# DeMoriarty/TorchPQ

Hardware: AMD Instinct MI355X
Metric: queries/sec + recall@100, SIFT1M IVFPQ d=128 m=64 nprobe=32 (higher is better)
Workload: dtype f32; 1 GPU; SIFT1M-like d=128 n=1000000 IVFPQ n_cells=1024 m=64 nprobe=32 k=100 on 1xMI355X per rank; n_query_per_rank=10000, code_layout=packed, codes=u8 (8-bit PQ), arithmetic=f32 LUT entries, f32 sums, exact ids, use_smart_probing=False, parallelism=query-sharded x1, replicated index, world_size_seen=1, index_broadcast_bytes=0

## Files before the change

include/torchpq_amd.h:

```cpp
#ifndef TORCHPQ_AMD_H_
#define TORCHPQ_AMD_H_

#include <stddef.h>
#include <stdint.h>

#ifdef __cplusplus
extern "C" {
#endif

#define TPQ_VERSION 500

#define TPQ_OK 0
#define TPQ_ERR_INVALID_ARGUMENT (-1)
#define TPQ_ERR_HIP (-2)
#define TPQ_ERR_WORKSPACE (-3)
#define TPQ_ERR_UNSUPPORTED (-4)

#define TPQ_METRIC_NEG_SQ_L2 0
#define TPQ_METRIC_INNER 1

typedef void* tpq_stream_t;

int tpq_version(void);
const char* tpq_last_error(void);

size_t tpq_ivfpq_scan_workspace_bytes(int nq, int k, int n_split, int m);

int tpq_ivfpq_scan_topk(const uint8_t* codes, const float* lut, const uint8_t* is_empty,
                        const int64_t* cell_start, const int64_t* cell_size,
                        const int64_t* n_probe_list, float* out_vals, int64_t* out_addr,
                        const int64_t* address2id, int64_t* out_ids, int64_t n_slots, int nq,
                        int max_nprobe, int m, int k, int n_split, void* workspace,
                        size_t workspace_bytes, tpq_stream_t stream);

int tpq_ivfpq_pack_codes(const uint8_t* codes, uint8_t* packed, int64_t n_slots, int m,
                         int64_t slot_begin, int64_t slot_end, tpq_stream_t stream);

int tpq_ivfpq_scan_topk_packed(const uint8_t* packed, const uint8_t* codes, const float* lut,
                               const uint8_t* is_empty, const int64_t* cell_start,
                               const int64_t* cell_size, const int64_t* n_probe_list,
                               float* out_vals, int64_t* out_addr, const int64_t* address2id,
                               int64_t* out_ids, int64_t n_slots, int nq, int max_nprobe, int m,
                               int k, int n_split, void* workspace, size_t workspace_bytes,
                               tpq_stream_t stream);
size_t tpq_ivfpq_scan_tickets_bytes(int nq);

#define TPQ_SCAN_ROUTE_REF 0
#define TPQ_SCAN_ROUTE_ONE_LAUNCH 1
#define TPQ_SCAN_ROUTE_LISTS 2
#define TPQ_SCAN_ROUTE_POOLS 3
#define TPQ_SCAN_ROUTE_DUMP_F32 8
#define TPQ_SCAN_ROUTE_DUMP_SEL16 16
#define TPQ_SCAN_ROUTE_DUMP_SEL16_W8 17
int tpq_ivfpq_scan_route(int nq, int k, int n_split, int m, int ds, int max_nprobe, int64_t slots_hint, int has_lut,
                         int has_packed, int has_tickets, int residual);
int tpq_ivfpq_scan_order(const int64_t* cell_start, const int64_t* cell_size, const int64_t* n_probe_list, int nq,
                         int max_nprobe, int tile_shift, int32_t* order, int32_t* rank, int32_t* work,
                         tpq_stream_t stream);
int tpq_ivfpq_scan_ordered(int nq, int k, int n_split, int m, int ds, int max_nprobe, int64_t slots_hint, int has_lut,
                           int has_packed, int has_tickets, int residual, int slots, size_t workspace_bytes);
int tpq_ivfpq_scan_topk_packed_tickets(const uint8_t* packed, const uint8_t* codes, const float* lut,
                                       const uint8_t* is_empty, const int64_t* cell_start,
                                       const int64_t* cell_size, const int64_t* n_probe_list,
                                       float* out_vals, int64_t* out_addr, const int64_t* address2id,
                                       int64_t* out_ids, int64_t n_slots, int nq, int max_nprobe,
                                       int m, int k, int n_split, void* workspace,
                                       size_t workspace_bytes, int32_t* tickets, int64_t slots_hint,
                                       tpq_stream_t stream);

int tpq_ivfpq_search_fused(const uint8_t* packed, const uint8_t* codes, const float* query,
                           const float* codebook, int ds, int metric, const uint8_t* is_empty,
                           const int64_t* cell_start, const int64_t* cell_size,
                           const int64_t* n_probe_list, float* out_vals, int64_t* out_addr,
                           const int64_t* address2id, int64_t* out_ids, int64_t n_slots, int nq,
                           int max_nprobe, int m, int k, int n_split, void* workspace,
                           size_t workspace_bytes, tpq_stream_t stream);
int tpq_ivfpq_search_fused_tickets(const uint8_t* packed, const uint8_t* codes, const float* query,
                                   const float* codebook, int ds, int metric, const uint8_t* is_empty,
                                   const int64_t* cell_start, const int64_t* cell_size,
                                   const int64_t* n_probe_list, float* out_vals, int64_t* out_addr,
                                   const int64_t* address2id, int64_t* out_ids, int64_t n_slots,
                                   int nq, int max_nprobe, int m, int k, int n_split, void* workspace,
                                   size_t workspace_bytes, int32_t* tickets, int64_t slots_hint,
                                   tpq_stream_t stream);
int tpq_ivfpq_search_fused_cells(const uint8_t* packed, const uint8_t* codes, const float* query,
                                 const float* codebook, int ds, int metric, const uint8_t* is_empty,
                                 const int64_t* cell_start, const int64_t* cell_size,
                                 const int64_t* n_probe_list, float* out_vals, int64_t* out_addr,
                                 const int64_t* address2id, int64_t* out_ids, int64_t n_slots,
                                 int nq, int max_nprobe, int m, int k, int n_split, void* workspace,
                                 size_t workspace_bytes, int32_t* tickets, int64_t slots_hint,
                                 const int64_t* cells, int n_cells, tpq_stream_t stream);
int tpq_ivfpq_scan_cell_major(int nq, int k, int n_split, int m, int ds, int max_nprobe, int64_t slots_hint, int has_lut,
                              int has_packed, int has_tickets, int residual, int n_cells, int64_t n_slots,
                              size_t workspace_bytes);
int tpq_ivfpq_scan_cell_norms(int nq, int k, int n_split, int m, int ds, int max_nprobe, int64_t slots_hint, int has_lut,
                              int has_packed, int has_tickets, int residual, int n_cells, int64_t n_slots,
                              size_t workspace_bytes);
size_t tpq_ivfpq_cell_candidates_workspace_bytes(int nq, int max_nprobe, int n_cells, int first_probe);
size_t tpq_ivfpq_cell_candidates_norms_workspace_bytes(int nq, int max_nprobe, int n_cells, int first_probe,
                                                       int64_t n_slots);
int tpq_ivfpq_cell_candidates(const uint8_t* codes, const float* query, const float* codebook, int ds, int metric,
                              const uint8_t* is_empty, const int64_t* cell_start, const int64_t* cell_size,
                              const int64_t* n_probe_list, const int64_t* cells, int n_cells, int first_probe,
                              const float* threshold, int64_t n_slots, int nq, int max_nprobe, int m, int capacity,
                              int32_t* out_count, uint32_t* out_keys, uint32_t* out_addr, float* out_delta,
                              int32_t* out_flags, void* workspace, size_t workspace_bytes, tpq_stream_t stream);
float tpq_ivfpq_cell_fold_threshold(float threshold, float q2);
int tpq_ivfpq_scan_cell_threshold(int nq, int k, int n_split, int m, int ds, int max_nprobe, int64_t slots_hint,
                                  int has_lut, int has_packed, int has_tickets, int residual, int n_cells,
                                  int64_t n_slots, size_t workspace_bytes);
int tpq_ivfpq_scan_use_cell_threshold(int on);
int tpq_ivfpq_scan_cell_threshold_probes(void);

int tpq_ivfpq_scan_topk_residual(const uint8_t* codes, const float* part1, const float* part2,
                                 const float* full_lut, const int64_t* cells,
                                 const float* base_sims, const uint8_t* is_empty,
                                 const int64_t* cell_start, const int64_t* cell_size,
                                 const int64_t* n_probe_list, float* out_vals, int64_t* out_addr,
                                 const int64_t* address2id, int64_t* out_ids, int64_t n_slots,
                                 int nq, int max_nprobe, int m, int k, tpq_stream_t stream);
int tpq_residual_part1(const float* query, const float* codebook, float* part1, int m, int ds,
                       int nq, tpq_stream_t stream);

int tpq_ivfpq_residual_slot_terms(const uint8_t* codes, const float* part2,
                                  const int64_t* cell_start, const int64_t* cell_size,
                                  float* slot_term, float* cell_bound, int64_t n_slots,
                                  int n_cells, int m, tpq_stream_t stream);
int tpq_ivfpq_scan_topk_residual_packed(
    const uint8_t* packed, const uint8_t* codes, const float* part1, const float* query,
    const float* codebook, int ds, const float* part2, const float* slot_term,
    const float* cell_bound, const int64_t* cells, const float* base_sims, const uint8_t* is_empty,
    const int64_t* cell_start, const int64_t* cell_size, const int64_t* n_probe_list,
    float* out_vals, int64_t* out_addr, const int64_t* address2id, int64_t* out_ids,
    int64_t n_slots, int nq, int max_nprobe, int m, int k, int n_split, void* workspace,
    size_t workspace_bytes, tpq_stream_t stream);

int tpq_adc_lut(const float* query, const float* codebook, float* lut, int m, int ds, int nq,
                int metric, tpq_stream_t stream);

int tpq_topk_select(const float* x, float* vals, int64_t* idx, int rows, int cols, int k,
                    tpq_stream_t stream);

int tpq_coarse_select(const float* dots, const float* a2, const float* b2, float* vals, int64_t* idx,
                      int rows, int cols, int k, tpq_stream_t stream);

size_t tpq_ivfpq_coarse_probe_workspace_bytes(int nq, int n_cells);
int tpq_ivfpq_coarse_probe(const float* query, const float* centroids,
                           const int64_t* cell_start_tbl, const int64_t* cell_size_tbl,
                           float* topk_sims, int64_t* cells, int64_t* cell_start,
                           int64_t* cell_size, int64_t* n_probe_list, int d, int nq, int n_cells,
                           int n_probe, float smart_temperature, void* workspace,
                           size_t workspace_bytes, tpq_stream_t stream);
#define TPQ_PROBE_ROUTE_AUTO 0
#define TPQ_PROBE_ROUTE_FP32 1
#define TPQ_PROBE_ROUTE_FP16 2
size_t tpq_ivfpq_coarse_probe_route_workspace_bytes(int d, int nq, int n_cells, int route);
int tpq_ivfpq_coarse_probe_route(const float* query, const float* centroids,
                                 const int64_t* cell_start_tbl, const int64_t* cell_size_tbl,
                                 float* topk_sims, int64_t* cells, int64_t* cell_start,
                                 int64_t* cell_size, int64_t* n_probe_list, int d, int nq, int n_cells,
                                 int n_probe, float smart_temperature, int route, const void* prepared,
                                 void* workspace, size_t workspace_bytes, tpq_stream_t stream);
size_t tpq_ivfpq_coarse_probe_prepared_bytes(int d, int n_cells);
int tpq_ivfpq_coarse_probe_prepare(const float* centroids, int d, int n_cells, void* prepared,
                                   size_t prepared_bytes, tpq_stream_t stream);

int tpq_smart_probing(const float* topk_sims, int64_t* n_probe_list, int rows, int n_probe,
                      float temperature, tpq_stream_t stream);

int tpq_get_address_by_id(const int64_t* address2id, int64_t capacity, const int64_t* ids,
                          int64_t* address, int64_t n_ids, tpq_stream_t stream);

int tpq_get_id_by_address(const int64_t* address2id, int64_t capacity, const int64_t* address,
                          int64_t* ids, int64_t n, tpq_stream_t stream);

int tpq_max_sim(const float* A, const float* B, float* vals, int64_t* inds, int l, int d, int m,
                int n, int metric, tpq_stream_t stream);

int tpq_max_sim_split_supported(int d, int64_t m, int n);
int tpq_max_sim_split(const float* A, const float* B, float* vals, int64_t* inds, int l, int d, int m,
                      int n, int metric, tpq_stream_t stream);

#define TPQ_ASSIGN_ROUTE_AUTO 0
#define TPQ_ASSIGN_ROUTE_CASCADE 1
int tpq_coarse_assign_supported(int d, int64_t m, int n);
size_t tpq_coarse_assign_workspace_bytes(int d, int64_t m, int n);
size_t tpq_coarse_assign_count_offset(int d, int64_t m, int n);
int tpq_coarse_assign(const float* A, const float* B, float* vals, int64_t* inds, int d, int64_t m, int n,
                      int metric, void* workspace, size_t workspace_bytes, tpq_stream_t stream);
size_t tpq_coarse_assign_route_workspace_bytes(int d, int64_t m, int n, int route);
int tpq_coarse_assign_route(const float* A, const float* B, float* vals, int64_t* inds, int d, int64_t m, int n,
                            int metric, int route, void* workspace, size_t workspace_bytes, tpq_stream_t stream);

int tpq_max_sim_select_supported(int l, int d, int64_t m, int n);
size_t tpq_max_sim_select_workspace_bytes(int l, int d, int64_t m, int n);
int tpq_max_sim_select(const float* A, const float* B, float* vals, int64_t* inds, int l, int d, int64_t m,
                       int n, int metric, void* workspace, size_t workspace_bytes, tpq_stream_t stream);

int tpq_lloyd_supported(int l, int d, int64_t m, int n);
size_t tpq_lloyd_prepared_bytes(int l, int d, int64_t m);
int tpq_lloyd_prepare(const float* data, const float* centroids0, void* prepared, size_t prepared_bytes,
                      int l, int d, int64_t m, int n, tpq_stream_t stream);
size_t tpq_lloyd_step_workspace_bytes(int l, int d, int64_t m, int n);
size_t tpq_lloyd_step_count_offset(int l, int d, int64_t m, int n, int level);
int tpq_lloyd_step(const float* data, const void* prepared, const float* centroids, float* new_centroids,
                   float* vals, int64_t* inds, int l, int d, int64_t m, int n, void* workspace,
                   size_t workspace_bytes, tpq_stream_t stream);

size_t tpq_compute_centroids_workspace_bytes(int l, int d, int k);
int tpq_compute_centroids(const float* data, const int64_t* labels, float* centroids, int l, int d,
                          int64_t n, int k, void* workspace, size_t workspace_bytes,
                          tpq_stream_t stream);

size_t tpq_get_ioa_workspace_bytes(int64_t n);
int tpq_get_ioa(const int64_t* labels, int64_t* ioa, int64_t n, int64_t n_cells, void* workspace,
                size_t workspace_bytes, tpq_stream_t stream);
int tpq_get_write_address(const uint8_t* is_empty, const int64_t* cell_start,
                          const int64_t* cell_capacity, const int64_t* labels, const int64_t* ioa,
                          int64_t* write_address, int64_t n_slots, int64_t n_labels,
                          tpq_stream_t stream);
int tpq_get_cell_by_address(const int64_t* address, const int64_t* cell_start,
                            const int64_t* cell_capacity, int64_t* cells, int64_t n_address,
                            int64_t n_cells, tpq_stream_t stream);

int tpq_grow_cells(const uint8_t* storage, const int64_t* address2id, const uint8_t* is_empty,
                   const int64_t* old_start, const int64_t* old_capacity, const int64_t* new_start,
                   const int64_t* new_capacity, uint8_t* new_storage, int64_t* new_address2id,
                   uint8_t* new_is_empty, int64_t old_slots, int64_t new_slots, int n_cells, int m,
                   tpq_stream_t stream);

int tpq_pq_decode(const float* codebook, const uint8_t* codes, float* out, int m, int ds, int64_t n,
                  tpq_stream_t stream);

int tpq_scatter_codes(const uint8_t* codes, const int64_t* address, uint8_t* storage,
                      uint8_t* packed, int m, int64_t n, int64_t n_slots, tpq_stream_t stream);

int tpq_ivfpqr_rerank(const uint8_t* storage, int64_t capacity, int m, int m_r, const float* codebook,
                      const float* codebook_r, const float* query, int d, int nq, const int64_t* cand_address,
                      int k1, int k, int use_residual, int distance, const int64_t* address2id, float* out_vals,
                      int64_t* out_address, int64_t* out_ids, tpq_stream_t stream);

size_t tpq_ivfflat_scan_workspace_bytes(int nq, int k, int n_split);
int tpq_ivfflat_scan_topk(const float* vectors, const float* query, const uint8_t* is_empty,
                          const int64_t* cell_start, const int64_t* cell_size, const int64_t* n_probe_list,
                          float* out_vals, int64_t* out_addr, int64_t n_slots, int d, int nq, int max_nprobe, int k,
                          int metric, int n_split, void* workspace, size_t workspace_bytes, tpq_stream_t stream);

size_t tpq_ivfpq4_scan_workspace_bytes(int nq, int k, int n_split);
int tpq_ivfpq4_scan_topk(const uint8_t* codes, const float* query, const float* codebook, const uint8_t* is_empty,
                         const int64_t* cell_start, const int64_t* cell_size, const int64_t* n_probe_list,
                         float* out_vals, int64_t* out_addr, int64_t n_slots, int m, int ds, int nq, int max_nprobe,
                         int k, int metric, int n_split, void* workspace, size_t workspace_bytes,
                         tpq_stream_t stream);

int tpq_ivfpq4_scan_residual_topk(const uint8_t* codes, const float* query, const float* codebook,
                                  const float* centroids, const int64_t* cells, int n_cells, const uint8_t* is_empty,
                                  const int64_t* cell_start, const int64_t* cell_size, const int64_t* n_probe_list,
                                  float* out_vals, int64_t* out_addr, int64_t n_slots, int m, int ds, int nq,
                                  int max_nprobe, int k, int metric, int n_split, void* workspace,
                                  size_t workspace_bytes, tpq_stream_t stream);

size_t tpq_ivfflat_range_segments(int nq, int n_split);
int tpq_ivfflat_range_count(const float* vectors, const float* query, const uint8_t* is_empty,
                            const int64_t* cell_start, const int64_t* cell_size, const int64_t* n_probe_list,
                            const float* threshold, int32_t* wave_counts, int64_t n_slots, int d, int nq,
// ... 92 lines not shown
```

torchpq_amd/_lib.py:

```python
from __future__ import annotations

import ctypes as C
import os

import torch

_HERE = os.path.dirname(os.path.abspath(__file__))
LIB_PATH = os.environ.get("TPQ_AMD_LIB") or os.path.join(_HERE, "libtorchpq_amd.so")

METRIC_NEG_SQ_L2 = 0
METRIC_INNER = 1
ERR_UNSUPPORTED = -4
ERR_WORKSPACE = -3
ASSIGN_ROUTE_AUTO = 0
ASSIGN_ROUTE_CASCADE = 1
PROBE_ROUTE_AUTO, PROBE_ROUTE_FP32, PROBE_ROUTE_FP16 = 0, 1, 2

_vp, _i, _i64, _sz, _f = C.c_void_p, C.c_int, C.c_int64, C.c_size_t, C.c_float

SIGNATURES = {
    "tpq_version": (_i, []),
    "tpq_last_error": (C.c_char_p, []),
    "tpq_ivfpq_scan_workspace_bytes": (_sz, [_i, _i, _i, _i]),
    "tpq_ivfpq_scan_topk": (_i, [_vp, _vp, _vp, _vp, _vp, _vp, _vp, _vp, _vp, _vp, _i64, _i, _i, _i,
                                 _i, _i, _vp, _sz, _vp]),
    "tpq_ivfpq_pack_codes": (_i, [_vp, _vp, _i64, _i, _i64, _i64, _vp]),
    "tpq_ivfpq_scan_topk_packed": (_i, [_vp, _vp, _vp, _vp, _vp, _vp, _vp, _vp, _vp, _vp, _vp, _i64,
                                        _i, _i, _i, _i, _i, _vp, _sz, _vp]),
    "tpq_ivfpq_search_fused": (_i, [_vp, _vp, _vp, _vp, _i, _i, _vp, _vp, _vp, _vp, _vp, _vp, _vp, _vp,
                                    _i64, _i, _i, _i, _i, _i, _vp, _sz, _vp]),
    "tpq_ivfpq_scan_tickets_bytes": (_sz, [_i]),
    "tpq_ivfpq_scan_route": (_i, [_i, _i, _i, _i, _i, _i, _i64, _i, _i, _i, _i]),
    "tpq_ivfpq_scan_order": (_i, [_vp, _vp, _vp, _i, _i, _i, _vp, _vp, _vp, _vp]),
    "tpq_ivfpq_scan_ordered": (_i, [_i, _i, _i, _i, _i, _i, _i64, _i, _i, _i, _i, _i, _sz]),
    "tpq_ivfpq_scan_topk_packed_tickets": (_i, [_vp, _vp, _vp, _vp, _vp, _vp, _vp, _vp, _vp, _vp, _vp, _i64,
                                                _i, _i, _i, _i, _i, _vp, _sz, _vp, _i64, _vp]),
    "tpq_ivfpq_search_fused_tickets": (_i, [_vp, _vp, _vp, _vp, _i, _i, _vp, _vp, _vp, _vp, _vp, _vp, _vp, _vp,
                                            _i64, _i, _i, _i, _i, _i, _vp, _sz, _vp, _i64, _vp]),
    "tpq_ivfpq_search_fused_cells": (_i, [_vp, _vp, _vp, _vp, _i, _i, _vp, _vp, _vp, _vp, _vp, _vp, _vp, _vp,
                                          _i64, _i, _i, _i, _i, _i, _vp, _sz, _vp, _i64, _vp, _i, _vp]),
    "tpq_ivfpq_scan_cell_major": (_i, [_i, _i, _i, _i, _i, _i, _i64, _i, _i, _i, _i, _i, _i64, _sz]),
    "tpq_ivfpq_scan_cell_norms": (_i, [_i, _i, _i, _i, _i, _i, _i64, _i, _i, _i, _i, _i, _i64, _sz]),
    "tpq_ivfpq_cell_candidates_workspace_bytes": (_sz, [_i, _i, _i, _i]),
    "tpq_ivfpq_cell_candidates_norms_workspace_bytes": (_sz, [_i, _i, _i, _i, _i64]),
    "tpq_ivfpq_cell_candidates": (_i, [_vp, _vp, _vp, _i, _i, _vp, _vp, _vp, _vp, _vp, _i, _i, _vp, _i64, _i, _i, _i,
                                       _i, _vp, _vp, _vp, _vp, _vp, _vp, _sz, _vp]),
    "tpq_ivfpq_cell_fold_threshold": (_f, [_f, _f]),
    "tpq_ivfpq_scan_cell_threshold": (_i, [_i, _i, _i, _i, _i, _i, _i64, _i, _i, _i, _i, _i, _i64, _sz]),
    "tpq_ivfpq_scan_use_cell_threshold": (_i, [_i]),
    "tpq_ivfpq_scan_cell_threshold_probes": (_i, []),
    "tpq_ivfpq_scan_topk_residual": (_i, [_vp, _vp, _vp, _vp, _vp, _vp, _vp, _vp, _vp, _vp, _vp, _vp,
                                          _vp, _vp, _i64, _i, _i, _i, _i, _vp]),
    "tpq_residual_part1": (_i, [_vp, _vp, _vp, _i, _i, _i, _vp]),
    "tpq_ivfpq_residual_slot_terms": (_i, [_vp, _vp, _vp, _vp, _vp, _vp, _i64, _i, _i, _vp]),
    "tpq_ivfpq_scan_topk_residual_packed": (_i, [_vp, _vp, _vp, _vp, _vp, _i, _vp, _vp, _vp, _vp, _vp,
                                                 _vp, _vp, _vp, _vp, _vp, _vp, _vp, _vp, _i64, _i, _i,
                                                 _i, _i, _i, _vp, _sz, _vp]),
    "tpq_adc_lut": (_i, [_vp, _vp, _vp, _i, _i, _i, _i, _vp]),
    "tpq_topk_select": (_i, [_vp, _vp, _vp, _i, _i, _i, _vp]),
    "tpq_coarse_select": (_i, [_vp, _vp, _vp, _vp, _vp, _i, _i, _i, _vp]),
    "tpq_smart_probing": (_i, [_vp, _vp, _i, _i, _f, _vp]),
    "tpq_ivfpq_coarse_probe_workspace_bytes": (_sz, [_i, _i]),
    "tpq_ivfpq_coarse_probe": (_i, [_vp, _vp, _vp, _vp, _vp, _vp, _vp, _vp, _vp, _i, _i, _i, _i, _f,
                                    _vp, _sz, _vp]),
    "tpq_ivfpq_coarse_probe_route_workspace_bytes": (_sz, [_i, _i, _i, _i]),
    "tpq_ivfpq_coarse_probe_route": (_i, [_vp, _vp, _vp, _vp, _vp, _vp, _vp, _vp, _vp, _i, _i, _i, _i, _f, _i,
                                          _vp, _vp, _sz, _vp]),
    "tpq_ivfpq_coarse_probe_prepared_bytes": (_sz, [_i, _i]),
    "tpq_ivfpq_coarse_probe_prepare": (_i, [_vp, _i, _i, _vp, _sz, _vp]),
    "tpq_get_id_by_address": (_i, [_vp, _i64, _vp, _vp, _i64, _vp]),
    "tpq_get_address_by_id": (_i, [_vp, _i64, _vp, _vp, _i64, _vp]),
    "tpq_max_sim": (_i, [_vp, _vp, _vp, _vp, _i, _i, _i, _i, _i, _vp]),
    "tpq_max_sim_split_supported": (_i, [_i, _i64, _i]),
    "tpq_max_sim_split": (_i, [_vp, _vp, _vp, _vp, _i, _i, _i, _i, _i, _vp]),
    "tpq_max_sim_select_supported": (_i, [_i, _i, _i64, _i]),
    "tpq_max_sim_select_workspace_bytes": (_sz, [_i, _i, _i64, _i]),
    "tpq_max_sim_select": (_i, [_vp, _vp, _vp, _vp, _i, _i, _i64, _i, _i, _vp, _sz, _vp]),
    "tpq_lloyd_supported": (_i, [_i, _i, _i64, _i]),
    "tpq_lloyd_prepared_bytes": (_sz, [_i, _i, _i64]),
    "tpq_lloyd_prepare": (_i, [_vp, _vp, _vp, _sz, _i, _i, _i64, _i, _vp]),
    "tpq_lloyd_step_workspace_bytes": (_sz, [_i, _i, _i64, _i]),
    "tpq_lloyd_step_count_offset": (_sz, [_i, _i, _i64, _i, _i]),
    "tpq_lloyd_step": (_i, [_vp, _vp, _vp, _vp, _vp, _vp, _i, _i, _i64, _i, _vp, _sz, _vp]),
    "tpq_coarse_assign_supported": (_i, [_i, _i64, _i]),
    "tpq_coarse_assign_workspace_bytes": (_sz, [_i, _i64, _i]),
    "tpq_coarse_assign_count_offset": (_sz, [_i, _i64, _i]),
    "tpq_coarse_assign": (_i, [_vp, _vp, _vp, _vp, _i, _i64, _i, _i, _vp, _sz, _vp]),
    "tpq_coarse_assign_route_workspace_bytes": (_sz, [_i, _i64, _i, _i]),
    "tpq_coarse_assign_route": (_i, [_vp, _vp, _vp, _vp, _i, _i64, _i, _i, _i, _vp, _sz, _vp]),
    "tpq_compute_centroids_workspace_bytes": (_sz, [_i, _i, _i]),
    "tpq_compute_centroids": (_i, [_vp, _vp, _vp, _i, _i, _i64, _i, _vp, _sz, _vp]),
    "tpq_get_ioa_workspace_bytes": (_sz, [_i64]),
    "tpq_get_ioa": (_i, [_vp, _vp, _i64, _i64, _vp, _sz, _vp]),
    "tpq_get_write_address": (_i, [_vp, _vp, _vp, _vp, _vp, _vp, _i64, _i64, _vp]),
    "tpq_get_cell_by_address": (_i, [_vp, _vp, _vp, _vp, _i64, _i64, _vp]),
    "tpq_grow_cells": (_i, [_vp, _vp, _vp, _vp, _vp, _vp, _vp, _vp, _vp, _vp, _i64, _i64, _i, _i, _vp]),
    "tpq_pq_decode": (_i, [_vp, _vp, _vp, _i, _i, _i64, _vp]),
    "tpq_scatter_codes": (_i, [_vp, _vp, _vp, _vp, _i, _i64, _i64, _vp]),
    "tpq_ivfpqr_rerank": (_i, [_vp, _i64, _i, _i, _vp, _vp, _vp, _i, _i, _vp, _i, _i, _i, _i, _vp, _vp, _vp, _vp,
                               _vp]),
    "tpq_ivfflat_scan_workspace_bytes": (_sz, [_i, _i, _i]),
    "tpq_ivfflat_scan_topk": (_i, [_vp, _vp, _vp, _vp, _vp, _vp, _vp, _vp, _i64, _i, _i, _i, _i, _i, _i, _vp, _sz,
                                   _vp]),
    "tpq_ivfpq4_scan_workspace_bytes": (_sz, [_i, _i, _i]),
    "tpq_ivfpq4_scan_topk": (_i, [_vp] * 9 + [_i64, _i, _i, _i, _i, _i, _i, _i, _vp, _sz, _vp]),
    "tpq_ivfpq4_scan_residual_topk": (_i, [_vp] * 5 + [_i] + [_vp] * 6 + [_i64, _i, _i, _i, _i, _i, _i, _i, _vp, _sz,
                                           _vp]),
    "tpq_ivfpq4_scan_filtered_topk": (_i, [_vp] * 9 + [_i, _i64, _vp, _vp, _i64, _i, _i, _i, _i, _i, _i, _i, _vp, _sz,
                                           _vp]),
    "tpq_ivfpq4_scan_filtered_residual_topk": (_i, [_vp] * 5 + [_i] + [_vp] * 6 + [_i, _i64, _vp, _vp, _i64, _i, _i,
                                                    _i, _i, _i, _i, _i, _vp, _sz, _vp]),
    "tpq_ivfflat_range_segments": (_sz, [_i, _i]),
    "tpq_ivfflat_range_count": (_i, [_vp, _vp, _vp, _vp, _vp, _vp, _vp, _vp, _i64, _i, _i, _i, _i, _i, _vp]),
    "tpq_ivfflat_range_fill": (_i, [_vp, _vp, _vp, _vp, _vp, _vp, _vp, _vp, _vp, _vp, _i64, _i, _i, _i, _i, _i,
                                    _vp]),
    "tpq_ivfpq_range_segments": (_sz, [_i, _i]),
    "tpq_ivfpq_range_count": (_i, [_vp] * 4 + [_i, _i] + [_vp] * 6 + [_i64, _i, _i, _i, _i, _vp]),
    "tpq_ivfpq_range_fill": (_i, [_vp] * 4 + [_i, _i] + [_vp] * 8 + [_i64, _i, _i, _i, _i, _vp]),
    "tpq_ivfpq_range_residual_segments": (_sz, [_i, _i]),
    "tpq_ivfpq_range_residual_count": (_i, [_vp] * 4 + [_i] + [_vp] * 10 + [_i64, _i, _i, _i, _vp]),
    "tpq_ivfpq_range_residual_fill": (_i, [_vp] * 4 + [_i] + [_vp] * 12 + [_i64, _i, _i, _i, _vp]),
    "tpq_ivfpq_scan_filtered_workspace_bytes": (_sz, [_i, _i, _i]),
    "tpq_ivfpq_scan_filtered_topk": (_i, [_vp] * 4 + [_i, _i] + [_vp] * 6 + [_i, _i64] + [_vp] * 4
                                     + [_i64, _i, _i, _i, _i, _i, _vp, _sz, _vp]),
    "tpq_ivfpq_scan_filtered_residual_topk": (_i, [_vp] * 4 + [_i] + [_vp] * 10 + [_i, _i64] + [_vp] * 4
                                              + [_i64, _i, _i, _i, _i, _vp]),
    "tpq_slot_filter_build": (_i, [_vp, _i64, _vp, _i64, _vp]),
    "tpq_flat_topk_workspace_bytes": (_sz, [_i, _i, _i]),
    "tpq_flat_topk": (_i, [_vp, _vp, _vp, _vp, _vp, _vp, _i64, _i, _i, _i, _i, _i, _vp, _sz, _vp]),
    "tpq_flat_range_segments": (_sz, [_i, _i]),
    "tpq_flat_range_count": (_i, [_vp, _vp, _vp, _vp, _vp, _i64, _i, _i, _i, _i, _vp]),
    "tpq_flat_range_fill": (_i, [_vp, _vp, _vp, _vp, _vp, _vp, _vp, _vp, _i64, _i, _i, _i, _i, _vp]),
    "tpq_ubench_stream_read": (_i, [_vp, _sz, _vp, _i, _vp]),
    "tpq_ubench_stream_read_ex": (_i, [_vp, _sz, _vp, _i, _i, _i, _sz, _i, _vp]),
    "tpq_ubench_rows_read": (_i, [_vp, _i, _i, _i64, _i, _vp, _vp]),
}

_lib = None


class TorchPQAmdError(RuntimeError):
    pass


def load():
    global _lib
    if _lib is None:
        if not os.path.exists(LIB_PATH):
            raise TorchPQAmdError(
                f"{LIB_PATH} not found: build it with `python -c 'import __graft_entry__ as g; "
                "g.build()'` (or torchpq_amd/csrc/build.sh). torchpq_amd has no CPU fallback.")
        lib = C.CDLL(LIB_PATH)
        for name, (res, args) in SIGNATURES.items():
            fn = getattr(lib, name)
            fn.restype = res
            fn.argtypes = args
        _lib = lib
    return _lib


def last_error() -> str:
    msg = load().tpq_last_error()
    return msg.decode("utf-8", "replace") if msg else ""


def check(rc: int, what: str):
    if rc != 0:
        raise TorchPQAmdError(f"{what} failed (code {rc}): {last_error()}")


def ptr(t):
    return None if t is None else C.c_void_p(t.data_ptr())


def stream_ptr(device=None):
    return C.c_void_p(torch.cuda.current_stream(device).cuda_stream)


def require_gpu(*tensors):
    for t in tensors:
        if t is None:
            continue
        if t.device.type != "cuda":
            raise TorchPQAmdError(
                "torchpq_amd runs on an AMD GPU (torch device 'cuda'); got a tensor on "
                f"'{t.device}'. There is no CPU fallback.")
        if not t.is_contiguous():
            raise TorchPQAmdError("torchpq_amd kernels need contiguous tensors")
```

torchpq_amd/csrc/scan.hip:

```cpp
#include <atomic>
#include <chrono>

#include "scan_cells.h"
#include "scan_device.h"
#include "scan_order.h"
#include "scan_ref.h"

namespace tpq {

__global__ __launch_bounds__(256) void residual_part1_kernel(const float* __restrict__ query,
                                                            const float* __restrict__ codebook,
                                                            float* __restrict__ part1, int m,
                                                            int ds, int nq) {
  const int j = blockIdx.y, q = blockIdx.x, c = threadIdx.x;
  float dot = 0.f;
  for (int e = 0; e < ds; ++e)
    dot = fmaf(query[(int64_t)(j * ds + e) * nq + q], codebook[((int64_t)j * ds + e) * 256 + c], dot);
  part1[((int64_t)q * m + j) * 256 + c] = 2.f * dot;
}


static size_t ref_lds_bytes(int m, int R, int max_nprobe, int fused_floats) {
  return list_scan_lds_bytes(list_region0((size_t)m * 1024, R), max_nprobe, (size_t)fused_floats * 4);
}
// ... 114 lines not shown
  }
  if (a.lut || !dump_built(a.m, kDumpSel16) || a.ds > 2) return 0;
  const int rl8 = list_regs_scan(a.k, a.m, a.max_nprobe, a.slots_hint);
  if (rl4 <= 2 || (rl4 <= 4 && rl4 <= rl8)) return kDumpSel16;
  if (e && atoi(e) == 1) return 0;
  if (a.k > 248 && rl8 <= 2) return kDumpSel16W8;
  return 0;
}

template <int N, class Query>
static int device_cached(std::atomic<int> (&cache)[64][N], int i, int fallback, Query query) {
  int dev = 0;
  if (hipGetDevice(&dev) != hipSuccess || dev < 0 || dev >= 64) return fallback;
  int n = cache[dev][i].load(std::memory_order_relaxed);
  if (n <= 0) {
    n = query(dev);
    if (n <= 0) n = fallback;
    cache[dev][i].store(n, std::memory_order_relaxed);
  }
  return n;
}
static int device_cus() {
  static std::atomic<int> cus[64][1] = {};
  return device_cached(cus, 0, 256, [](int dev) {
    int n = 0;
    return hipDeviceGetAttribute(&n, hipDeviceAttributeMultiprocessorCount, dev) == hipSuccess ? n : 0;
  });
}
static int dump_slots(const PackedUnit& u, int mode) {
  static std::atomic<int> per_cu[64][3 * 4] = {};
  const int mi = mode == kDumpSel16 ? 0 : (mode == kDumpF32 ? 1 : 2), ci = u.m == 64 ? 0 : (u.m == 32 ? 1 : (u.m == 16 ? 2 : 3));
  return device_cached(per_cu, mi * 4 + ci, 4, [&](int) { return u.dump_occupancy(mode); }) * device_cus();
}
static void dump_tail(int nq, int nw, int RL, int slots, int* unsplit, int* parts) {
  *unsplit = nq;
  *parts = 1;
  if (slots <= 0) return;
  const int whole = (nq / slots) * slots, rest = nq - whole;
  if (rest == 0) return;
  for (int c = 4; c >= 2; c >>= 1) {
    if ((int64_t)rest * c <= slots && c * nw * RL <= 16) {
      *unsplit = whole;
      *parts = c;
      return;
    }
  }
}

struct ScanPlan {
  int route = -1;
  int R = 0;
  int RL = 0;
  int Rf = 0;
  int mode = 0;
  int waves = 0;
  int n_split = 1;
  bool fuse = false;
  bool small_lists = false;
  int unsplit = 0;
  int parts = 1;
  bool ordered = false;
};

static ScanPlan plan_scan(const ScanArgs& a, bool residual) {
  const int m = a.m, k = a.k;
  ScanPlan p;
  p.n_split = a.n_split;
  if (!packed_unit(m)) {
    if (!residual && !a.lut) p.route = TPQ_SCAN_ROUTE_REF;
    return p;
  }
  p.R = list_regs_packed(k);
  p.waves = packed_waves(m);
  const bool lds_fits =
      scan_lds_bytes_packed(m, p.R > 16 ? 16 : p.R, a.max_nprobe, fused_floats_of(a), residual) <= 160 * 1024;
  if (p.R > 16 || !lds_fits) {
    p.route = TPQ_SCAN_ROUTE_REF;
    if (residual) p.n_split = 1;
    return p;
  }
  const bool pools = !residual && p.R >= pool_min_list_regs(m) && (p.waves < 16 || k > 768) && fuse_enabled();
  const int Rf = dump_finish_regs(k, a.slots_hint), mode = dump_route(a, residual, Rf);
  if (mode && !(is_sel16(mode) && pools)) {
    const int nw = scan_waves(m, mode), RL = list_regs_scan(k, m, a.max_nprobe, a.slots_hint, nw);
    if (dump_pair_built(mode, RL, Rf)) {
      p.route = mode == kDumpF32 ? TPQ_SCAN_ROUTE_DUMP_F32
                                 : (mode == kDumpSel16 ? TPQ_SCAN_ROUTE_DUMP_SEL16 : TPQ_SCAN_ROUTE_DUMP_SEL16_W8);
      p.mode = mode, p.waves = nw, p.RL = RL, p.Rf = Rf, p.n_split = 1;
      return p;
    }
  }
  if (pools) {
    p.route = TPQ_SCAN_ROUTE_POOLS;
    p.RL = pool_list_regs(k, m);
    if (p.n_split > pool_max_split(m, k)) p.n_split = pool_max_split(m, k);
    return p;
  }
  p.RL = list_regs_scan(k, m, a.max_nprobe, a.slots_hint);
  p.small_lists = p.RL < p.R;
  p.fuse = !residual && fuse_enabled() && fuse_fits(m, p.R) && p.waves * p.RL >= p.R && (a.n_split == 1 || a.tickets);
  p.route = p.fuse ? TPQ_SCAN_ROUTE_ONE_LAUNCH : TPQ_SCAN_ROUTE_LISTS;
  return p;
}

static void plan_dump_dispatch(ScanPlan& p, int nq, int slots, size_t workspace_bytes) {
  int unsplit = nq, parts = 1;
  if (p.mode != kDumpSel16W8) dump_tail(nq, p.waves, p.RL, slots, &unsplit, &parts);
  if (parts > 1 && workspace_bytes < ws_bytes_for(nq, p.RL, parts * p.waves)) unsplit = nq, parts = 1;
  p.parts = parts;
  p.unsplit = parts > 1 ? unsplit : 0;
  p.ordered = slots > 0 && nq > slots && nq <= kOrderMaxQueries &&
              workspace_bytes >= ws_bytes_for(nq, p.RL, parts * p.waves) + order_ws_bytes(nq);
}
static bool is_dump_route(int route) {
  return route == TPQ_SCAN_ROUTE_DUMP_F32 || route == TPQ_SCAN_ROUTE_DUMP_SEL16 || route == TPQ_SCAN_ROUTE_DUMP_SEL16_W8;
}

static ScanArgs route_query_args(int nq, int k, int n_split, int m, int ds, int max_nprobe, int64_t slots_hint,
                                 int has_lut, int has_tickets) {
  ScanArgs a{};
  static const float dummy_lut = 0.f;
  static int32_t dummy_tickets = 0;
  a.lut = has_lut ? &dummy_lut : nullptr;
  a.ds = has_lut ? 0 : ds;
  a.nq = nq; a.k = k; a.n_split = n_split; a.m = m; a.max_nprobe = max_nprobe;
  a.slots_hint = slots_hint;
  a.tickets = has_tickets ? &dummy_tickets : nullptr;
  return a;
}

extern "C" int tpq_ivfpq_scan_route(int nq, int k, int n_split, int m, int ds, int max_nprobe, int64_t slots_hint,
                                    int has_lut, int has_packed, int has_tickets, int residual) {
  if (nq <= 0 || k < 1 || k > 1024 || m < 4 || m % 4 != 0 || n_split < 1 || max_nprobe < 1) return -1;
  if (!has_packed) return TPQ_SCAN_ROUTE_REF;
  return plan_scan(route_query_args(nq, k, n_split, m, ds, max_nprobe, slots_hint, has_lut, has_tickets), residual != 0)
      .route;
}

extern "C" int tpq_ivfpq_scan_ordered(int nq, int k, int n_split, int m, int ds, int max_nprobe, int64_t slots_hint,
                                      int has_lut, int has_packed, int has_tickets, int residual, int slots,
                                      size_t workspace_bytes) {
  if (nq <= 0 || k < 1 || k > 1024 || m < 4 || m % 4 != 0 || n_split < 1 || max_nprobe < 1) return -1;
  if (!has_packed) return 0;
  ScanPlan p =
      plan_scan(route_query_args(nq, k, n_split, m, ds, max_nprobe, slots_hint, has_lut, has_tickets), residual != 0);
  if (!is_dump_route(p.route)) return 0;
  plan_dump_dispatch(p, nq, slots > 0 ? slots : dump_slots(*packed_unit(m), p.mode), workspace_bytes);
  return p.ordered ? 1 : 0;
}

struct CellMajor {
  const int64_t* cells;
  int n_cells;
};
static int cell_major_chunks(const ScanArgs& a, const ScanPlan& p, bool residual, int n_cells, size_t workspace_bytes) {
  if (residual || p.route != TPQ_SCAN_ROUTE_DUMP_SEL16 || a.lut || a.m != 64 || a.ds < 1 || a.ds > 2) return 0;
  if (a.k > 128 || a.max_nprobe <= kCellP0 || n_cells < 1 || a.n_slots <= 0 || a.slots_hint <= 0) return 0;
  if ((int64_t)a.nq * a.slots_hint < (int64_t)kCellMinRereads * a.n_slots) return 0;
  if ((int64_t)a.nq * a.max_nprobe >= 0x7fffffffLL) return 0;
  const size_t extra = cell_extra_bytes(a.nq, a.max_nprobe, n_cells, kCellP0);
  for (int chunks = 16; chunks >= 8; chunks >>= 1)
    if ((a.k + 63) / 64 < chunks && workspace_bytes >= ws_bytes_for(a.nq, 1, chunks) + extra) return chunks;
  return 0;
}
static bool cell_major_norms(const ScanArgs& a, int chunks, int n_cells, size_t workspace_bytes) {
  return chunks > 0 && workspace_bytes >= ws_bytes_for(a.nq, 1, chunks) +
                                              cell_extra_bytes(a.nq, a.max_nprobe, n_cells, kCellP0) +
                                              cell_norm_bytes(a.n_slots);
}

static int run_cell_major(ScanArgs& a, ScanPlan p, const PackedUnit& u, const CellMajor& cm, int chunks, void* workspace,
                          size_t workspace_bytes, hipStream_t st) {
  const int nq = a.nq;
  ScanArgs t = a;
  t.probe_cap = kCellP0;
  plan_dump_dispatch(p, nq, dump_slots(u, p.mode), workspace_bytes);
  t.n_split = p.parts;
  t.unsplit = p.unsplit;
  const size_t lists_bytes = ws_bytes_for(nq, p.RL, p.parts * p.waves);
  int rc = need_ws(workspace, workspace_bytes, lists_bytes, "ivfpq_scan_packed");
  if (rc) return rc;
  fill_ws(t, workspace, p.RL, p.parts * p.waves);
  if (p.ordered) {
    int* o = reinterpret_cast<int*>(reinterpret_cast<char*>(workspace) + lists_bytes);
    const size_t stride = order_ws_bytes(nq) / 3 / sizeof(int);
    rc = launch_scan_order(a.cell_start, a.cell_size, a.n_probe_list, nq, a.max_nprobe, packed_tile_shift(a.m), o,
                           o + stride, o + 2 * stride, st, kCellP0);
    if (rc) return rc;
    t.order = o;
    t.rank = o + stride;
  }
  rc = u.dump(t, p.RL, p.Rf, p.mode, st);
  if (rc) return rc;
  a.n_split = 1;
  a.unsplit = 0;
  fill_ws(a, workspace, 1, chunks);
  CellArgs c{};
  c.codes = a.codes; c.query = a.query; c.codebook = a.codebook; c.is_empty = a.is_empty;
  c.cell_start = a.cell_start; c.cell_size = a.cell_size; c.n_probe_list = a.n_probe_list; c.cells = cm.cells;
  c.n_slots = a.n_slots; c.nq = nq; c.max_nprobe = a.max_nprobe; c.n_cells = cm.n_cells; c.ds = a.ds;
  c.euclid = a.euclid; c.p0 = kCellP0; c.p_hi = a.max_nprobe; c.k = a.k; c.chunks = chunks; c.epoch = a.epoch;
  c.rel = cell_delta_rel(a.ds);
  c.seed_vals = a.out_vals; c.seed_addr = a.out_addr;
  c.keys = reinterpret_cast<unsigned*>(a.ws_vals); c.idx = reinterpret_cast<unsigned*>(a.ws_idx);
  c.list_evict = a.list_evict; c.flags = a.flags; c.ws_delta = a.ws_delta;
  const size_t cm_lists = ws_bytes_for(nq, 1, chunks);
  cell_fill_extras(c, reinterpret_cast<char*>(workspace) + cm_lists, workspace_bytes - cm_lists);
  rc = launch_cell_candidates(c, st);
  if (rc) return rc;
  return u.finish(a, chunks, p.Rf, (a.k + 63) / 64, c.cnt, st);
}

static bool cell_threshold_form(const ScanArgs& a, int chunks, int n_cells, size_t workspace_bytes) {
  if (!cell_major_norms(a, chunks, n_cells, workspace_bytes) || a.max_nprobe <= kCellThrProbes) return false;
  const size_t need = ws_bytes_for(a.nq, 1, chunks) + cell_extra_bytes(a.nq, a.max_nprobe, n_cells, kCellP0) +
                      cell_norm_bytes(a.n_slots) + cell_thr_bytes(a.nq, a.max_nprobe, n_cells);
  const int64_t mean_cell = a.slots_hint / a.max_nprobe;
  return workspace_bytes >= need && mean_cell >= kCellThrMinCell &&
         (int64_t)kCellThrProbes * mean_cell / kCellThrGroup >= 2 * (int64_t)a.k;
}

static int run_cell_threshold(ScanArgs& a, const ScanPlan& p, const PackedUnit& u, const CellMajor& cm, int chunks,
                              void* workspace, hipStream_t st) {
  const int nq = a.nq;
  a.n_split = 1;
  a.unsplit = 0;
  fill_ws(a, workspace, 1, chunks);
  CellArgs c{};
  c.codes = a.codes; c.query = a.query; c.codebook = a.codebook; c.is_empty = a.is_empty;
  c.cell_start = a.cell_start; c.cell_size = a.cell_size; c.n_probe_list = a.n_probe_list; c.cells = cm.cells;
  c.n_slots = a.n_slots; c.nq = nq; c.max_nprobe = a.max_nprobe; c.n_cells = cm.n_cells; c.ds = a.ds;
  c.euclid = a.euclid; c.p0 = 0; c.p_hi = a.max_nprobe; c.k = 0; c.thr_k = a.k; c.chunks = chunks; c.epoch = a.epoch;
  c.rel = cell_delta_rel(a.ds);
  c.keys = reinterpret_cast<unsigned*>(a.ws_vals); c.idx = reinterpret_cast<unsigned*>(a.ws_idx);
  c.list_evict = a.list_evict; c.flags = a.flags; c.ws_delta = a.ws_delta;
  char* at = reinterpret_cast<char*>(workspace) + ws_bytes_for(nq, 1, chunks);
  const size_t head = cell_extra_bytes(nq, a.max_nprobe, cm.n_cells, kCellP0) + cell_norm_bytes(a.n_slots);
  cell_fill_extras(c, at, head, kCellP0);
  CellThrArrays t{};
  cell_fill_thr(t, at + head, nq, a.max_nprobe, cm.n_cells);
  int rc = launch_cell_threshold(c, t, st);
  if (rc) return rc;
  return u.finish(a, chunks, p.Rf, 0, c.cnt, st);
}

extern "C" int tpq_ivfpq_scan_cell_major(int nq, int k, int n_split, int m, int ds, int max_nprobe, int64_t slots_hint,
                                         int has_lut, int has_packed, int has_tickets, int residual, int n_cells,
                                         int64_t n_slots, size_t workspace_bytes) {
  if (nq <= 0 || k < 1 || k > 1024 || m < 4 || m % 4 != 0 || n_split < 1 || max_nprobe < 1) return -1;
  if (!has_packed) return 0;
  ScanArgs a = route_query_args(nq, k, n_split, m, ds, max_nprobe, slots_hint, has_lut, has_tickets);
  a.n_slots = n_slots;
  const ScanPlan p = plan_scan(a, residual != 0);
  return cell_major_chunks(a, p, residual != 0, n_cells, workspace_bytes) ? 1 : 0;
}

extern "C" int tpq_ivfpq_scan_cell_norms(int nq, int k, int n_split, int m, int ds, int max_nprobe, int64_t slots_hint,
                                         int has_lut, int has_packed, int has_tickets, int residual, int n_cells,
                                         int64_t n_slots, size_t workspace_bytes) {
  if (nq <= 0 || k < 1 || k > 1024 || m < 4 || m % 4 != 0 || n_split < 1 || max_nprobe < 1) return -1;
  if (!has_packed) return 0;
  ScanArgs a = route_query_args(nq, k, n_split, m, ds, max_nprobe, slots_hint, has_lut, has_tickets);
  a.n_slots = n_slots;
  const ScanPlan p = plan_scan(a, residual != 0);
  const int chunks = cell_major_chunks(a, p, residual != 0, n_cells, workspace_bytes);
  return cell_major_norms(a, chunks, n_cells, workspace_bytes) ? 1 : 0;
}

extern "C" int tpq_ivfpq_scan_cell_threshold(int nq, int k, int n_split, int m, int ds, int max_nprobe,
                                             int64_t slots_hint, int has_lut, int has_packed, int has_tickets,
                                             int residual, int n_cells, int64_t n_slots, size_t workspace_bytes) {
  if (nq <= 0 || k < 1 || k > 1024 || m < 4 || m % 4 != 0 || n_split < 1 || max_nprobe < 1) return -1;
  if (!has_packed) return 0;
  ScanArgs a = route_query_args(nq, k, n_split, m, ds, max_nprobe, slots_hint, has_lut, has_tickets);
  a.n_slots = n_slots;
  const ScanPlan p = plan_scan(a, residual != 0);
  const int chunks = cell_major_chunks(a, p, residual != 0, n_cells, workspace_bytes);
  return cell_threshold_form(a, chunks, n_cells, workspace_bytes) ? 1 : 0;
}

static std::atomic<int> g_cell_threshold{1};
extern "C" int tpq_ivfpq_scan_use_cell_threshold(int on) { return g_cell_threshold.exchange(on ? 1 : 0); }
extern "C" int tpq_ivfpq_scan_cell_threshold_probes(void) { return kCellThrProbes; }

static int run_packed(ScanArgs a, const ResidualArgs* ra, void* workspace, size_t workspace_bytes,
                      tpq_stream_t stream, const CellMajor* cm = nullptr) {
  int rc = validate(a);
  if (rc) return rc;
  TPQ_REQUIRE(a.packed != nullptr, "ivfpq_scan_packed: null packed pointer");
  if (a.nq == 0) return TPQ_OK;
  hipStream_t st = reinterpret_cast<hipStream_t>(stream);
  ScanPlan p = plan_scan(a, ra != nullptr);
  if (p.route == TPQ_SCAN_ROUTE_REF) {
    a.n_split = p.n_split;
    return ra ? run_residual_ref(a, *ra, st) : run_ref(a, workspace, workspace_bytes, st);
  }
  if (p.route < 0) {
    set_error("ivfpq_scan_packed: no scan-layout kernel instantiated for n_subvectors=%d; use "
              "tpq_ivfpq_scan_topk", a.m);
    return TPQ_ERR_UNSUPPORTED;
  }
  const PackedUnit& u = *packed_unit(a.m);
  const int nq = a.nq;
  a.n_split = p.n_split;
  a.small_lists = p.small_lists;
  a.fuse = p.fuse;
  if (!p.fuse) a.tickets = nullptr;
  a.epoch = fresh_epoch();
#ifdef TPQ_SCAN_PROFILE
  a.prof = g_scan_prof;
#endif
  switch (p.route) {
    case TPQ_SCAN_ROUTE_POOLS: {
      const int n_lists = p.n_split * p.waves;
      rc = need_ws(workspace, workspace_bytes, pool_ws_bytes(nq, a.k, a.m, n_lists), "ivfpq_scan_packed");
      if (rc) return rc;
      fill_ws_pool(a, workspace, n_lists);
      rc = u.pool(a, p.RL, st);
      break;
    }
    case TPQ_SCAN_ROUTE_DUMP_F32:
    case TPQ_SCAN_ROUTE_DUMP_SEL16:
    case TPQ_SCAN_ROUTE_DUMP_SEL16_W8: {
      if (const int chunks = cm ? cell_major_chunks(a, p, ra != nullptr, cm->n_cells, workspace ? workspace_bytes : 0) : 0) {
        rc = g_cell_threshold.load() && cell_threshold_form(a, chunks, cm->n_cells, workspace_bytes)
                 ? run_cell_threshold(a, p, u, *cm, chunks, workspace, st)
                 : run_cell_major(a, p, u, *cm, chunks, workspace, workspace_bytes, st);
        break;
      }
      plan_dump_dispatch(p, nq, dump_slots(u, p.mode), workspace ? workspace_bytes : 0);
      a.n_split = p.parts;
      a.unsplit = p.unsplit;
      const size_t lists_bytes = ws_bytes_for(nq, p.RL, p.parts * p.waves);
      rc = need_ws(workspace, workspace_bytes, lists_bytes, "ivfpq_scan_packed");
      if (rc) return rc;
      fill_ws(a, workspace, p.RL, p.parts * p.waves);
      if (p.ordered) {
        int* o = reinterpret_cast<int*>(reinterpret_cast<char*>(workspace) + lists_bytes);
        const size_t stride = order_ws_bytes(nq) / 3 / sizeof(int);
        rc = launch_scan_order(a.cell_start, a.cell_size, a.n_probe_list, nq, a.max_nprobe, packed_tile_shift(a.m), o,
                               o + stride, o + 2 * stride, st, 0);
        if (rc) return rc;
        a.order = o;
        a.rank = o + stride;
      }
      rc = u.dump(a, p.RL, p.Rf, p.mode, st);
      break;
    }
    default: {
      const int n_lists = p.n_split * p.waves;
      rc = need_ws(workspace, workspace_bytes, ws_bytes_for(nq, p.RL, n_lists), "ivfpq_scan_packed");
      if (rc) return rc;
      fill_ws(a, workspace, p.RL, n_lists);
      rc = u.packed(a, ra, p.RL, p.R, st);
      if (p.fuse) return rc;
    }
  }
  if (rc) return rc;
  return redo_flagged(a, ra, st);
}

extern "C" size_t tpq_ivfpq_scan_tickets_bytes(int nq) { return nq > 0 ? (size_t)nq * sizeof(int32_t) : 0; }

extern "C" int tpq_ivfpq_search_fused_cells(const uint8_t* packed, const uint8_t* codes,
                                            const float* query, const float* codebook, int ds,
                                            int metric, const uint8_t* is_empty,
                                            const int64_t* cell_start, const int64_t* cell_size,
                                            const int64_t* n_probe_list, float* out_vals,
                                            int64_t* out_addr, const int64_t* address2id,
                                            int64_t* out_ids, int64_t n_slots, int nq, int max_nprobe,
                                            int m, int k, int n_split, void* workspace,
                                            size_t workspace_bytes, int32_t* tickets,
                                            int64_t slots_hint, const int64_t* cells, int n_cells,
                                            tpq_stream_t stream) {
  TPQ_REQUIRE(metric == TPQ_METRIC_NEG_SQ_L2 || metric == TPQ_METRIC_INNER,
              "ivfpq_search_fused: bad metric %d", metric);
  TPQ_REQUIRE(ds >= 1 && ds <= 1024, "ivfpq_search_fused: bad sub-vector length %d", ds);
  ScanArgs a = scan_args(codes, packed, nullptr, is_empty, cell_start, cell_size, n_probe_list, out_vals, out_addr,
                         address2id, out_ids, n_slots, nq, max_nprobe, m, k, n_split);
  a.query = query; a.codebook = codebook; a.ds = ds; a.euclid = metric == TPQ_METRIC_NEG_SQ_L2 ? 1 : 0;
  a.tickets = tickets; a.slots_hint = slots_hint;
  const CellMajor cm{cells, n_cells};
  return packed ? run_packed(a, nullptr, workspace, workspace_bytes, stream, cells ? &cm : nullptr)
                : run_ref(a, workspace, workspace_bytes, reinterpret_cast<hipStream_t>(stream));
}

extern "C" int tpq_ivfpq_search_fused_tickets(const uint8_t* packed, const uint8_t* codes,
                                              const float* query, const float* codebook, int ds,
                                              int metric, const uint8_t* is_empty,
                                              const int64_t* cell_start, const int64_t* cell_size,
                                              const int64_t* n_probe_list, float* out_vals,
                                              int64_t* out_addr, const int64_t* address2id,
                                              int64_t* out_ids, int64_t n_slots, int nq, int max_nprobe,
                                              int m, int k, int n_split, void* workspace,
                                              size_t workspace_bytes, int32_t* tickets,
                                              int64_t slots_hint, tpq_stream_t stream) {
  return tpq_ivfpq_search_fused_cells(packed, codes, query, codebook, ds, metric, is_empty, cell_start, cell_size,
                                      n_probe_list, out_vals, out_addr, address2id, out_ids, n_slots, nq, max_nprobe, m,
                                      k, n_split, workspace, workspace_bytes, tickets, slots_hint, nullptr, 0, stream);
}

extern "C" int tpq_ivfpq_search_fused(const uint8_t* packed, const uint8_t* codes,
                                      const float* query, const float* codebook, int ds,
                                      int metric, const uint8_t* is_empty,
                                      const int64_t* cell_start, const int64_t* cell_size,
                                      const int64_t* n_probe_list, float* out_vals,
                                      int64_t* out_addr, const int64_t* address2id,
                                      int64_t* out_ids, int64_t n_slots, int nq, int max_nprobe,
                                      int m, int k, int n_split, void* workspace,
                                      size_t workspace_bytes, tpq_stream_t stream) {
  return tpq_ivfpq_search_fused_tickets(packed, codes, query, codebook, ds, metric, is_empty, cell_start,
                                        cell_size, n_probe_list, out_vals, out_addr, address2id, out_ids,
                                        n_slots, nq, max_nprobe, m, k, n_split, workspace, workspace_bytes,
                                        nullptr, 0, stream);
}

extern "C" int tpq_ivfpq_scan_topk(const uint8_t* codes, const float* lut, const uint8_t* is_empty,
                                   const int64_t* cell_start, const int64_t* cell_size,
                                   const int64_t* n_probe_list, float* out_vals, int64_t* out_addr,
                                   const int64_t* address2id, int64_t* out_ids, int64_t n_slots,
                                   int nq, int max_nprobe, int m, int k, int n_split,
                                   void* workspace, size_t workspace_bytes, tpq_stream_t stream) {
  const ScanArgs a = scan_args(codes, nullptr, lut, is_empty, cell_start, cell_size, n_probe_list, out_vals, out_addr,
                               address2id, out_ids, n_slots, nq, max_nprobe, m, k, n_split);
  return run_ref(a, workspace, workspace_bytes, reinterpret_cast<hipStream_t>(stream));
}

extern "C" int tpq_ivfpq_scan_topk_packed_tickets(const uint8_t* packed, const uint8_t* codes,
                                                  const float* lut, const uint8_t* is_empty,
                                                  const int64_t* cell_start, const int64_t* cell_size,
                                                  const int64_t* n_probe_list, float* out_vals,
                                                  int64_t* out_addr, const int64_t* address2id,
                                                  int64_t* out_ids, int64_t n_slots, int nq, int max_nprobe,
                                                  int m, int k, int n_split, void* workspace,
                                                  size_t workspace_bytes, int32_t* tickets,
                                                  int64_t slots_hint, tpq_stream_t stream) {
  ScanArgs a = scan_args(codes, packed, lut, is_empty, cell_start, cell_size, n_probe_list, out_vals, out_addr,
                         address2id, out_ids, n_slots, nq, max_nprobe, m, k, n_split);
  a.tickets = tickets; a.slots_hint = slots_hint;
  return run_packed(a, nullptr, workspace, workspace_bytes, stream);
}

extern "C" int tpq_ivfpq_scan_topk_packed(const uint8_t* packed, const uint8_t* codes,
                                          const float* lut, const uint8_t* is_empty,
                                          const int64_t* cell_start, const int64_t* cell_size,
                                          const int64_t* n_probe_list, float* out_vals,
                                          int64_t* out_addr, const int64_t* address2id,
                                          int64_t* out_ids, int64_t n_slots, int nq, int max_nprobe,
                                          int m, int k, int n_split, void* workspace,
                                          size_t workspace_bytes, tpq_stream_t stream) {
  return tpq_ivfpq_scan_topk_packed_tickets(packed, codes, lut, is_empty, cell_start, cell_size, n_probe_list,
                                            out_vals, out_addr, address2id, out_ids, n_slots, nq, max_nprobe, m,
                                            k, n_split, workspace, workspace_bytes, nullptr, 0, stream);
}

extern "C" int tpq_ivfpq_scan_topk_residual(const uint8_t* codes, const float* part1,
                                            const float* part2, const float* full_lut,
                                            const int64_t* cells, const float* base_sims,
                                            const uint8_t* is_empty, const int64_t* cell_start,
                                            const int64_t* cell_size, const int64_t* n_probe_list,
                                            float* out_vals, int64_t* out_addr,
                                            const int64_t* address2id, int64_t* out_ids,
                                            int64_t n_slots, int nq, int max_nprobe, int m, int k,
                                            tpq_stream_t stream) {
  const ScanArgs a = scan_args(codes, nullptr, part1 ? part1 : full_lut, is_empty, cell_start, cell_size, n_probe_list,
                               out_vals, out_addr, address2id, out_ids, n_slots, nq, max_nprobe, m, k, 1);
  int rc = validate(a);
  if (rc) return rc;
  TPQ_REQUIRE(base_sims != nullptr, "ivfpq_scan_residual: base_sims is required");
  TPQ_REQUIRE(full_lut != nullptr || (part1 && part2 && cells),
              "ivfpq_scan_residual: need either full_lut or (part1, part2, cells)");
  if (nq == 0) return TPQ_OK;
  ResidualArgs ra{part1, part2, full_lut, cells, base_sims, nullptr, nullptr};
  return run_residual_ref(a, ra, reinterpret_cast<hipStream_t>(stream));
}

extern "C" int tpq_ivfpq_scan_topk_residual_packed(
    const uint8_t* packed, const uint8_t* codes, const float* part1, const float* query,
    const float* codebook, int ds, const float* part2, const float* slot_term,
    const float* cell_bound, const int64_t* cells, const float* base_sims, const uint8_t* is_empty,
    const int64_t* cell_start, const int64_t* cell_size, const int64_t* n_probe_list,
    float* out_vals, int64_t* out_addr, const int64_t* address2id, int64_t* out_ids,
    int64_t n_slots, int nq, int max_nprobe, int m, int k, int n_split, void* workspace,
    size_t workspace_bytes, tpq_stream_t stream) {
  TPQ_REQUIRE(part1 || (query && codebook && ds >= 1 && ds <= 1024),
              "ivfpq_scan_residual_packed: need part1 or (query, codebook, ds)");
  TPQ_REQUIRE(part2 && slot_term && cell_bound && cells && base_sims,
              "ivfpq_scan_residual_packed: null pointer argument");
  ScanArgs a = scan_args(codes, packed, part1, is_empty, cell_start, cell_size, n_probe_list, out_vals, out_addr,
                         address2id, out_ids, n_slots, nq, max_nprobe, m, k, n_split);
  a.query = query; a.codebook = codebook; a.ds = ds;
  a.euclid = 2;
  ResidualArgs ra{part1, part2, nullptr, cells, base_sims, slot_term, cell_bound};
  return run_packed(a, &ra, workspace, workspace_bytes, stream);
}

namespace tpq {
__global__ __launch_bounds__(256) void residual_slot_term_kernel(
    const uint32_t* __restrict__ codes32, const float* __restrict__ part2,
    const int64_t* __restrict__ cell_start, const int64_t* __restrict__ cell_size,
    float* __restrict__ slot_term, int64_t n_slots, int m) {
  const int cell = blockIdx.x;
  const float* __restrict__ p2 = part2 + (int64_t)cell * m * 256;
  const int64_t st = cell_start[cell], sz = cell_size[cell];
  const int G = m >> 2;
  for (int64_t o = (int64_t)blockIdx.y * 256 + threadIdx.x; o < sz; o += (int64_t)gridDim.y * 256) {
    const int64_t s = st + o;
    float v = 0.f;
    for (int g = 0; g < G; ++g) {
      const uint32_t w = codes32[(int64_t)g * n_slots + s];
      v = lut_word(v, p2 + g * 1024, w);
    }
    slot_term[s] = v;
  }
}

__global__ __launch_bounds__(64) void residual_cell_bound_kernel(const float* __restrict__ part2,
                                                                 float* __restrict__ cell_bound,
                                                                 int m) {
  const int cell = blockIdx.x, lane = threadIdx.x;
  const float4* __restrict__ p2 = reinterpret_cast<const float4*>(part2 + (int64_t)cell * m * 256);
  float sum = 0.f;
  for (int j = 0; j < m; ++j) {
    const float4 x = p2[j * 64 + lane];
    float mx = fmaxf(fmaxf(fabsf(x.x), fabsf(x.y)), fmaxf(fabsf(x.z), fabsf(x.w)));
#pragma unroll
    for (int d = 32; d > 0; d >>= 1) mx = fmaxf(mx, __shfl_xor(mx, d, 64));
    sum += mx;
  }
  if (lane == 0) cell_bound[cell] = sum;
}
}

extern "C" int tpq_ivfpq_residual_slot_terms(const uint8_t* codes, const float* part2,
                                             const int64_t* cell_start, const int64_t* cell_size,
                                             float* slot_term, float* cell_bound, int64_t n_slots,
                                             int n_cells, int m, tpq_stream_t stream) {
// ... 31 lines not shown
```

torchpq_amd/csrc/scan_cells.h:

```cpp
#pragma once
#include "common.h"

namespace tpq {

#ifndef TPQ_CELL_P0
#define TPQ_CELL_P0 4
#endif
constexpr int kCellP0 = TPQ_CELL_P0;
#ifndef TPQ_CELL_THR_PROBES
#define TPQ_CELL_THR_PROBES 6
#endif
#ifndef TPQ_CELL_THR_GROUP
#define TPQ_CELL_THR_GROUP 16
#endif
constexpr int kCellThrProbes = TPQ_CELL_THR_PROBES;
constexpr int kCellThrGroup = TPQ_CELL_THR_GROUP;
static_assert(kCellThrGroup == 8 || kCellThrGroup == 16, "a group is half or all of a lane's 16 rows of a tile");
constexpr int kCellThrMinCell = 512;
constexpr int kCellMinRereads = 96;
constexpr int kCellQSplit = 256;
constexpr int kCellGroup = 32;
#ifndef TPQ_CELL_SLICE
#define TPQ_CELL_SLICE 128
#endif
constexpr int kCellSlice = TPQ_CELL_SLICE;
constexpr int kCellLdsCells = 16384;

struct CellArgs {
  const uint8_t* codes;
  const float* query;
  const float* codebook;
  const uint8_t* is_empty;
  const int64_t* cell_start;
  const int64_t* cell_size;
  const int64_t* n_probe_list;
  const int64_t* cells;
  int64_t n_slots;
  int nq, max_nprobe, n_cells, ds, euclid;
  int p0;
  int p_hi;
  int k;
  int thr_k;
  int work;
  int chunks;
  int epoch;
  float rel;
  const float* seed_vals;
  const int64_t* seed_addr;
  const float* thr_in;
  unsigned* keys;
  unsigned* idx;
  int* list_evict;
  int* flags;
  float* ws_delta;
  float* params;
  float* thr;
  float* qscale;
  float* qnorm;
  int* cnt;
  int* hist;
  int* cell_off;
  int* blk_off;
  int* cell_st;
  int* cell_sz;
  int* pairs;
  _Float16* qsplit;
  float* norm;
  int* hist2;
  int* n_max;
};
struct CellThrArrays {
  int* pairs_b;
  int *hist, *cell_off, *blk_off, *cell_st, *cell_sz, *pairs, *n_max;
};

inline size_t cell_align(size_t x) { return (x + 255) & ~(size_t)255; }
inline size_t cell_extra_bytes(int nq, int max_nprobe, int n_cells, int p0) {
  const int np = max_nprobe > p0 ? max_nprobe - p0 : 0;
  return 256 + 4 * cell_align((size_t)nq * 4) + cell_align((size_t)n_cells * 4) +
         2 * cell_align(((size_t)n_cells + 1) * 4) + 2 * cell_align((size_t)n_cells * 4) +
         cell_align((size_t)nq * np * 4) + cell_align((size_t)nq * kCellQSplit * 2);
}
inline size_t cell_norm_bytes(int64_t n_slots) { return cell_align((size_t)(n_slots > 0 ? n_slots : 0) * 4); }
inline size_t cell_thr_bytes(int nq, int max_nprobe, int n_cells) {
  const int t = max_nprobe < kCellThrProbes ? max_nprobe : kCellThrProbes;
  return cell_align((size_t)nq * max_nprobe * 4) + 3 * cell_align((size_t)n_cells * 4) +
         2 * cell_align(((size_t)n_cells + 1) * 4) + cell_align((size_t)nq * t * 4) + cell_align((size_t)nq * 4);
}
__host__ __device__ inline int cell_float_ord(float f) {
  const unsigned b = __builtin_bit_cast(unsigned, f);
  return (b & 0x80000000u) ? (int)(0x80000000u - b) : (int)b;
}
__host__ __device__ inline float cell_ord_float(int o) {
  return __builtin_bit_cast(float, o >= 0 ? (unsigned)o : 0x80000000u - (unsigned)o);
}
__host__ __device__ inline float cell_fold_threshold(float thr, float q2) {
  constexpr long long kTop = 0x7f800000;
  if (!(thr == thr) || thr == __builtin_inff() || thr == -__builtin_inff()) return thr;
  auto pass = [&](long long o) { return (cell_ord_float((int)o) - q2) >= thr; };
  const float t0 = thr + q2;
  if (!(t0 == t0)) return t0;
  long long lo, hi, step = 1;
  if (pass(cell_float_ord(t0))) {
    hi = cell_float_ord(t0);
    for (;; step *= 2) {
      lo = hi - step > -kTop ? hi - step : -kTop;
      if (lo == -kTop || !pass(lo)) break;
      hi = lo;
    }
  } else {
    lo = cell_float_ord(t0);
    for (;; step *= 2) {
      hi = lo + step < kTop ? lo + step : kTop;
      if (hi == kTop || pass(hi)) break;
      lo = hi;
    }
  }
  while (hi - lo > 1) {
    const long long mid = lo + (hi - lo) / 2;
    if (pass(mid)) hi = mid; else lo = mid;
  }
  return cell_ord_float((int)hi);
}

void cell_fill_extras(CellArgs& a, void* at, size_t room, int layout_p0 = -1);
float cell_delta_rel(int ds);
int launch_cell_candidates(const CellArgs& a, hipStream_t st);
void cell_fill_thr(CellThrArrays& t, void* at, int nq, int max_nprobe, int n_cells);
int launch_cell_threshold(const CellArgs& a, const CellThrArrays& t, hipStream_t st);

}
```

torchpq_amd/csrc/scan_cells.hip:

```cpp
#include <cmath>

#include "mfma_util.h"
#include "scan_cells.h"
#include "scan_fk.h"
#include "wave_topk.h"

namespace tpq {

float cell_delta_rel(int ds) {
  const double D = 64.0 * ds, N = 3.0 * D, u = 1.0 / 16777216.0;
  const double sum = 0.5 * (3.03 * 4 * u + 1.003 * N * 2 * u) + 1.01 * std::sqrt(D) * u / 4 + (D + 1) * u + 14 * u + 4 * u +
                     1.001 * (64 + ds + 2) * u;
  return (float)(1.25 * sum * (1.0 + 1.0 / 1024));
}

void cell_fill_extras(CellArgs& a, void* at, size_t room, int layout_p0) {
  char* p = reinterpret_cast<char*>(at);
  const int p0 = layout_p0 >= 0 ? layout_p0 : a.p0;
  const size_t extras = cell_extra_bytes(a.nq, a.max_nprobe, a.n_cells, p0);
  a.norm = room >= extras && room - extras >= cell_norm_bytes(a.n_slots) ? reinterpret_cast<float*>(p + extras) : nullptr;
  auto take = [&](size_t bytes) {
    char* r = p;
    p += cell_align(bytes);
    return r;
  };
  const int np = a.max_nprobe > p0 ? a.max_nprobe - p0 : 0;
  a.params = reinterpret_cast<float*>(take(256));
  a.thr = reinterpret_cast<float*>(take((size_t)a.nq * 4));
  a.qscale = reinterpret_cast<float*>(take((size_t)a.nq * 4));
  a.qnorm = reinterpret_cast<float*>(take((size_t)a.nq * 4));
  a.cnt = reinterpret_cast<int*>(take((size_t)a.nq * 4));
  a.hist = reinterpret_cast<int*>(take((size_t)a.n_cells * 4));
  a.cell_off = reinterpret_cast<int*>(take(((size_t)a.n_cells + 1) * 4));
  a.blk_off = reinterpret_cast<int*>(take(((size_t)a.n_cells + 1) * 4));
  a.cell_st = reinterpret_cast<int*>(take((size_t)a.n_cells * 4));
  a.cell_sz = reinterpret_cast<int*>(take((size_t)a.n_cells * 4));
  a.pairs = reinterpret_cast<int*>(take((size_t)a.nq * np * 4));
  a.qsplit = reinterpret_cast<_Float16*>(take((size_t)a.nq * kCellQSplit * 2));
}

constexpr int kCellScaleExp = 12;
constexpr int kCellMaxExp = 40;
constexpr unsigned kMaxFiniteBits = 0x7f7fffffu;

__device__ __forceinline__ float pow2i(int e) { return __uint_as_float((unsigned)(e + 127) << 23); }
__device__ __forceinline__ int exp_of_bits(unsigned bits) { return (int)((bits >> 23) & 255u) - 127; }

__global__ __launch_bounds__(1024) void cell_prep_kernel(CellArgs a) {
  __shared__ unsigned maxbits_s;
  __shared__ float c2max_s[64];
  const int tid = (int)threadIdx.x, lane = tid & 63, wave = tid >> 6;
  if (tid == 0) maxbits_s = 0u;
  for (int i = tid; i < a.n_cells; i += 1024) a.hist[i] = 0;
  if (a.hist2)
    for (int i = tid; i < a.n_cells; i += 1024) a.hist2[i] = 0;
  __syncthreads();
  unsigned mb = 0u;
  for (int j = wave; j < 64; j += 16) {
    float c2m = 0.f;
    for (int c = lane; c < 256; c += 64) {
      float c2 = 0.f;
      for (int e = 0; e < a.ds; ++e) {
        const float y = a.codebook[((int64_t)j * a.ds + e) * 256 + c];
        const unsigned b = __float_as_uint(y) & 0x7fffffffu;
        mb = b > mb ? b : mb;
        c2 = fmaf(y, y, c2);
      }
      c2m = fmaxf(c2m, c2);
    }
#pragma unroll
    for (int d = 32; d > 0; d >>= 1) c2m = fmaxf(c2m, __shfl_xor(c2m, d, 64));
    if (lane == 0) c2max_s[j] = c2m;
  }
  atomicMax(&maxbits_s, mb);
  __syncthreads();
  if (tid == 0) {
    float x2 = 0.f;
    for (int j = 0; j < 64; ++j) x2 += c2max_s[j];
    x2 *= 1.0001f;
    const unsigned bits = maxbits_s;
    const int e = exp_of_bits(bits);
    const bool ok = bits != 0u && bits <= kMaxFiniteBits && e >= -kCellMaxExp && e <= kCellMaxExp && x2 <= 3e38f;
    a.params[0] = __uint_as_float(bits);
    a.params[1] = x2;
    a.params[2] = ok ? 1.f : 0.f;
    a.params[3] = ok ? pow2i(kCellScaleExp - e) : 0.f;
    reinterpret_cast<int*>(a.params)[8] = 0;
    reinterpret_cast<int*>(a.params)[9] = 0;
  }
}

struct ListedProbe {
  bool listed;
  int cell;
};
__device__ __forceinline__ int cell_n_probe(const CellArgs& a, int q) {
  const int n = (int)a.n_probe_list[q];
  return n < 0 ? 0 : (n > a.p_hi ? a.p_hi : n);
}
__device__ __forceinline__ ListedProbe listed_probe(const CellArgs& a, int q, int p) {
  const int64_t o = (int64_t)q * a.max_nprobe + p;
  const int64_t st = a.cell_start[o], sz = a.cell_size[o];
  const bool again = p > 0 && a.cell_start[o - 1] == st;
  return ListedProbe{sz > 0 && !again, (int)a.cells[o]};
}

__global__ __launch_bounds__(256) void cell_seed_kernel(CellArgs a) {
  const int lane = (int)(threadIdx.x & 63);
  const int q = (int)blockIdx.x * 4 + (int)(threadIdx.x >> 6);
  if (q >= a.nq) return;
  const int D = 64 * a.ds;
  const float x0 = lane < D ? a.query[(int64_t)lane * a.nq + q] : 0.f;
  const float x1 = 64 + lane < D ? a.query[(int64_t)(64 + lane) * a.nq + q] : 0.f;
  unsigned mb = __float_as_uint(x0) & 0x7fffffffu;
  const unsigned mb1 = __float_as_uint(x1) & 0x7fffffffu;
  mb = mb1 > mb ? mb1 : mb;
  float q2 = fmaf(x1, x1, x0 * x0);
#pragma unroll
  for (int d = 32; d > 0; d >>= 1) {
    const unsigned o = (unsigned)__shfl_xor((int)mb, d, 64);
    mb = o > mb ? o : mb;
    q2 += __shfl_xor(q2, d, 64);
  }
  const int n_probe = cell_n_probe(a, q);
  bool bad_cell = false;
  for (int p = a.p0 + lane; p < n_probe; p += 64) {
    const int64_t c = a.cells[(int64_t)q * a.max_nprobe + p];
    bad_cell = bad_cell || c < 0 || c >= (int64_t)a.n_cells;
  }
  bad_cell = __ballot(bad_cell) != 0ull;
  const float tau = a.k > 0 ? a.seed_vals[(int64_t)q * a.k + a.k - 1] : (a.thr_k > 0 ? 0.f : a.thr_in[q]);
  const int eq = exp_of_bits(mb);
  const bool flagged = a.k > 0 && a.flags[q] == a.epoch;
  const bool scalable = a.params[2] != 0.f && mb != 0u && mb <= kMaxFiniteBits && eq >= -kCellMaxExp &&
                        eq <= kCellMaxExp && q2 <= 3e38f;
  const bool tau_ok = tau == tau && tau != INFINITY;
  const bool active = !flagged && scalable && tau_ok && !bad_cell;
  if (!active) {
    if (lane == 0) {
      a.flags[q] = a.epoch;
      a.cnt[q] = 0;
      a.thr[q] = INFINITY;
    }
    return;
  }
  const float B = sqrtf(q2) * 1.000001f + sqrtf(a.params[1]) * 1.000001f;
  const float delta = a.rel * (B * B);
  if (lane == 0) {
    if (a.thr_k == 0) a.thr[q] = a.euclid ? cell_fold_threshold(tau - delta, q2) : tau - delta;
    a.ws_delta[q] = 2.f * delta;
    a.qscale[q] = pow2i(kCellScaleExp - eq);
    a.qnorm[q] = q2;
    a.cnt[q] = 0;
    if (a.k == 0) a.flags[q] = 0;
  }
  if (a.list_evict && lane < a.chunks) a.list_evict[(int64_t)q * a.chunks + lane] = 0;
  {
    const float sq = pow2i(kCellScaleExp - eq);
    _Float16* qs = a.qsplit + (int64_t)q * kCellQSplit;
    const float y0 = x0 * sq, y1 = x1 * sq;
    const _Float16 h0 = (_Float16)y0, h1 = (_Float16)y1;
    if (lane < D) {
      qs[lane] = h0;
      qs[128 + lane] = (_Float16)(y0 - (float)h0);
    }
    if (64 + lane < D) {
      qs[64 + lane] = h1;
      qs[192 + lane] = (_Float16)(y1 - (float)h1);
    }
  }
  const int64_t base = (int64_t)q * a.chunks * 64;
  const int seed_chunks = (a.k + 63) / 64;
  for (int t = 0; t < a.chunks; ++t) {
    const int e = t * 64 + lane;
    Key key = pad_key();
    if (e < a.k) {
      const int64_t ad = a.seed_addr[(int64_t)q * a.k + e];
      if (ad >= 0) key = make_key(a.seed_vals[(int64_t)q * a.k + e], (int)ad);
    }
    if (t < seed_chunks) a.keys[base + e] = key.hi;
    a.idx[base + e] = key.lo;
  }
}

constexpr int kCellSliceThreads = 1024;
template <class F>
__device__ __forceinline__ void for_slice_pairs(const CellArgs& a, int q0, F&& f) {
  const int np = a.p_hi - a.p0;
  const int nqs = a.nq - q0 < kCellSlice ? a.nq - q0 : kCellSlice;
  for (int i = (int)threadIdx.x; i < nqs * np; i += kCellSliceThreads) {
    const int dq = i / np;
    const int q = q0 + dq, p = a.p0 + (i - dq * np);
    if (p >= cell_n_probe(a, q) || a.flags[q] == a.epoch) continue;
    const ListedProbe lp = listed_probe(a, q, p);
    if (lp.listed) f(q, p, lp.cell);
  }
}
__device__ __forceinline__ void count_slice(const CellArgs& a, int q0, int* cell_h) {
  for (int c = (int)threadIdx.x; c < a.n_cells; c += kCellSliceThreads) cell_h[c] = 0;
  __syncthreads();
  for_slice_pairs(a, q0, [&](int, int, int c) { atomicAdd(&cell_h[c], 1); });
  __syncthreads();
}

__global__ __launch_bounds__(kCellSliceThreads) void cell_count_kernel(CellArgs a) {
  extern __shared__ int cell_h[];
  count_slice(a, (int)blockIdx.x * kCellSlice, cell_h);
  for (int c = (int)threadIdx.x; c < a.n_cells; c += kCellSliceThreads) {
    const int h = cell_h[c];
    if (h) atomicAdd(&a.hist[c], h);
  }
}

__global__ __launch_bounds__(256) void cell_count_wide_kernel(CellArgs a) {
  const int lane = (int)(threadIdx.x & 63);
  const int q = (int)blockIdx.x * 4 + (int)(threadIdx.x >> 6);
  if (q >= a.nq) return;
  if (a.flags[q] == a.epoch) return;
  const int n_probe = cell_n_probe(a, q);
  for (int p = a.p0 + lane; p < n_probe; p += 64) {
    const ListedProbe lp = listed_probe(a, q, p);
    if (lp.listed) atomicAdd(&a.hist[lp.cell], 1);
  }
}

__global__ __launch_bounds__(1024) void cell_scan_kernel(CellArgs a) {
  __shared__ int sp[2][1024], sb[2][1024];
  const int tid = (int)threadIdx.x;
  const int per = (a.n_cells + 1023) / 1024;
  const int lo = tid * per < a.n_cells ? tid * per : a.n_cells;
  const int hi = lo + per < a.n_cells ? lo + per : a.n_cells;
  int np = 0, nb = 0;
  for (int c = lo; c < hi; ++c) {
    const int h = a.hist[c];
    np += h;
    nb += (h + kCellGroup - 1) / kCellGroup;
  }
  sp[0][tid] = np;
  sb[0][tid] = nb;
  __syncthreads();
  int cur = 0;
  for (int d = 1; d < 1024; d <<= 1) {
    const int vp = sp[cur][tid] + (tid >= d ? sp[cur][tid - d] : 0);
    const int vb = sb[cur][tid] + (tid >= d ? sb[cur][tid - d] : 0);
    sp[cur ^ 1][tid] = vp;
    sb[cur ^ 1][tid] = vb;
    cur ^= 1;
    __syncthreads();
  }
  int op = sp[cur][tid] - np, ob = sb[cur][tid] - nb;
  for (int c = lo; c < hi; ++c) {
    const int h = a.hist[c];
    a.cell_off[c] = op;
    a.blk_off[c] = ob;
    a.hist[c] = op;
    op += h;
    ob += (h + kCellGroup - 1) / kCellGroup;
  }
  if (tid == 1023) {
    a.cell_off[a.n_cells] = sp[cur][1023];
    a.blk_off[a.n_cells] = sb[cur][1023];
  }
}

__device__ __forceinline__ void place_pair(const CellArgs& a, int q, int p, int c, int pos) {
  a.pairs[pos] = q;
  if (pos == a.cell_off[c]) {
    const int64_t o = (int64_t)q * a.max_nprobe + p;
    a.cell_st[c] = (int)a.cell_start[o];
    a.cell_sz[c] = (int)a.cell_size[o];
  }
}

__global__ __launch_bounds__(kCellSliceThreads) void cell_scatter_kernel(CellArgs a) {
  extern __shared__ int cell_h[];
  const int q0 = (int)blockIdx.x * kCellSlice;
  count_slice(a, q0, cell_h);
  for (int c = (int)threadIdx.x; c < a.n_cells; c += kCellSliceThreads) {
    const int h = cell_h[c];
    if (h) cell_h[c] = atomicAdd(&a.hist[c], h);
  }
  __syncthreads();
  for_slice_pairs(a, q0, [&](int q, int p, int c) { place_pair(a, q, p, c, atomicAdd(&cell_h[c], 1)); });
}

__global__ __launch_bounds__(256) void cell_scatter_wide_kernel(CellArgs a) {
  const int lane = (int)(threadIdx.x & 63);
  const int q = (int)blockIdx.x * 4 + (int)(threadIdx.x >> 6);
  if (q >= a.nq) return;
  if (a.flags[q] == a.epoch) return;
  const int n_probe = cell_n_probe(a, q);
  for (int p = a.p0 + lane; p < n_probe; p += 64) {
    const ListedProbe lp = listed_probe(a, q, p);
    if (lp.listed) place_pair(a, q, p, lp.cell, atomicAdd(&a.hist[lp.cell], 1));
  }
}

#ifndef TPQ_CELL_WAVES
#define TPQ_CELL_WAVES 8
#endif
constexpr int kCellWaves = TPQ_CELL_WAVES;
constexpr size_t kCellLdsBytes = 160 * 1024;
template <int DS>
struct CellBook {
  static constexpr int KS = 4 * DS;
  static constexpr size_t kBook = (size_t)64 * 256 * 4 * DS;
  static constexpr int kWaves = kCellWaves;
  static constexpr int kThreads = 64 * kWaves;
  static constexpr size_t kNorms = (size_t)kWaves * 32 * 4;
  static constexpr int kDepth = (int)((kCellLdsBytes - (size_t)64 * 256 * 8 - kNorms) / ((size_t)kWaves * 64 * 8));
  static constexpr size_t kBytes = kBook + kNorms + (size_t)kWaves * 64 * kDepth * 8;
  static_assert(kDepth >= 1 && kBytes <= kCellLdsBytes, "the staging area does not fit the CU's LDS");
};

__device__ __forceinline__ unsigned pack_f16x2(_Float16 lo, _Float16 hi) {
  return (unsigned)__builtin_bit_cast(unsigned short, lo) | ((unsigned)__builtin_bit_cast(unsigned short, hi) << 16);
}
__device__ __forceinline__ float f16_lo(unsigned w) { return (float)__builtin_bit_cast(_Float16, (unsigned short)(w & 0xffffu)); }
__device__ __forceinline__ float f16_hi(unsigned w) { return (float)__builtin_bit_cast(_Float16, (unsigned short)(w >> 16)); }

template <int DS>
__global__ __launch_bounds__(512) void cell_norm_kernel(CellArgs a) {
  constexpr int KS = 4 * DS;
  extern __shared__ __attribute__((aligned(16))) char smem[];
  float* sums = reinterpret_cast<float*>(smem);
  const int tid = (int)threadIdx.x;
  const float sx = a.params[3];
  const float inv_sx = 1.f / sx;
  const float inv_sx2 = inv_sx * inv_sx;
  for (int i = tid; i < 64 * 256; i += 512) {
    const int j = i >> 8, c = i & 255;
#pragma unroll
    for (int e = 0; e < DS; ++e) {
      const float ys = a.codebook[(j * DS + e) * 256 + c] * sx;
      const _Float16 h = (_Float16)ys;
      const _Float16 l = (_Float16)(ys - (float)h);
      sums[i * DS + e] = (float)h + (float)l;
    }
  }
  __syncthreads();
  for (int c = (int)blockIdx.x; c < a.n_cells; c += (int)gridDim.x) {
    if (a.cell_off[c + 1] == a.cell_off[c]) continue;
    const int64_t st = a.cell_st[c];
    int sz = a.cell_sz[c];
    if (st < 0 || sz < 0 || st + sz > a.n_slots) sz = 0;
    for (int r = tid; r < sz; r += 512) {
      const int64_t slot = st + r;
      const uint32_t* __restrict__ cw = reinterpret_cast<const uint32_t*>(a.codes) + slot;
      uint32_t w[16];
#pragma unroll
      for (int g = 0; g < 16; ++g) w[g] = cw[(int64_t)g * a.n_slots];
      const bool empty = a.is_empty && a.is_empty[slot];
      float x2h[2];
#pragma unroll
      for (int half = 0; half < 2; ++half) {
        float x2 = 0.f;
#pragma unroll
        for (int s = 0; s < KS; ++s) {
#pragma unroll
          for (int bb = 0; bb < 8 / DS; ++bb) {
            const int j = (16 * s + 8 * half) / DS + bb;
            const int code = (int)((w[j >> 2] >> (8 * (j & 3))) & 255u);
            if constexpr (DS == 2) {
              const float2 v = reinterpret_cast<const float2*>(sums)[j * 256 + code];
              x2 = fmaf(v.x, v.x, x2);
              x2 = fmaf(v.y, v.y, x2);
            } else {
              const float v = sums[j * 256 + code];
              x2 = fmaf(v, v, x2);
            }
          }
        }
        x2h[half] = x2;
      }
      a.norm[slot] = empty ? __builtin_nanf("") : (x2h[0] + x2h[1]) * inv_sx2;
    }
  }
}

template <int DS, bool NORMS, bool EUCLID, bool MAXIMA = false>
__global__ __launch_bounds__(CellBook<DS>::kThreads) void cell_cand_kernel(CellArgs a) {
  static_assert(!MAXIMA || NORMS, "pass A reads the slot norms");
  using T = CellBook<DS>;
  constexpr int KS = T::KS;
  constexpr int kDepth = T::kDepth;
  extern __shared__ __attribute__((aligned(16))) char smem[];
  unsigned* book = reinterpret_cast<unsigned*>(smem);
  const int tid = (int)threadIdx.x, lane = tid & 63, wave = tid >> 6;
  float* x2w = reinterpret_cast<float*>(smem + T::kBook) + wave * 32;
  uint2* stage = reinterpret_cast<uint2*>(smem + T::kBook + T::kNorms) + wave * (64 * kDepth) + lane;
  int* work = reinterpret_cast<int*>(a.params) + 8 + a.work;
  const int n_blocks = a.blk_off[a.n_cells];
  const int col = lane & 31, half = lane >> 5;
  const float sx = a.params[3];
  const float inv_sx = 1.f / sx;
  const float inv_sx2 = inv_sx * inv_sx;
  const uint8_t* __restrict__ emp = a.is_empty ? a.is_empty : a.codes;
  for (int i = tid; i < 64 * 256; i += T::kThreads) {
    const int j = i >> 8, c = i & 255;
    _Float16 h[DS], l[DS];
#pragma unroll
    for (int e = 0; e < DS; ++e) {
      const float ys = a.codebook[(j * DS + e) * 256 + c] * sx;
      h[e] = (_Float16)ys;
      l[e] = (_Float16)(ys - (float)h[e]);
    }
    if constexpr (DS == 2) {
      book[2 * i] = pack_f16x2(h[0], h[1]);
      book[2 * i + 1] = pack_f16x2(l[0], l[1]);
    } else {
      book[i] = pack_f16x2(h[0], l[0]);
    }
  }
  __syncthreads();
  const int64_t cap = (int64_t)a.chunks * 64;
  const int seed_entries = ((a.k + 63) / 64) * 64;
  for (;;) {
    int b = 0;
    if (lane == 0) b = atomicAdd(work, 1);
    b = __builtin_amdgcn_readfirstlane(b);
    if (b >= n_blocks) break;
    int lo = 0, hi = a.n_cells;
    while (hi - lo > 1) {
      const int mid = (lo + hi) >> 1;
      if (a.blk_off[mid] <= b) lo = mid; else hi = mid;
    }
    const int c = lo, g = b - a.blk_off[c];
    const int first = a.cell_off[c] + g * kCellGroup;
    const int n_listed = a.cell_off[c + 1] - first;
    const int nqs = n_listed < kCellGroup ? n_listed : kCellGroup;
    const int64_t st = a.cell_st[c];
    int sz = a.cell_sz[c];
    if (st < 0 || sz < 0 || st + sz > a.n_slots) sz = 0;
    if (sz == 0) continue;
    const bool qvalid = col < nqs;
    const int q = qvalid ? a.pairs[first + col] : 0;
    const float sq = qvalid ? a.qscale[q] : 0.f;
    const float thr2 = qvalid ? a.thr[q] : INFINITY;
    const float q2 = qvalid ? a.qnorm[q] : 0.f;
    const float unscale = qvalid ? (1.f / sq) * inv_sx : 0.f;
    const float um = EUCLID ? 2.f * unscale : unscale;
    f16x8 qh[KS], ql[KS];
    const _Float16* __restrict__ qs = a.qsplit + (int64_t)q * kCellQSplit + 8 * half;
#pragma unroll
    for (int s = 0; s < KS; ++s) {
      const u32x4 z = {0u, 0u, 0u, 0u};
      qh[s] = __builtin_bit_cast(f16x8, qvalid ? *reinterpret_cast<const u32x4*>(qs + 16 * s) : z);
      ql[s] = __builtin_bit_cast(f16x8, qvalid ? *reinterpret_cast<const u32x4*>(qs + 128 + 16 * s) : z);
    }
    auto load_tile = [&](int r0, uint32_t (&w)[8], unsigned& aux) {
      const int row = r0 + col < sz ? r0 + col : sz - 1;
      const int64_t slot = st + row;
      const uint32_t* __restrict__ cw = reinterpret_cast<const uint32_t*>(a.codes) + slot;
#pragma unroll
      for (int i = 0; i < 8; ++i) {
        const int gq = DS == 2 ? 2 * i + half : 4 * (i >> 1) + 2 * half + (i & 1);
        w[i] = cw[(int64_t)gq * a.n_slots];
      }
      if constexpr (NORMS)
        aux = __float_as_uint(a.norm[slot]);
      else
        aux = emp[slot];
    };
    int fill = 0;
    auto flush = [&]() {
      if (fill > 0) {
        const int64_t e0 = (int64_t)seed_entries + atomicAdd(&a.cnt[q], fill);
        if (e0 + fill > cap) a.flags[q] = a.epoch;
        unsigned* __restrict__ qkeys = a.keys + (int64_t)q * cap + e0;
        unsigned* __restrict__ qidx = a.idx + (int64_t)q * cap + e0;
        const int fits = e0 + fill <= cap ? fill : (e0 < cap ? (int)(cap - e0) : 0);
#pragma unroll 1
        for (int i = 0; i < fits; ++i) {
          const uint2 v = stage[i * 64];
          qkeys[i] = v.x;
          qidx[i] = v.y;
        }
      }
      fill = 0;
    };
    int me = (int)cap;
    unsigned* __restrict__ mkeys = a.keys + (int64_t)q * cap;
    if constexpr (MAXIMA) {
      if (qvalid) me = atomicAdd(&a.cnt[q], ((sz + 31) >> 5) * (16 / kCellThrGroup));
    }
    uint32_t w[8], wn[8];
    unsigned aux = 0u, aux_n = 0u;
    load_tile(0, w, aux);
    for (int r0 = 0; r0 < sz; r0 += 32) {
      load_tile(r0 + 32, wn, aux_n);
      const bool rv = r0 + col < sz;
      asm volatile("" : "+v"(aux));
      float nrm = 0.f;
      bool live = false;
      if constexpr (NORMS)
        nrm = rv ? __uint_as_float(aux) : __builtin_nanf("");
      else
        live = rv & ((a.is_empty == nullptr) | (aux == 0u));
      f32x16 acc = zero_f32x16();
      float x2 = 0.f;
#pragma unroll
      for (int s = 0; s < KS; ++s) {
        u32x4 vh, vl;
        if constexpr (DS == 2) {
          const int j0 = 8 * s + 4 * half;
          uint2 en[4];
#pragma unroll
          for (int bb = 0; bb < 4; ++bb)
            en[bb] = reinterpret_cast<const uint2*>(book)[(j0 + bb) * 256 + (int)((w[s] >> (8 * bb)) & 255u)];
#pragma unroll
          for (int bb = 0; bb < 4 && !NORMS; ++bb) {
            const float v0 = f16_lo(en[bb].x) + f16_lo(en[bb].y), v1 = f16_hi(en[bb].x) + f16_hi(en[bb].y);
            x2 = fmaf(v0, v0, x2);
            x2 = fmaf(v1, v1, x2);
          }
          vh = u32x4{en[0].x, en[1].x, en[2].x, en[3].x};
          vl = u32x4{en[0].y, en[1].y, en[2].y, en[3].y};
        } else {
          const int j0 = 16 * s + 8 * half;
          unsigned en[8];
#pragma unroll
          for (int bb = 0; bb < 8; ++bb)
            en[bb] = book[(j0 + bb) * 256 + (int)((w[2 * s + (bb >> 2)] >> (8 * (bb & 3))) & 255u)];
#pragma unroll
          for (int bb = 0; bb < 8 && !NORMS; ++bb) {
            const float v0 = f16_lo(en[bb]) + f16_hi(en[bb]);
            x2 = fmaf(v0, v0, x2);
          }
          vh = u32x4{(en[0] & 0xffffu) | (en[1] << 16), (en[2] & 0xffffu) | (en[3] << 16),
                        (en[4] & 0xffffu) | (en[5] << 16), (en[6] & 0xffffu) | (en[7] << 16)};
          vl = u32x4{(en[0] >> 16) | (en[1] & 0xffff0000u), (en[2] >> 16) | (en[3] & 0xffff0000u),
                     (en[4] >> 16) | (en[5] & 0xffff0000u), (en[6] >> 16) | (en[7] & 0xffff0000u)};
        }
        acc = __builtin_amdgcn_mfma_f32_32x32x16_f16(__builtin_bit_cast(f16x8, vl), qh[s], acc, 0, 0, 0);
        acc = __builtin_amdgcn_mfma_f32_32x32x16_f16(__builtin_bit_cast(f16x8, vh), ql[s], acc, 0, 0, 0);
        acc = __builtin_amdgcn_mfma_f32_32x32x16_f16(__builtin_bit_cast(f16x8, vh), qh[s], acc, 0, 0, 0);
      }
      if constexpr (NORMS) {
        if (half == 0) x2w[col] = EUCLID ? nrm : nrm * 0.f;
      } else {
        x2 += __shfl_xor(x2, 32, 64);
        const float v = live ? x2 * inv_sx2 : __builtin_nanf("");
        if (half == 0) x2w[col] = EUCLID ? v : v * 0.f;
      }
      __builtin_amdgcn_fence(__ATOMIC_ACQ_REL, "wavefront");
      if constexpr (MAXIMA) {
        float gm[16 / kCellThrGroup];
#pragma unroll
        for (int g = 0; g < 16 / kCellThrGroup; ++g) gm[g] = -INFINITY;
#pragma unroll
        for (int gq = 0; gq < 4; ++gq) {
          const f32x4 x4 = *reinterpret_cast<const f32x4*>(x2w + 8 * gq + 4 * half);
#pragma unroll
          for (int i = 0; i < 4; ++i) {
            const int r = 4 * gq + i;
            gm[r / kCellThrGroup] = fmaxf(gm[r / kCellThrGroup], fmaf(acc[r], um, -x4[i]));
          }
        }
#pragma unroll
        for (int g = 0; g < 16 / kCellThrGroup; ++g) {
          const unsigned key = gm[g] == -INFINITY ? 0u : f2key(EUCLID ? gm[g] - q2 : gm[g]);
          if (me < (int)cap) mkeys[(int)cap - 1 - me] = key;
          ++me;
        }
        __builtin_amdgcn_fence(__ATOMIC_ACQ_REL, "wavefront");
#pragma unroll
        for (int i = 0; i < 8; ++i) w[i] = wn[i];
        aux = aux_n;
        continue;
      }
      float xr[16];
      bool adm[16];
      unsigned long long any[16];
#pragma unroll
      for (int gq = 0; gq < 4; ++gq) {
        const f32x4 x4 = *reinterpret_cast<const f32x4*>(x2w + 8 * gq + 4 * half);
#pragma unroll
        for (int i = 0; i < 4; ++i) {
          const int r = 4 * gq + i;
          xr[r] = x4[i];
          adm[r] = fmaf(acc[r], um, -xr[r]) >= thr2;
          any[r] = __ballot(adm[r]);
        }
      }
#pragma unroll
      for (int r = 0; r < 16; ++r) asm volatile("" ::"s"(any[r]));
#pragma unroll
      for (int r = 0; r < 16; ++r) {
        if (__builtin_expect(any[r] != 0ull, 0)) {
          if ((any[r] & __ballot(fill >= kDepth)) != 0ull) flush();
          if (adm[r]) {
            const int row = (r & 3) + 8 * (r >> 2) + 4 * half;
            float s = acc[r];
            asm volatile("" : "+v"(s));
            const float dot = s * unscale;
            const float fast = EUCLID ? (2.f * dot - xr[r]) - q2 : dot;
            stage[fill * 64] = make_uint2(f2key(fast), ~(unsigned)(st + r0 + row));
            ++fill;
          }
        }
      }
      __builtin_amdgcn_fence(__ATOMIC_ACQ_REL, "wavefront");
#pragma unroll
      for (int i = 0; i < 8; ++i) w[i] = wn[i];
      aux = aux_n;
    }
    flush();
  }
}

template <int NCH>
__global__ __launch_bounds__(256) void cell_kth_kernel(CellArgs a) {
  const int lane = (int)(threadIdx.x & 63);
  const int q = (int)blockIdx.x * 4 + (int)(threadIdx.x >> 6);
  if (q >= a.nq) return;
  const int n_all = __builtin_amdgcn_readfirstlane(a.cnt[q]);
  if (lane == 0) {
    a.cnt[q] = 0;
    if (a.n_max) a.n_max[q] = n_all;
  }
  if (a.flags[q] == a.epoch) return;
  const int cap = a.chunks * 64;
  const int n = n_all < cap ? n_all : cap;
  const unsigned* __restrict__ keys = a.keys + (int64_t)q * cap;
  unsigned hi[NCH];
#pragma unroll
  for (int t = 0; t < NCH; ++t) hi[t] = t * 64 + lane < n ? keys[cap - 1 - (t * 64 + lane)] : 0u;
  const unsigned fk = finish_fk_upto<2, NCH>(hi, (n + 63) / 64, a.thr_k);
  if (lane == 0) {
    const float t = (fk ? key2f(fk) : -INFINITY) - a.ws_delta[q];
    a.thr[q] = a.euclid ? cell_fold_threshold(t, a.qnorm[q]) : t;
  }
}

template <int DS, bool NORMS, bool MAXIMA = false>
static int launch_cand(const CellArgs& a, dim3 grid, dim3 wg, hipStream_t st) {
  return a.euclid ? launch_with_lds(cell_cand_kernel<DS, NORMS, true, MAXIMA>, "cell_cand_kernel", grid, wg, CellBook<DS>::kBytes, st, a)
                  : launch_with_lds(cell_cand_kernel<DS, NORMS, false, MAXIMA>, "cell_cand_kernel", grid, wg, CellBook<DS>::kBytes, st, a);
}

static int cell_cus() {
  int dev = 0, n_cus = 0;
  if (hipGetDevice(&dev) != hipSuccess ||
      hipDeviceGetAttribute(&n_cus, hipDeviceAttributeMultiprocessorCount, dev) != hipSuccess || n_cus <= 0)
    n_cus = 256;
  return n_cus;
}

static int launch_cell_head(const CellArgs& a, hipStream_t st) {
  hipLaunchKernelGGL(cell_prep_kernel, dim3(1), dim3(1024), 0, st, a);
  TPQ_LAUNCH_CHECK("cell_prep_kernel");
  hipLaunchKernelGGL(cell_seed_kernel, dim3((unsigned)((a.nq + 3) / 4)), dim3(256), 0, st, a);
  TPQ_LAUNCH_CHECK("cell_seed_kernel");
  return TPQ_OK;
}

static int launch_cell_inversion(const CellArgs& a, hipStream_t st) {
  const dim3 per_query((unsigned)((a.nq + 3) / 4));
  const bool lds_hist = a.n_cells <= kCellLdsCells;
  const dim3 per_slice((unsigned)((a.nq + kCellSlice - 1) / kCellSlice)), slice_wg(kCellSliceThreads);
  const size_t hist_lds = (size_t)a.n_cells * sizeof(int);
  if (lds_hist) {
    hipLaunchKernelGGL(cell_count_kernel, per_slice, slice_wg, hist_lds, st, a);
    TPQ_LAUNCH_CHECK("cell_count_kernel");
  } else {
    hipLaunchKernelGGL(cell_count_wide_kernel, per_query, dim3(256), 0, st, a);
    TPQ_LAUNCH_CHECK("cell_count_wide_kernel");
  }
  hipLaunchKernelGGL(cell_scan_kernel, dim3(1), dim3(1024), 0, st, a);
  TPQ_LAUNCH_CHECK("cell_scan_kernel");
  if (lds_hist) {
    hipLaunchKernelGGL(cell_scatter_kernel, per_slice, slice_wg, hist_lds, st, a);
    TPQ_LAUNCH_CHECK("cell_scatter_kernel");
  } else {
    hipLaunchKernelGGL(cell_scatter_wide_kernel, per_query, dim3(256), 0, st, a);
    TPQ_LAUNCH_CHECK("cell_scatter_wide_kernel");
  }
  return TPQ_OK;
}

static int launch_cell_norms(const CellArgs& a, int n_cus, hipStream_t st) {
  const dim3 norm_grid((unsigned)(a.n_cells < n_cus ? a.n_cells : n_cus)), wg(512);
  return a.ds == 1 ? launch_with_lds(cell_norm_kernel<1>, "cell_norm_kernel", norm_grid, wg, 64 * 256 * 4, st, a)
                   : launch_with_lds(cell_norm_kernel<2>, "cell_norm_kernel", norm_grid, wg, 64 * 256 * 8, st, a);
}

static unsigned cell_cand_grid(const CellArgs& a, int n_cus) {
  const int64_t np = (int64_t)a.nq * (a.p_hi > a.p0 ? a.p_hi - a.p0 : 0);
  int64_t blocks = (int64_t)a.n_cells + np / kCellGroup;
  if (blocks > np) blocks = np;
  if (blocks < 1) return 0;
  blocks = (blocks + kCellWaves - 1) / kCellWaves;
  return (unsigned)(blocks > n_cus ? n_cus : blocks);
}

int launch_cell_candidates(const CellArgs& a, hipStream_t st) {
  if (a.nq <= 0) return TPQ_OK;
  if (int rc = launch_cell_head(a, st)) return rc;
  if (a.p_hi <= a.p0) return TPQ_OK;
  if (int rc = launch_cell_inversion(a, st)) return rc;
  const int n_cus = cell_cus();
  const dim3 grid(cell_cand_grid(a, n_cus)), cand_wg(64 * kCellWaves);
  if (a.norm) {
    if (int rc = launch_cell_norms(a, n_cus, st)) return rc;
    return a.ds == 1 ? launch_cand<1, true>(a, grid, cand_wg, st) : launch_cand<2, true>(a, grid, cand_wg, st);
  }
  return a.ds == 1 ? launch_cand<1, false>(a, grid, cand_wg, st) : launch_cand<2, false>(a, grid, cand_wg, st);
}

void cell_fill_thr(CellThrArrays& t, void* at, int nq, int max_nprobe, int n_cells) {
  char* p = reinterpret_cast<char*>(at);
  auto take = [&](size_t bytes) {
    int* r = reinterpret_cast<int*>(p);
    p += cell_align(bytes);
    return r;
  };
  const int tp = max_nprobe < kCellThrProbes ? max_nprobe : kCellThrProbes;
  t.pairs_b = take((size_t)nq * max_nprobe * 4);
  t.hist = take((size_t)n_cells * 4);
  t.cell_off = take(((size_t)n_cells + 1) * 4);
  t.blk_off = take(((size_t)n_cells + 1) * 4);
  t.cell_st = take((size_t)n_cells * 4);
  t.cell_sz = take((size_t)n_cells * 4);
  t.pairs = take((size_t)nq * tp * 4);
  t.n_max = take((size_t)nq * 4);
}

int launch_cell_threshold(const CellArgs& a, const CellThrArrays& t, hipStream_t st) {
  if (a.nq <= 0) return TPQ_OK;
  TPQ_REQUIRE(a.norm && a.k == 0 && a.thr_k >= 1 && a.p0 == 0 && a.p_hi == a.max_nprobe && a.chunks <= 16,
              "ivfpq_scan (cell threshold): arguments outside the form");
  CellArgs b = a;
  b.n_max = t.n_max;
  b.pairs = t.pairs_b;
  b.hist2 = t.hist;
  b.work = 0;
  CellArgs pa = b;
  pa.p_hi = a.max_nprobe < kCellThrProbes ? a.max_nprobe : kCellThrProbes;
  pa.hist = t.hist; pa.cell_off = t.cell_off; pa.blk_off = t.blk_off; pa.cell_st = t.cell_st; pa.cell_sz = t.cell_sz;
  pa.pairs = t.pairs;
  pa.hist2 = nullptr;
  pa.work = 1;
  if (int rc = launch_cell_head(b, st)) return rc;
  if (int rc = launch_cell_inversion(b, st)) return rc;
  const int n_cus = cell_cus();
  if (int rc = launch_cell_norms(b, n_cus, st)) return rc;
  if (int rc = launch_cell_inversion(pa, st)) return rc;
  const dim3 cand_wg(64 * kCellWaves);
  if (int rc = a.ds == 1 ? launch_cand<1, true, true>(pa, dim3(cell_cand_grid(pa, n_cus)), cand_wg, st)
                         : launch_cand<2, true, true>(pa, dim3(cell_cand_grid(pa, n_cus)), cand_wg, st))
    return rc;
  const dim3 per_query((unsigned)((a.nq + 3) / 4));
  if (a.chunks <= 8)
    hipLaunchKernelGGL(cell_kth_kernel<8>, per_query, dim3(256), 0, st, b);
  else
    hipLaunchKernelGGL(cell_kth_kernel<16>, per_query, dim3(256), 0, st, b);
  TPQ_LAUNCH_CHECK("cell_kth_kernel");
  const dim3 grid(cell_cand_grid(b, n_cus));
  return a.ds == 1 ? launch_cand<1, true>(b, grid, cand_wg, st) : launch_cand<2, true>(b, grid, cand_wg, st);
}

}

using namespace tpq;

extern "C" int tpq_ivfpq_cell_candidates(const uint8_t* codes, const float* query, const float* codebook, int ds,
                                         int metric, const uint8_t* is_empty, const int64_t* cell_start,
                                         const int64_t* cell_size, const int64_t* n_probe_list, const int64_t* cells,
                                         int n_cells, int first_probe, const float* threshold, int64_t n_slots, int nq,
                                         int max_nprobe, int m, int capacity, int32_t* out_count, uint32_t* out_keys,
                                         uint32_t* out_addr, float* out_delta, int32_t* out_flags, void* workspace,
                                         size_t workspace_bytes, tpq_stream_t stream) {
  TPQ_REQUIRE(codes && query && codebook && cell_start && cell_size && n_probe_list && cells && threshold &&
                  out_count && out_keys && out_addr && out_delta && out_flags,
              "ivfpq_cell_candidates: null pointer argument");
  TPQ_REQUIRE(m == 64 && (ds == 1 || ds == 2), "ivfpq_cell_candidates: m = 64 and ds <= 2 only (m=%d, ds=%d)", m, ds);
  TPQ_REQUIRE(metric == TPQ_METRIC_NEG_SQ_L2 || metric == TPQ_METRIC_INNER, "ivfpq_cell_candidates: bad metric %d",
              metric);
  TPQ_REQUIRE(nq >= 0 && max_nprobe >= 1 && n_cells >= 1 && first_probe >= 0 && n_slots >= 0 &&
                  n_slots < 0x7fffffffLL && (int64_t)nq * max_nprobe < 0x7fffffffLL,
              "ivfpq_cell_candidates: bad shape (nq=%d, max_nprobe=%d, n_cells=%d, first_probe=%d)", nq, max_nprobe,
              n_cells, first_probe);
  TPQ_REQUIRE(capacity >= 64 && capacity % 64 == 0 && capacity <= 65536,
              "ivfpq_cell_candidates: capacity=%d must be a multiple of 64 in [64, 65536]", capacity);
  const size_t need = cell_extra_bytes(nq, max_nprobe, n_cells, first_probe);
  if (!workspace || workspace_bytes < need) {
    set_error("ivfpq_cell_candidates: workspace too small (%zu < %zu)", workspace_bytes, need);
    return TPQ_ERR_WORKSPACE;
  }
  CellArgs a{};
  a.codes = codes; a.query = query; a.codebook = codebook; a.is_empty = is_empty;
  a.cell_start = cell_start; a.cell_size = cell_size; a.n_probe_list = n_probe_list; a.cells = cells;
  a.n_slots = n_slots; a.nq = nq; a.max_nprobe = max_nprobe; a.n_cells = n_cells; a.ds = ds;
  a.euclid = metric == TPQ_METRIC_NEG_SQ_L2 ? 1 : 0;
  a.p0 = first_probe; a.p_hi = max_nprobe; a.k = 0; a.chunks = capacity / 64; a.epoch = 1; a.rel = cell_delta_rel(ds);
  a.thr_in = threshold;
  a.keys = out_keys; a.idx = out_addr; a.flags = out_flags; a.ws_delta = out_delta;
  cell_fill_extras(a, workspace, workspace_bytes);
  a.cnt = out_count;
  return launch_cell_candidates(a, reinterpret_cast<hipStream_t>(stream));
}

extern "C" float tpq_ivfpq_cell_fold_threshold(float threshold, float q2) { return cell_fold_threshold(threshold, q2); }

extern "C" size_t tpq_ivfpq_cell_candidates_workspace_bytes(int nq, int max_nprobe, int n_cells, int first_probe) {
  if (nq <= 0 || max_nprobe < 1 || n_cells < 1 || first_probe < 0) return 0;
  return cell_extra_bytes(nq, max_nprobe, n_cells, first_probe);
}

extern "C" size_t tpq_ivfpq_cell_candidates_norms_workspace_bytes(int nq, int max_nprobe, int n_cells, int first_probe,
                                                                  int64_t n_slots) {
  if (nq <= 0 || max_nprobe < 1 || n_cells < 1 || first_probe < 0 || n_slots < 0) return 0;
  return cell_extra_bytes(nq, max_nprobe, n_cells, first_probe) + cell_norm_bytes(n_slots);
}
```

torchpq_amd/fn/IVFPQTopk.py:

```python
from ..kernels import IVFPQTopkHip


class IVFPQTopk:
    def __init__(self, n_subvectors, contiguous_size=4, sm_size=None):
        self.n_subvectors = n_subvectors
        self.contiguous_size = contiguous_size
        self._scan = IVFPQTopkHip(m=n_subvectors, n_cs=contiguous_size)

    def topk(self, data, precomputed, cell_start, cell_size, is_empty, n_probe_list, k=256,
             packed=None, address2id=None, slots_hint=None):
        assert 0 < k <= 1024
        return self._scan.topk(data=data, precomputed=precomputed, is_empty=is_empty,
                               cell_start=cell_start, cell_size=cell_size,
                               n_probe_list=n_probe_list, n_candidates=k, packed=packed,
                               address2id=address2id, slots_hint=slots_hint)

    def topk_fused(self, data, query, codebook, cell_start, cell_size, is_empty, n_probe_list, k=256,
                   distance="euclidean", packed=None, address2id=None, slots_hint=None, cells=None, n_cells=0,
                   cell_threshold=True):
        assert 0 < k <= 1024
        return self._scan.topk_fused(data=data, query=query, codebook=codebook, is_empty=is_empty,
                                     cell_start=cell_start, cell_size=cell_size,
                                     n_probe_list=n_probe_list, n_candidates=k, distance=distance,
                                     packed=packed, address2id=address2id, slots_hint=slots_hint,
                                     cells=cells, n_cells=n_cells, cell_threshold=cell_threshold)

    def topk_residual(self, data, precomputed, cell_start, cell_size, base_sims, is_empty,
                      n_probe_list, k=256, address2id=None):
        assert 0 < k <= 1024
        return self._scan.topk_residual(data=data, precomputed=precomputed, base_sims=base_sims,
                                        is_empty=is_empty, cell_start=cell_start,
                                        cell_size=cell_size, n_probe_list=n_probe_list,
                                        n_candidates=k, address2id=address2id)

    def topk_residual_precomputed(self, data, part1, part2, cell_start, cell_size, cells, base_sims,
                                  is_empty, n_probe_list=None, k=256, address2id=None):
        assert 0 < k <= 1024
        return self._scan.topk_residual_precomputed(
            data=data, part1=part1, part2=part2, cells=cells, base_sims=base_sims,
            is_empty=is_empty, cell_start=cell_start, cell_size=cell_size,
            n_probe_list=n_probe_list, n_candidates=k, address2id=address2id)
```

torchpq_amd/index/IVFPQIndex.py:

```python
import torch

from .. import util
from ..codec import PQCodec
from ..container import CellContainer
from ..fn import IVFPQTopk
from ..kernels import PACKED_M, IVFPQFilteredTopkHip, IVFPQRangeHip, ResidualPart1Hip, ResidualSlotTermsHip
from ._coarse import CoarseProbeMixin
from ._filter import IdFilter, filtered_search_batches
from ._range import range_search_batches


class IVFPQIndex(CoarseProbeMixin, CellContainer):
    packed_min_subvectors = 0
    packed_max_short_subvectors = 24
    fused_lut_max_subvector = 4
    use_cell_major = True
    use_cell_threshold = True

    def __init__(self, d_vector, n_subvectors=8, n_cells=128, initial_size=None,
                 expand_step_size=128, expand_mode="double", distance="euclidean",
                 device="cuda:0", pq_use_residual=False, verbose=0):
        if torch.device(device).type == "cuda":
            assert torch.cuda.is_available(), "cuda is not available"
            assert n_subvectors <= util.max_subvectors()
        assert d_vector % n_subvectors == 0
        assert n_subvectors % 4 == 0, "codes are stored 4 sub-quantizers per word (contiguous_size=4)"
        assert distance in ("euclidean", "cosine"), \
            "euclidean and cosine work end to end (MultiKMeans.py:82-113)"
        super().__init__(code_size=n_subvectors, n_cells=n_cells, dtype="uint8", device=device,
                         initial_size=initial_size, expand_step_size=expand_step_size,
                         expand_mode=expand_mode, use_inverse_id_mapping=True, contiguous_size=4,
                         verbose=verbose)
        self.d_vector = d_vector
        self.n_subvectors = n_subvectors
        self.d_subvector = d_vector // n_subvectors
        self.distance = distance
        self.verbose = verbose
        self.pq_use_residual = pq_use_residual
        self._use_precomputed = bool(pq_use_residual and
                                     (n_cells * 256 * n_subvectors * 4) <= 4 * 1024 ** 3)
        self._precomputed_part2 = None
        self._part2_by_cell = None
        self._slot_terms = None
        self._use_cublas = True
        self._use_tensor_core = False
        self._fp16_scale_mode = "a"
        self.use_packed_layout = True
        self.use_fused_lut = True
        self.use_cell_major = True
        self.use_cell_threshold = True

        self._init_coarse(n_cells, verbose)
        self.pq_codec = PQCodec(d_vector=d_vector, n_subvectors=n_subvectors, n_clusters=256,
                                distance=distance, verbose=verbose)
        self._ivfpq_topk = IVFPQTopk(n_subvectors=n_subvectors, contiguous_size=self.contiguous_size)
        self._ivfpq_range = IVFPQRangeHip(m=n_subvectors)
        self._ivfpq_filtered = IVFPQFilteredTopkHip(m=n_subvectors)
        self.to(device)

    @property
    def use_cublas(self):
        return self._use_cublas

    @use_cublas.setter
    def use_cublas(self, value):
        assert type(value) is bool
        self._use_cublas = value

    @property
    def use_tensor_core(self):
        return self._use_tensor_core

    @use_tensor_core.setter
    def use_tensor_core(self, value):
        assert type(value) is bool
        assert self.use_cublas
        self._use_tensor_core = value
        self._coarse_probe.route = "fp16" if value else "auto"

    @property
    def fp16_scale_mode(self):
        return self._fp16_scale_mode

    @fp16_scale_mode.setter
    def fp16_scale_mode(self, value):
        assert value in ["a", "b", "both", "none"]
        self._fp16_scale_mode = value

    @property
    def use_precomputed(self):
        return self._use_precomputed

    @use_precomputed.setter
    def use_precomputed(self, value):
        assert type(value) is bool
        if value:
            assert self.pq_use_residual, " `use_precomputed=True` is only valid when `pq_use_residual` is True"
            assert (self.pq_codec.is_trained and self.vq_codec.is_trained), "index is not trained"
            self.precompute_part2()
        else:
            self._drop_part2()
        self._use_precomputed = value

    def _drop_part2(self):
        self._precomputed_part2 = None
        self._part2_by_cell = None
        self._slot_terms = None

    def precompute_part2(self):
        pq_codebook = self.pq_codec.codebook
        vq_codebook = self.vq_codec.codebook.reshape(self.n_subvectors, self.d_subvector, self.n_cells)
        part2 = (torch.bmm(vq_codebook.transpose(-1, -2), pq_codebook) * -2
                 - pq_codebook.norm(dim=1).pow(2)[:, None])
        self._part2_by_cell = part2.transpose(0, 1).contiguous()
        del part2
        self._precomputed_part2 = self._part2_by_cell.transpose(0, 1)
        self._slot_terms = None

    def _residual_slot_terms(self):
        if self._slot_terms is None or self._slot_terms[0] != self._codes_version:
            st, cb = ResidualSlotTermsHip()(self._storage, self._part2_by_cell, self._cell_start,
                                            self._cell_size)
            self._slot_terms = (self._codes_version, st, cb)
        return self._slot_terms[1], self._slot_terms[2]

    def _codec_knob(codec, attr, typed):
        def getter(self):
            return getattr(getattr(self, codec).kmeans, attr)

        def setter(self, value):
            if typed:
                assert type(value) is int
                assert value > 0
            assert not getattr(self, codec).is_trained, f"{codec} is already trained"
            setattr(getattr(self, codec).kmeans, attr, value)
        return property(getter, setter)

    vq_codec_max_iter = _codec_knob("vq_codec", "max_iter", True)
    vq_codec_n_redo = _codec_knob("vq_codec", "n_redo", True)
    vq_codec_tolerance = _codec_knob("vq_codec", "tol", False)
    pq_codec_max_iter = _codec_knob("pq_codec", "max_iter", True)
    pq_codec_n_redo = _codec_knob("pq_codec", "n_redo", True)
    pq_codec_tolerance = _codec_knob("pq_codec", "tol", False)
    del _codec_knob

    def _after_load_state_dict(self):
        self.to(self.device)
        self._drop_part2()
        super()._after_load_state_dict()

    def train(self, x, force_retrain=False):
        if self.vq_codec.is_trained and self.pq_codec.is_trained and not force_retrain:
            self.print_message("index is already trained", 1)
            return
        x = self._prepare(x)
        self.print_message("start training VQ codec...", 1)
        code = self.vq_codec.train(x)
        self.print_message("start training PQ codec...", 1)
        if self.pq_use_residual:
            self.pq_codec.train((x - self.vq_codec.decode(code)).contiguous())
            self._drop_part2()
        else:
            self.pq_codec.train(x)
        self.print_message("index is trained successfully!", 1)

    def encode(self, x):
        x = self._prepare(x)
        if self.pq_use_residual:
            return self._encode_raw(x)
        return self.pq_codec.encode(x)

    def decode(self, x):
        if self.pq_use_residual:
            assert len(x) == 2
            pq_code, vq_code = x
            assert pq_code.shape[0] == self.n_subvectors
            assert pq_code.shape[1] == vq_code.shape[0]
            return self.vq_codec.decode(vq_code.to(self.device)) + self.pq_codec.decode(pq_code.to(self.device))
        assert len(x.shape) == 2
        assert x.shape[0] == self.n_subvectors
        return self.pq_codec.decode(x.to(self.device))

    def add(self, x, ids=None, return_address=False):
        x = self._prepare(x)
        if self.pq_use_residual:
            codes, assigned_cells = self._encode_raw(x)
        else:
            assigned_cells = self.vq_codec.encode(x)
            codes = self.pq_codec.encode(x)
        return super().add(codes, cells=assigned_cells, ids=ids, return_address=return_address)

    def _encode_raw(self, x):
        vq_code = self.vq_codec.encode(x)
        return self.pq_codec.encode((x - self.vq_codec.decode(vq_code)).contiguous()), vq_code

    def precomputed_adc_residual_precomputed(self, x):
        part1 = ResidualPart1Hip()(x, self.pq_codec.codebook)
        if self._precomputed_part2 is None:
            self.precompute_part2()
        return part1, self._part2_by_cell

    def precomputed_adc_residual(self, x, cells):
        n_query, n_probe = cells.shape
        pq_codebook = self.pq_codec.codebook
        xs = x.reshape(self.n_subvectors, self.d_subvector, n_query).transpose(-1, -2)
        part1 = 2 * (xs @ pq_codebook).permute(1, 0, 2) - pq_codebook.norm(dim=1).pow(2)[None]
        vq = self.vq_codec.codebook.reshape(self.n_subvectors, self.d_subvector, self.n_cells)
        vq = vq[:, :, cells].permute(0, 2, 3, 1)
        part2 = -2 * (vq @ pq_codebook[:, None].expand(-1, n_query, -1, -1))
        return (part1[:, None] + part2.permute(1, 2, 0, 3)).contiguous()

    def _scan_layout(self):
        m = self.n_subvectors
        if self.use_packed_layout and m in PACKED_M and (
                m >= self.packed_min_subvectors or m <= self.packed_max_short_subvectors):
            return self.packed_storage()
        return None

    def search_cells(self, x, cells, base_sims=None, n_probe_list=None, k=1, return_address=False,
                     _extents=None):
        n_probe_list, cell_start, cell_size, slots_hint, is_empty = self._scan_preamble(x, cells, n_probe_list,
                                                                                        _extents)
        lists = dict(data=self._scan_codes(), cell_start=cell_start, cell_size=cell_size, is_empty=is_empty,
                     n_probe_list=n_probe_list, address2id=self._address2id)
        fused = self.use_fused_lut and self.d_subvector <= self.fused_lut_max_subvector
        if self.pq_use_residual:
            assert base_sims is not None, "base_sims is required when pq_use_residual is True"
            if self.use_precomputed and self.use_packed_layout and self.n_subvectors in PACKED_M:
                if self._precomputed_part2 is None:
                    self.precompute_part2()
                slot_term, cell_bound = self._residual_slot_terms()
                part1 = None if fused else self.precomputed_adc_residual_precomputed(x)[0]
                found = self._ivfpq_topk._scan.topk_residual_packed(
                    packed=self.packed_storage(), part2=self._part2_by_cell, slot_term=slot_term,
                    cell_bound=cell_bound, cells=cells, base_sims=base_sims, n_candidates=k, part1=part1,
                    query=x if fused else None, codebook=self.pq_codec.codebook if fused else None,
                    slots_hint=slots_hint, **lists)
            elif self.use_precomputed:
                part1, part2 = self.precomputed_adc_residual_precomputed(x)
                found = self._ivfpq_topk.topk_residual_precomputed(
                    part1=part1, part2=part2, cells=cells, base_sims=base_sims, k=k, **lists)
            else:
                found = self._ivfpq_topk.topk_residual(
                    base_sims=base_sims, precomputed=self.precomputed_adc_residual(x, cells), k=k, **lists)
        elif fused:
            found = self._ivfpq_topk.topk_fused(
                packed=self._scan_layout(), query=x, codebook=self.pq_codec.codebook, k=k, distance=self.distance,
                slots_hint=slots_hint, cells=cells if self.use_cell_major else None, n_cells=self.n_cells,
                cell_threshold=self.use_cell_threshold, **lists)
        else:
            found = self._ivfpq_topk.topk(
                packed=self._scan_layout(), precomputed=self.pq_codec.precompute_adc(x), k=k,
                slots_hint=slots_hint, **lists)
        topk_val, topk_address, topk_ids = found
        return (topk_val, topk_ids, topk_address) if return_address else (topk_val, topk_ids)

    def graphed_search(self, n_query, k=1):
        from .graphed import GraphedSearch
        return GraphedSearch(self, n_query, k)

    def search(self, x, k=1, return_address=False):
        x = self._prepare(x)
        assert 0 < k <= 1024
        assert self.vq_codec.is_trained and self.pq_codec.is_trained, "index is not trained"
        assert 1 <= self.n_probe <= self.n_cells
        return self._search_batches(x, lambda xb, sims, cells, n_probe_list, extents: self.search_cells(
            x=xb, cells=cells, base_sims=sims, n_probe_list=n_probe_list, k=k, return_address=False,
            _extents=extents))

    def range_search_cells(self, x, cells, threshold, base_sims=None, n_probe_list=None, return_address=False,
                           _extents=None):
        n_probe_list, cell_start, cell_size, slots_hint, is_empty = self._scan_preamble(x, cells, n_probe_list,
                                                                                        _extents)
        lists = dict(data=self._scan_codes(), cell_start=cell_start.contiguous(), cell_size=cell_size.contiguous(),
                     n_probe_list=n_probe_list, threshold=threshold, is_empty=is_empty)
        fused = self.use_fused_lut and self.d_subvector <= self.fused_lut_max_subvector
        if self.pq_use_residual:
            assert base_sims is not None, "base_sims is required when pq_use_residual is True"
            if self.use_precomputed:
                if self._precomputed_part2 is None:
                    self.precompute_part2()
                tables = dict(part2=self._part2_by_cell, cells=cells)
                if fused:
                    tables.update(query=x, codebook=self.pq_codec.codebook)
                else:
                    tables.update(part1=ResidualPart1Hip()(x, self.pq_codec.codebook))
            else:
                tables = dict(full=self.precomputed_adc_residual(x, cells))
            lims, vals, address = self._ivfpq_range.residual(base_sims=base_sims, **tables, **lists)
        elif fused:
            lims, vals, address = self._ivfpq_range(query=x, codebook=self.pq_codec.codebook, distance=self.distance,
                                                    slots_hint=slots_hint, **lists)
        else:
            lims, vals, address = self._ivfpq_range(precomputed=self.pq_codec.precompute_adc(x),
                                                    slots_hint=slots_hint, **lists)
        ids = self.get_id_by_address(address) if address.numel() else torch.empty_like(address)
        return (lims, vals, ids, address) if return_address else (lims, vals, ids)

    def range_search(self, x, threshold, return_address=False, sort=False):
        x = self._prepare(x)
        assert self.vq_codec.is_trained and self.pq_codec.is_trained, "index is not trained"
        assert 1 <= self.n_probe <= self.n_cells
        return range_search_batches(
            self, x, threshold, lambda xb, thr, sims, cells, n_probe_list, extents: self.range_search_cells(
                xb, cells, thr, base_sims=sims, n_probe_list=n_probe_list, return_address=True, _extents=extents),
            return_address, sort)

    def id_filter(self, ids):
        return IdFilter(self, ids)

    def search_cells_filtered(self, x, cells, flt, filter_of_query=None, base_sims=None, n_probe_list=None, k=1,
                              return_address=False, _extents=None):
        n_probe_list, cell_start, cell_size, slots_hint, is_empty = self._scan_preamble(x, cells, n_probe_list,
                                                                                        _extents)
        lists = dict(data=self._scan_codes(), cell_start=cell_start, cell_size=cell_size, n_probe_list=n_probe_list,
                     k=k, filter_bits=flt.bits(self), filter_of_query=filter_of_query, is_empty=is_empty,
                     address2id=self._address2id)
        fused = self.use_fused_lut and self.d_subvector <= self.fused_lut_max_subvector
        if self.pq_use_residual:
            assert base_sims is not None, "base_sims is required when pq_use_residual is True"
            if self.use_precomputed:
                if self._precomputed_part2 is None:
                    self.precompute_part2()
                tables = dict(part2=self._part2_by_cell, cells=cells)
                if fused:
                    tables.update(query=x, codebook=self.pq_codec.codebook)
                else:
                    tables.update(part1=ResidualPart1Hip()(x, self.pq_codec.codebook))
            else:
                tables = dict(full=self.precomputed_adc_residual(x, cells))
            vals, address, ids = self._ivfpq_filtered.residual(base_sims=base_sims, **tables, **lists)
        elif fused:
            vals, address, ids = self._ivfpq_filtered(query=x, codebook=self.pq_codec.codebook,
                                                      distance=self.distance, slots_hint=slots_hint, **lists)
        else:
            vals, address, ids = self._ivfpq_filtered(precomputed=self.pq_codec.precompute_adc(x),
                                                      slots_hint=slots_hint, **lists)
        return (vals, ids, address) if return_address else (vals, ids)

    def search_filtered(self, x, k, flt, filter_of_query=None):
        x = self._prepare(x)
        assert 0 < k <= 1024
        assert self.vq_codec.is_trained and self.pq_codec.is_trained, "index is not trained"
        assert 1 <= self.n_probe <= self.n_cells
        return filtered_search_batches(
            self, x, flt, filter_of_query, lambda xb, rows, sims, cells, n_probe_list, extents:
            self.search_cells_filtered(xb, cells, flt, filter_of_query=rows, base_sims=sims,
                                       n_probe_list=n_probe_list, k=k, _extents=extents))
```

torchpq_amd/index/graphed.py:

```python
import torch

from ..util import tensor_version


class GraphedSearch:

    KNOBS = ("n_probe", "use_smart_probing", "_smart_probing_temperature", "use_packed_layout",
             "use_fused_lut", "use_cell_major", "use_cell_threshold", "use_fused_probe", "use_cublas", "_use_precomputed", "pq_use_residual",
             "distance", "max_query_batch", "_has_holes", "_codes_version")

    @staticmethod
    def _buffers(index):
        slot = index._slot_terms
        return {
            "vq_codebook": index.vq_codec.codebook, "pq_codebook": index.pq_codec.codebook,
            "_storage": index._storage, "_packed": index._packed if index._packed_valid else None,
            "_is_empty": index._is_empty, "_address2id": index._address2id,
            "_cell_start": index._cell_start, "_cell_size": index._cell_size,
            "_part2_by_cell": index._part2_by_cell,
            "slot_term": None if slot is None else slot[1],
            "cell_bound": None if slot is None else slot[2],
        }

    @classmethod
    def _snapshot(cls, index):
        knobs = tuple(getattr(index, name) for name in cls.KNOBS)
        bufs = cls._buffers(index)
        ident = tuple((name, None if t is None else (t.data_ptr(), tuple(t.shape), tensor_version(t)))
                      for name, t in bufs.items())
        return knobs, ident, bufs

    def __init__(self, index, n_query, k, warmup=2):
        assert n_query >= 1
        self.index = index
        self.n_query = n_query
        self.k = k
        device = torch.device(index.device)
        self.x = torch.zeros(index.d_vector, n_query, device=device, dtype=torch.float32)
        self._tickets = torch.zeros(max(n_query, 1), device=device, dtype=torch.int32)
        scan = index._ivfpq_topk._scan
        side = torch.cuda.Stream(device=device)
        side.wait_stream(torch.cuda.current_stream(device))
        prev = scan.ticket_buffer
        scan.ticket_buffer = self._tickets
        try:
            with torch.cuda.stream(side):
                for _ in range(warmup):
                    index.search(self.x, k=k)
            torch.cuda.current_stream(device).wait_stream(side)
            self.graph = torch.cuda.CUDAGraph()
            with torch.cuda.graph(self.graph):
                self.values, self.ids = index.search(self.x, k=k)
        finally:
            scan.ticket_buffer = prev
        self._knobs, self._ident, self._held = self._snapshot(index)

    def stale_reason(self):
        knobs, ident, _ = self._snapshot(self.index)
        for name, old, new in zip(self.KNOBS, self._knobs, knobs):
            if old != new:
                return f"{name} changed ({old!r} -> {new!r})"
        for (name, old), (_, new) in zip(self._ident, ident):
            if old != new:
                return f"buffer {name} was replaced or written"
        return None

    def __call__(self, x):
        assert x.shape == self.x.shape, f"graph was captured for queries of shape {tuple(self.x.shape)}"
        why = self.stale_reason()
        if why is not None:
            raise RuntimeError(f"the index changed since the graph was captured ({why}): "
                               "call index.graphed_search() again")
        self.x.copy_(x, non_blocking=True)
        self.graph.replay()
        return self.values, self.ids
```

torchpq_amd/kernels/__init__.py:

```python
from .coarse import (CoarseProbeHip, CoarseSelectHip, SmartProbingHip, Top1SelectHip, Top32SelectHip,
                     TopkSelectHip)
from .container import (GetAddressByIdHip, GetCellByAddressHip, GetIdByAddressHip, GetIOAHip,
                        GetWriteAddressHip, GrowCellsHip, PackCodesHip, PQDecodeHip, ScatterCodesHip)
from .flat import FlatRangeHip, FlatTopkHip
from .kmeans import ComputeCentroidsHip, CoarseAssignHip, LloydStepHip, MaxSimHip, MaxSimSelectHip
from .scan import (PACKED_M, AdcLutHip, CellCandidatesHip, IVFFlatRangeHip, IVFFlatTopkHip, IVFPQ4FilteredTopkHip, IVFPQ4ResidualTopkHip, IVFPQ4TopkHip, IVFPQFilteredTopkHip, IVFPQRangeHip,
                   IVFPQRerankHip, IVFPQTop1Hip, IVFPQTopkHip, ResidualPart1Hip, ResidualSlotTermsHip, ScanOrderHip, SlotFilterBuildHip,
                   packed_chunk_width)

__all__ = [
    "IVFPQTopkHip", "IVFPQTop1Hip", "ScanOrderHip", "CellCandidatesHip", "ResidualPart1Hip", "ResidualSlotTermsHip", "AdcLutHip", "TopkSelectHip", "CoarseSelectHip", "CoarseProbeHip", "Top1SelectHip",
    "Top32SelectHip", "SmartProbingHip", "MaxSimHip", "CoarseAssignHip", "MaxSimSelectHip", "LloydStepHip", "ComputeCentroidsHip", "GetIOAHip",
    "GetWriteAddressHip", "GetCellByAddressHip", "GetIdByAddressHip", "GetAddressByIdHip", "GrowCellsHip", "PQDecodeHip",
    "ScatterCodesHip", "PackCodesHip", "IVFPQRerankHip", "IVFFlatTopkHip", "IVFFlatRangeHip", "IVFPQ4TopkHip", "IVFPQ4ResidualTopkHip", "IVFPQ4FilteredTopkHip", "IVFPQRangeHip", "IVFPQFilteredTopkHip", "SlotFilterBuildHip", "FlatTopkHip", "FlatRangeHip", "packed_chunk_width", "PACKED_M",
]
```

torchpq_amd/kernels/scan.py:

```python
import torch

from .._lib import check, load, ptr, require_gpu, stream_ptr
from ._common import alloc_pair, alloc_topk, call, metric_code, topk_result, workgroups_per_query

PACKED_M = (4, 8, 12, 16, 20, 24, 28, 32, 40, 48, 56, 64, 96, 120, 128)


def packed_chunk_width(m):
    return 16 if m % 16 == 0 else (8 if m % 8 == 0 else 4)


class IVFPQTopkHip:

    def __init__(self, m=8, k=256, tpb=256, n_cs=4, stack_capacity=2, sm_size=None):
        assert k == 256
        assert n_cs == 4
        assert m % n_cs == 0
        self.m = m
        self.k = k
        self.tpb = tpb
        self.n_cs = n_cs
        self.n_cus = None
        self.record_events = None
        self.last_n_split = None
        self.ticket_buffer = None
        self._ticket_cache = {}
        self.keep_workspace = False
        self.last_workspace = None
        self.last_call = None
        self.workspace_bytes = None
        self.last_workspace_bytes = None
        self._last_device = None
        self._last_cells = None
        self._last_withheld = False

    def _tickets(self, n_query, n_split, device):
        if n_split <= 1:
            return None
        if self.ticket_buffer is not None:
            t = self.ticket_buffer
            assert t.dtype == torch.int32 and t.numel() >= n_query and t.device == torch.device(device)
            return t
        if torch.cuda.is_current_stream_capturing():
            return None
        dev = torch.device(device)
        key = (dev.index, torch.cuda.current_stream(dev).cuda_stream)
        t = self._ticket_cache.get(key)
        if t is None or t.numel() < n_query:
            if len(self._ticket_cache) >= 64:
                self._ticket_cache.clear()
            t = torch.zeros(max(n_query, 1024), device=dev, dtype=torch.int32)
            self._ticket_cache[key] = t
        return t

    def _drop_tickets(self, device):
        dev = torch.device(device)
        self._ticket_cache.pop((dev.index, torch.cuda.current_stream(dev).cuda_stream), None)

    def last_redone(self, n_query):
        ws = self.last_workspace
        route = self.last_route()
        if ws is None or route in (None, "reference_layout", "rejected"):
            return None
        off = (n_query * 4 + 255) // 256 * 256
        d = ws[off:off + 4 * n_query].view(torch.float32)
        return int((d == (1.0 if route == "one_launch_finish" else -1.0)).sum().item())

    ROUTES = {0: "reference_layout", 1: "one_launch_finish", 2: "sorted_lists", 3: "pools", 8: "dump_f32",
              16: "dump_sel16", 17: "dump_sel16_w8", -1: "rejected"}

    def route(self, n_query, k, n_split=1, ds=0, n_probe=1, slots_hint=None, has_lut=True, packed=True,
              tickets=None, residual=False):
        if tickets is None:
            tickets = n_split > 1
        code = load().tpq_ivfpq_scan_route(int(n_query), int(k), int(n_split), self.m, int(ds), int(n_probe),
                                            int(slots_hint or 0), int(bool(has_lut)),
                                            int(bool(packed) and self.m in PACKED_M), int(bool(tickets)),
                                            int(bool(residual)))
        return self.ROUTES.get(code, str(code))

    def last_route(self):
        return None if self.last_call is None else self.route(**self.last_call)

    def ordered(self, workspace_bytes, slots=0):
        if self.last_call is None:
            return None
        c = self.last_call
        with torch.cuda.device(self._last_device):
            code = load().tpq_ivfpq_scan_ordered(int(c["n_query"]), int(c["k"]), int(c["n_split"]), self.m, int(c["ds"]),
                                                  int(c["n_probe"]), int(c["slots_hint"] or 0), int(bool(c["has_lut"])),
                                                  int(bool(c["packed"]) and self.m in PACKED_M), int(c["n_split"] > 1),
                                                  int(bool(c.get("residual", False))), int(slots), int(workspace_bytes))
        return code == 1

    def last_ordered(self):
        return None if self.last_call is None else self.ordered(self.last_workspace_bytes)

    def _cell_query(self, name, workspace_bytes, n_cells, n_slots):
        if self.last_call is None:
            return None
        c = self.last_call
        code = getattr(load(), name)(int(c["n_query"]), int(c["k"]), int(c["n_split"]), self.m, int(c["ds"]),
                                     int(c["n_probe"]), int(c["slots_hint"] or 0), int(bool(c["has_lut"])),
                                     int(bool(c["packed"]) and self.m in PACKED_M), int(c["n_split"] > 1),
                                     int(bool(c.get("residual", False))), int(n_cells), int(n_slots),
                                     int(workspace_bytes))
        return code == 1

    def cell_major(self, workspace_bytes, n_cells, n_slots):
        return self._cell_query("tpq_ivfpq_scan_cell_major", workspace_bytes, n_cells, n_slots)

    def cell_norms(self, workspace_bytes, n_cells, n_slots):
        return self._cell_query("tpq_ivfpq_scan_cell_norms", workspace_bytes, n_cells, n_slots)

    def last_cell_major(self):
        if self.last_call is None:
            return None
        if self._last_cells is None:
            return False
        return self.cell_major(self.last_workspace_bytes, *self._last_cells)

    def last_cell_norms(self):
        if self.last_call is None:
            return None
        if self._last_cells is None:
            return False
        return self.cell_norms(self.last_workspace_bytes, *self._last_cells)

    def cell_threshold(self, workspace_bytes, n_cells, n_slots):
        return self._cell_query("tpq_ivfpq_scan_cell_threshold", workspace_bytes, n_cells, n_slots)

    def last_cell_threshold(self):
        if self.last_call is None:
            return None
        if self._last_cells is None or self._last_withheld:
            return False
        return self.cell_threshold(self.last_workspace_bytes, *self._last_cells)

    def last_cell_threshold_state(self):
        assert self.last_workspace is not None and self.last_cell_threshold() is True
        ws, c = self.last_workspace, self.last_call
        nq, k, n_probe = c["n_query"], c["k"], c["n_probe"]
        n_cells, n_slots = self._last_cells
        align = lambda n: (n + 255) // 256 * 256
        lists = lambda ch: 2 * align(nq * 4) + nq * ch * 512 + align(nq * ch * 4)
        extras = load().tpq_ivfpq_cell_candidates_workspace_bytes(nq, n_probe, n_cells, 4)
        chunks = next(ch for ch in (16, 8) if (k + 63) // 64 < ch and self.last_workspace_bytes >= lists(ch) + extras)
        cap = chunks * 64

        def arr(off, n, dtype):
            return ws[off:off + 4 * n].view(dtype)
        band = arr(align(nq * 4), nq, torch.float32).clone()
        keys = arr(2 * align(nq * 4), nq * cap, torch.int32).view(nq, cap)
        ex = lists(chunks) + 256
        thr, qnorm, cand = (arr(ex + i * align(nq * 4), nq, t).clone()
                            for i, t in ((0, torch.float32), (2, torch.float32), (3, torch.int32)))
        t_probes = load().tpq_ivfpq_scan_cell_threshold_probes()
        off = (lists(chunks) + extras + align(n_slots * 4) + align(nq * n_probe * 4) + 3 * align(n_cells * 4)
               + 2 * align((n_cells + 1) * 4) + align(nq * min(t_probes, n_probe) * 4))
        count = arr(off, nq, torch.int32).clone()
        e = torch.arange(cap, device=ws.device)[None, :]
        stored = e < count.clamp(max=cap)[:, None]
        rev = keys.flip(1)
        bits = torch.where(rev < 0, rev & 0x7fffffff, ~rev).view(torch.float32)
        maxima = torch.where(stored, bits, torch.full_like(bits, -float("inf")))
        maxima = torch.where(stored & (rev == 0), torch.full_like(bits, float("nan")), maxima)
        survived = stored & (cap - 1 - e >= cand.clamp(max=cap)[:, None])
        return dict(count=count, maxima=maxima, survived=survived, threshold=thr, band=band, qnorm=qnorm,
                    candidates=cand)

    def _n_split(self, n_query, device, slots_hint=None):
        if self.n_cus is None:
            self.n_cus = torch.cuda.get_device_properties(device).multi_processor_count
        per_cu, waves = (4, 4) if self.m <= 32 else (2, 8) if self.m <= 64 else (1, 16)
        return workgroups_per_query(n_query, self.n_cus, per_cu, waves, slots_hint)

    def _scan(self, name, inputs, data, cell_start, address2id, k, n_split, slots_hint, packed, ticketed,
              cells=None, n_cells=0, cell_threshold=True, **route):
        n_data, device = data.shape[1], data.device
        n_query, n_probe = cell_start.shape
        values, address, ids = alloc_topk(n_query, k, device, address2id)
        if n_query == 0:
            return topk_result(values, address, ids)
        lib = load()
        if n_split is None:
            n_split = self._n_split(n_query, device, slots_hint)
        self.last_n_split = n_split
        self.last_call = dict(n_query=n_query, k=k, n_split=n_split, n_probe=n_probe, slots_hint=slots_hint,
                              packed=packed is not None, **route)
        self._last_cells = (int(n_cells), int(n_data)) if cells is not None else None
        self._last_withheld = not cell_threshold
        ws_bytes = lib.tpq_ivfpq_scan_workspace_bytes(n_query, k, n_split, self.m)
        if self.workspace_bytes is not None:
            ws_bytes = int(self.workspace_bytes)
        self.last_workspace_bytes, self._last_device = ws_bytes, device
        ws = torch.empty(max(ws_bytes, 1), device=device, dtype=torch.uint8)
        ev = None
        if self.record_events is not None:
            ev = (torch.cuda.Event(enable_timing=True), torch.cuda.Event(enable_timing=True))
            ev[0].record(torch.cuda.current_stream(device))
        with torch.cuda.device(device):
            tail = ()
            if ticketed:
                tickets = self._tickets(n_query, n_split, device) if packed is not None else None
                tail = (ptr(tickets), int(slots_hint or 0))
                if cells is not None:
                    tail += (ptr(cells), int(n_cells))
            before = lib.tpq_ivfpq_scan_use_cell_threshold(1 if cell_threshold else 0)
            try:
                rc = getattr(lib, name)(*inputs, ptr(values), ptr(address), ptr(address2id), ptr(ids), n_data, n_query,
                                        n_probe, self.m, k, n_split, ptr(ws), ws_bytes, *tail, stream_ptr(device))
            finally:
                lib.tpq_ivfpq_scan_use_cell_threshold(before)
            if rc != 0 and ticketed:
                self._drop_tickets(device)
            check(rc, name)
        if self.keep_workspace:
            self.last_workspace = ws
        if ev is not None:
            ev[1].record(torch.cuda.current_stream(device))
            self.record_events.append(ev)
        return topk_result(values, address, ids)

    def topk(self, data, precomputed, is_empty, cell_start, cell_size, n_probe_list,
             n_candidates=None, packed=None, address2id=None, n_split=None, slots_hint=None):
        n_data = data.shape[1]
        n_query, n_probe = cell_start.shape
        assert precomputed.shape == (self.m, n_query, self.k)
        assert data.shape[0] == self.m // self.n_cs
        assert data.shape[2] == self.n_cs
        assert cell_size.shape[1] == n_probe
        assert data.dtype == torch.uint8
        assert precomputed.dtype == torch.float32
        assert cell_start.dtype == cell_size.dtype == torch.int64
        assert n_probe_list.shape == (n_query,)
        assert n_probe_list.dtype == torch.int64
        if is_empty is not None:
            assert is_empty.shape[0] == n_data
            assert is_empty.dtype == torch.uint8
        if n_candidates is None:
            n_candidates = self.tpb
        assert 0 < n_candidates <= 1024
        require_gpu(data, precomputed, is_empty, cell_start, cell_size, n_probe_list, packed,
                    address2id)
        inputs = (ptr(data), ptr(precomputed), ptr(is_empty), ptr(cell_start), ptr(cell_size), ptr(n_probe_list))
        if packed is not None and self.m in PACKED_M:
            return self._scan("tpq_ivfpq_scan_topk_packed_tickets", (ptr(packed), *inputs), data, cell_start,
                              address2id, n_candidates, n_split, slots_hint, packed, True, ds=0, has_lut=True)
        return self._scan("tpq_ivfpq_scan_topk", inputs, data, cell_start, address2id, n_candidates, n_split,
                          slots_hint, packed, False, ds=0, has_lut=True)

    def topk_fused(self, data, query, codebook, is_empty, cell_start, cell_size, n_probe_list,
                   n_candidates, distance="euclidean", packed=None, address2id=None, n_split=None,
                   slots_hint=None, cells=None, n_cells=0, cell_threshold=True):
        n_data = data.shape[1]
        n_query, n_probe = cell_start.shape
        m, ds, kk = codebook.shape
        assert m == self.m and kk == self.k
        assert query.shape == (m * ds, n_query)
        assert query.dtype == codebook.dtype == torch.float32
        assert data.shape == (self.m // self.n_cs, n_data, self.n_cs) and data.dtype == torch.uint8
        assert cell_size.shape == (n_query, n_probe)
        assert cell_start.dtype == cell_size.dtype == torch.int64
        assert n_probe_list.shape == (n_query,) and n_probe_list.dtype == torch.int64
        assert 0 < n_candidates <= 1024
        query = query.contiguous()
        codebook = codebook.contiguous()
        require_gpu(data, query, codebook, is_empty, cell_start, cell_size, n_probe_list, packed,
                    address2id)
        inputs = (ptr(packed), ptr(data), ptr(query), ptr(codebook), ds, metric_code(distance), ptr(is_empty),
                  ptr(cell_start), ptr(cell_size), ptr(n_probe_list))
        if cells is not None:
            assert cells.shape == (n_query, n_probe) and cells.dtype == torch.int64 and n_cells >= 1
            cells = cells.contiguous()
            require_gpu(cells)
            return self._scan("tpq_ivfpq_search_fused_cells", inputs, data, cell_start, address2id, n_candidates,
                              n_split, slots_hint, packed, True, cells=cells, n_cells=n_cells, cell_threshold=cell_threshold,
                              ds=ds, has_lut=False)
        return self._scan("tpq_ivfpq_search_fused_tickets", inputs, data, cell_start, address2id, n_candidates,
                          n_split, slots_hint, packed, True, ds=ds, has_lut=False)

    def _residual(self, data, part1, part2, full, cells, base_sims, is_empty, cell_start, cell_size,
                  n_probe_list, n_candidates, address2id):
        n_data = data.shape[1]
        n_query, n_probe = cell_start.shape
        assert data.shape == (self.m // self.n_cs, n_data, self.n_cs)
        assert cell_size.shape == (n_query, n_probe)
        assert base_sims.shape == (n_query, n_probe)
        assert data.dtype == torch.uint8
        assert cell_start.dtype == cell_size.dtype == torch.int64
        assert base_sims.dtype == torch.float32
        assert n_probe_list.shape == (n_query,)
        assert n_probe_list.dtype == torch.int64
        if is_empty is not None:
            assert is_empty.shape == (n_data,) and is_empty.dtype == torch.uint8
        if n_candidates is None:
            n_candidates = self.tpb
        assert 0 < n_candidates <= 1024
        part1 = None if part1 is None else part1.contiguous()
        part2 = None if part2 is None else part2.contiguous()
        full = None if full is None else full.contiguous()
        cells = None if cells is None else cells.contiguous()
        base_sims = base_sims.contiguous()
        require_gpu(data, part1, part2, full, cells, base_sims, is_empty, cell_start, cell_size,
                    n_probe_list, address2id)
        k = n_candidates
        values, address, ids = alloc_topk(n_query, k, data.device, address2id)
        if n_query:
            call("tpq_ivfpq_scan_topk_residual", data.device,
                 ptr(data), ptr(part1), ptr(part2), ptr(full), ptr(cells), ptr(base_sims),
                 ptr(is_empty), ptr(cell_start), ptr(cell_size), ptr(n_probe_list), ptr(values),
                 ptr(address), ptr(address2id), ptr(ids), n_data, n_query, n_probe, self.m, k)
        return topk_result(values, address, ids)

    def topk_residual_packed(self, data, packed, part2, slot_term, cell_bound, cells, base_sims,
                             is_empty, cell_start, cell_size, n_probe_list, n_candidates,
                             part1=None, query=None, codebook=None, address2id=None, n_split=None,
                             slots_hint=None):
        n_data = data.shape[1]
        n_query, n_probe = cell_start.shape
        assert self.m in PACKED_M and packed is not None
        assert data.shape == (self.m // self.n_cs, n_data, self.n_cs) and data.dtype == torch.uint8
        assert part2.shape[1:] == (self.m, self.k) and part2.dtype == torch.float32
        assert part2.is_contiguous()
        assert slot_term.shape == (n_data,) and slot_term.dtype == torch.float32
        assert cell_bound.shape == (part2.shape[0],) and cell_bound.dtype == torch.float32
        assert cells.shape == cell_start.shape == cell_size.shape == base_sims.shape
        assert cells.dtype == cell_start.dtype == cell_size.dtype == torch.int64
        assert base_sims.dtype == torch.float32
        assert n_probe_list.shape == (n_query,) and n_probe_list.dtype == torch.int64
        assert 0 < n_candidates <= 1024
        ds = 0
        if part1 is not None:
            assert part1.shape == (n_query, self.m, self.k) and part1.dtype == torch.float32
            part1 = part1.contiguous()
        else:
            assert query is not None and codebook is not None
            ds = codebook.shape[1]
            assert codebook.shape == (self.m, ds, self.k) and query.shape == (self.m * ds, n_query)
            assert query.dtype == codebook.dtype == torch.float32
            query = query.contiguous()
            codebook = codebook.contiguous()
        cells = cells.contiguous()
        base_sims = base_sims.contiguous()
        require_gpu(data, packed, part1, query, codebook, part2, slot_term, cell_bound, cells,
                    base_sims, is_empty, cell_start, cell_size, n_probe_list, address2id)
        inputs = (ptr(packed), ptr(data), ptr(part1), ptr(query), ptr(codebook), ds, ptr(part2), ptr(slot_term),
                  ptr(cell_bound), ptr(cells), ptr(base_sims), ptr(is_empty), ptr(cell_start), ptr(cell_size),
                  ptr(n_probe_list))
        return self._scan("tpq_ivfpq_scan_topk_residual_packed", inputs, data, cell_start, address2id,
                          n_candidates, n_split, slots_hint, packed, False, ds=ds, has_lut=part1 is not None,
                          residual=True)

    def topk_residual(self, data, precomputed, base_sims, is_empty, cell_start, cell_size,
                      n_probe_list, n_candidates=None, address2id=None):
        n_query, n_probe = cell_start.shape
        assert precomputed.shape == (n_query, n_probe, self.m, self.k)
        assert precomputed.dtype == torch.float32
        return self._residual(data, None, None, precomputed, None, base_sims, is_empty, cell_start,
                              cell_size, n_probe_list, n_candidates, address2id)

    def topk_residual_precomputed(self, data, part1, part2, cells, base_sims, is_empty, cell_start,
                                  cell_size, n_probe_list, n_candidates=None, address2id=None):
        n_query = cell_start.shape[0]
        assert part1.shape == (n_query, self.m, self.k) and part2.shape[1:] == (self.m, self.k)
        assert part1.dtype == part2.dtype == torch.float32
        assert cells.shape == cell_start.shape and cells.dtype == torch.int64
        return self._residual(data, part1, part2, None, cells, base_sims, is_empty, cell_start,
                              cell_size, n_probe_list, n_candidates, address2id)


class CellCandidatesHip:

    def __call__(self, data, query, codebook, cells, n_cells, cell_start, cell_size, n_probe_list, threshold,
                 first_probe=0, capacity=1024, is_empty=None, distance="euclidean", slot_norms=True):
        m, ds, kk = codebook.shape
        n_data = data.shape[1]
        n_query, n_probe = cell_start.shape
        assert m == 64 and kk == 256 and ds in (1, 2) and query.shape == (m * ds, n_query)
        assert data.shape == (16, n_data, 4) and data.dtype == torch.uint8
        assert cells.shape == cell_size.shape == (n_query, n_probe)
        assert cells.dtype == cell_start.dtype == cell_size.dtype == n_probe_list.dtype == torch.int64
        assert threshold.shape == (n_query,) and threshold.dtype == torch.float32
        query, codebook, cells = query.contiguous(), codebook.contiguous(), cells.contiguous()
        require_gpu(data, query, codebook, cells, is_empty, cell_start, cell_size, n_probe_list, threshold)
        dev = data.device
        count = torch.zeros(n_query, device=dev, dtype=torch.int32)
        keys = torch.zeros(n_query, capacity, device=dev, dtype=torch.int32)
        addr = torch.zeros(n_query, capacity, device=dev, dtype=torch.int32)
        band = torch.zeros(n_query, device=dev, dtype=torch.float32)
        flags = torch.zeros(n_query, device=dev, dtype=torch.int32)
        if slot_norms:
            ws_bytes = load().tpq_ivfpq_cell_candidates_norms_workspace_bytes(n_query, n_probe, int(n_cells),
                                                                              int(first_probe), n_data)
        else:
            ws_bytes = load().tpq_ivfpq_cell_candidates_workspace_bytes(n_query, n_probe, int(n_cells), int(first_probe))
        ws = torch.empty(max(ws_bytes, 1), device=dev, dtype=torch.uint8)
        call("tpq_ivfpq_cell_candidates", dev, ptr(data), ptr(query), ptr(codebook), ds, metric_code(distance),
             ptr(is_empty), ptr(cell_start), ptr(cell_size), ptr(n_probe_list), ptr(cells), int(n_cells),
             int(first_probe), ptr(threshold), n_data, n_query, n_probe, m, int(capacity), ptr(count), ptr(keys),
             ptr(addr), ptr(band), ptr(flags), ptr(ws), ws_bytes)
        address = (~addr).to(torch.int64)
        stored = torch.arange(capacity, device=dev)[None, :] < count.clamp(max=capacity)[:, None]
        address = torch.where(stored, address, torch.full_like(address, -1))
        neg = keys < 0
        bits = torch.where(neg, keys & 0x7fffffff, ~keys)
        values = torch.where(stored, bits.view(torch.float32), torch.full_like(band[:, None].expand_as(bits), -float("inf")))
        return count, values, address, band, flags


class ScanOrderHip:

    def __call__(self, cell_start, cell_size, n_probe_list, tile_shift=6):
        n_query, n_probe = cell_start.shape
        assert cell_size.shape == (n_query, n_probe) and n_probe >= 1
        assert cell_start.dtype == cell_size.dtype == torch.int64
        assert n_probe_list.shape == (n_query,) and n_probe_list.dtype == torch.int64
        require_gpu(cell_start, cell_size, n_probe_list)
        order, rank, work = (torch.empty(n_query, device=cell_start.device, dtype=torch.int32) for _ in range(3))
        if n_query:
            call("tpq_ivfpq_scan_order", cell_start.device, ptr(cell_start), ptr(cell_size), ptr(n_probe_list),
                 n_query, n_probe, int(tile_shift), ptr(order), ptr(rank), ptr(work))
        return order, rank, work


class ResidualSlotTermsHip:

    def __call__(self, data, part2, cell_start, cell_size):
        n_cells, m, kk = part2.shape
        n_data = data.shape[1]
        assert kk == 256 and data.shape == (m // 4, n_data, 4) and data.dtype == torch.uint8
# ... 540 lines not shown
```

Baseline: 11.71 million queries/s.

## Persist codebook maxima, book and slot norms across cell-major searches

Adds a persistent 'kept' device buffer holding codebook-derived parameters, a code book table and per-slot norms. It is built on the first cell-major fused search and reused on later calls, with event-based stream ordering and invalidation keyed on the index state. This removes the per-call work of recomputing slot norms and codebook maxima. It also unrolls codebook-maxima prep per DS, moves histogram zeroing into the seed kernel, and adds a two-histogram count variant. The risk is stale state if the index changes without invalidation, plus extra persistent memory.

```diff
diff --git a/include/torchpq_amd.h b/include/torchpq_amd.h
--- a/include/torchpq_amd.h
+++ b/include/torchpq_amd.h
@@ -112,6 +112,18 @@
                                   int64_t n_slots, size_t workspace_bytes);
 int tpq_ivfpq_scan_use_cell_threshold(int on);
 int tpq_ivfpq_scan_cell_threshold_probes(void);
+#define TPQ_HAS_IVFPQ_CELL_KEPT 1
+size_t tpq_ivfpq_cell_kept_bytes(int64_t n_slots, int ds);
+long long tpq_ivfpq_scan_cell_inversions(void);
+int tpq_ivfpq_search_fused_cells_kept(const uint8_t* packed, const uint8_t* codes, const float* query,
+                                      const float* codebook, int ds, int metric, const uint8_t* is_empty,
+                                      const int64_t* cell_start, const int64_t* cell_size,
+                                      const int64_t* n_probe_list, float* out_vals, int64_t* out_addr,
+                                      const int64_t* address2id, int64_t* out_ids, int64_t n_slots,
+                                      int nq, int max_nprobe, int m, int k, int n_split, void* workspace,
+                                      size_t workspace_bytes, int32_t* tickets, int64_t slots_hint,
+                                      const int64_t* cells, int n_cells, void* kept, size_t kept_bytes,
+                                      int kept_valid, tpq_stream_t stream);
 
 int tpq_ivfpq_scan_topk_residual(const uint8_t* codes, const float* part1, const float* part2,
                                  const float* full_lut, const int64_t* cells,
diff --git a/torchpq_amd/_lib.py b/torchpq_amd/_lib.py
--- a/torchpq_amd/_lib.py
+++ b/torchpq_amd/_lib.py
@@ -39,6 +39,11 @@
                                             _i64, _i, _i, _i, _i, _i, _vp, _sz, _vp, _i64, _vp]),
     "tpq_ivfpq_search_fused_cells": (_i, [_vp, _vp, _vp, _vp, _i, _i, _vp, _vp, _vp, _vp, _vp, _vp, _vp, _vp,
                                           _i64, _i, _i, _i, _i, _i, _vp, _sz, _vp, _i64, _vp, _i, _vp]),
+    "tpq_ivfpq_search_fused_cells_kept": (_i, [_vp, _vp, _vp, _vp, _i, _i, _vp, _vp, _vp, _vp, _vp, _vp, _vp, _vp,
+                                               _i64, _i, _i, _i, _i, _i, _vp, _sz, _vp, _i64, _vp, _i, _vp, _sz, _i,
+                                               _vp]),
+    "tpq_ivfpq_cell_kept_bytes": (_sz, [_i64, _i]),
+    "tpq_ivfpq_scan_cell_inversions": (_i64, []),
     "tpq_ivfpq_scan_cell_major": (_i, [_i, _i, _i, _i, _i, _i, _i64, _i, _i, _i, _i, _i, _i64, _sz]),
     "tpq_ivfpq_scan_cell_norms": (_i, [_i, _i, _i, _i, _i, _i, _i64, _i, _i, _i, _i, _i, _i64, _sz]),
     "tpq_ivfpq_cell_candidates_workspace_bytes": (_sz, [_i, _i, _i, _i]),
diff --git a/torchpq_amd/csrc/scan.hip b/torchpq_amd/csrc/scan.hip
--- a/torchpq_amd/csrc/scan.hip
+++ b/torchpq_amd/csrc/scan.hip
@@ -290,7 +290,13 @@
 struct CellMajor {
   const int64_t* cells;
   int n_cells;
+  void* kept = nullptr;
+  size_t kept_bytes = 0;
+  int kept_valid = 0;
 };
+static void cell_major_use_kept(CellArgs& c, const CellMajor& cm) {
+  if (cm.kept && c.norm && cm.kept_bytes >= cell_kept_bytes(c.n_slots, c.ds)) cell_use_kept(c, cm.kept, cm.kept_valid);
+}
 static int cell_major_chunks(const ScanArgs& a, const ScanPlan& p, bool residual, int n_cells, size_t workspace_bytes) {
   if (residual || p.route != TPQ_SCAN_ROUTE_DUMP_SEL16 || a.lut || a.m != 64 || a.ds < 1 || a.ds > 2) return 0;
   if (a.k > 128 || a.max_nprobe <= kCellP0 || n_cells < 1 || a.n_slots <= 0 || a.slots_hint <= 0) return 0;
@@ -344,6 +350,7 @@
   c.list_evict = a.list_evict; c.flags = a.flags; c.ws_delta = a.ws_delta;
   const size_t cm_lists = ws_bytes_for(nq, 1, chunks);
   cell_fill_extras(c, reinterpret_cast<char*>(workspace) + cm_lists, workspace_bytes - cm_lists);
+  cell_major_use_kept(c, cm);
   rc = launch_cell_candidates(c, st);
   if (rc) return rc;
   return u.finish(a, chunks, p.Rf, (a.k + 63) / 64, c.cnt, st);
@@ -375,6 +382,7 @@
   char* at = reinterpret_cast<char*>(workspace) + ws_bytes_for(nq, 1, chunks);
   const size_t head = cell_extra_bytes(nq, a.max_nprobe, cm.n_cells, kCellP0) + cell_norm_bytes(a.n_slots);
   cell_fill_extras(c, at, head, kCellP0);
+  cell_major_use_kept(c, cm);
   CellThrArrays t{};
   cell_fill_thr(t, at + head, nq, a.max_nprobe, cm.n_cells);
   int rc = launch_cell_threshold(c, t, st);
@@ -500,6 +508,35 @@
 
 extern "C" size_t tpq_ivfpq_scan_tickets_bytes(int nq) { return nq > 0 ? (size_t)nq * sizeof(int32_t) : 0; }
 
+extern "C" size_t tpq_ivfpq_cell_kept_bytes(int64_t n_slots, int ds) {
+  return n_slots > 0 && (ds == 1 || ds == 2) ? cell_kept_bytes(n_slots, ds) : 0;
+}
+
+extern "C" int tpq_ivfpq_search_fused_cells_kept(const uint8_t* packed, const uint8_t* codes,
+                                                 const float* query, const float* codebook, int ds,
+                                                 int metric, const uint8_t* is_empty,
+                                                 const int64_t* cell_start, const int64_t* cell_size,
+                                                 const int64_t* n_probe_list, float* out_vals,
+                                                 int64_t* out_addr, const int64_t* address2id,
+                                                 int64_t* out_ids, int64_t n_slots, int nq, int max_nprobe,
+                                                 int m, int k, int n_split, void* workspace,
+                                                 size_t workspace_bytes, int32_t* tickets,
+                                                 int64_t slots_hint, const int64_t* cells, int n_cells,
+                                                 void* kept, size_t kept_bytes, int kept_valid,
+                                                 tpq_stream_t stream) {
+  TPQ_REQUIRE(metric == TPQ_METRIC_NEG_SQ_L2 || metric == TPQ_METRIC_INNER,
+              "ivfpq_search_fused: bad metric %d", metric);
+  TPQ_REQUIRE(ds >= 1 && ds <= 1024, "ivfpq_search_fused: bad sub-vector length %d", ds);
+  ScanArgs a = scan_args(codes, packed, nullptr, is_empty, cell_start, cell_size, n_probe_list, out_vals, out_addr,
+                         address2id, out_ids, n_slots, nq, max_nprobe, m, k, n_split);
+  a.query = query; a.codebook = codebook; a.ds = ds; a.euclid = metric == TPQ_METRIC_NEG_SQ_L2 ? 1 : 0;
+  a.tickets = tickets; a.slots_hint = slots_hint;
+  TPQ_REQUIRE((reinterpret_cast<uintptr_t>(kept) & 15) == 0, "ivfpq_search_fused: the kept state must be 16-byte aligned");
+  const CellMajor cm{cells, n_cells, kept, kept_bytes, kept_valid};
+  return packed ? run_packed(a, nullptr, workspace, workspace_bytes, stream, cells ? &cm : nullptr)
+                : run_ref(a, workspace, workspace_bytes, reinterpret_cast<hipStream_t>(stream));
+}
+
 extern "C" int tpq_ivfpq_search_fused_cells(const uint8_t* packed, const uint8_t* codes,
                                             const float* query, const float* codebook, int ds,
                                             int metric, const uint8_t* is_empty,
@@ -511,16 +548,10 @@
                                             size_t workspace_bytes, int32_t* tickets,
                                             int64_t slots_hint, const int64_t* cells, int n_cells,
                                             tpq_stream_t stream) {
-  TPQ_REQUIRE(metric == TPQ_METRIC_NEG_SQ_L2 || metric == TPQ_METRIC_INNER,
-              "ivfpq_search_fused: bad metric %d", metric);
-  TPQ_REQUIRE(ds >= 1 && ds <= 1024, "ivfpq_search_fused: bad sub-vector length %d", ds);
-  ScanArgs a = scan_args(codes, packed, nullptr, is_empty, cell_start, cell_size, n_probe_list, out_vals, out_addr,
-                         address2id, out_ids, n_slots, nq, max_nprobe, m, k, n_split);
-  a.query = query; a.codebook = codebook; a.ds = ds; a.euclid = metric == TPQ_METRIC_NEG_SQ_L2 ? 1 : 0;
-  a.tickets = tickets; a.slots_hint = slots_hint;
-  const CellMajor cm{cells, n_cells};
-  return packed ? run_packed(a, nullptr, workspace, workspace_bytes, stream, cells ? &cm : nullptr)
-                : run_ref(a, workspace, workspace_bytes, reinterpret_cast<hipStream_t>(stream));
+  return tpq_ivfpq_search_fused_cells_kept(packed, codes, query, codebook, ds, metric, is_empty, cell_start, cell_size,
+                                           n_probe_list, out_vals, out_addr, address2id, out_ids, n_slots, nq,
+                                           max_nprobe, m, k, n_split, workspace, workspace_bytes, tickets, slots_hint,
+                                           cells, n_cells, nullptr, 0, 0, stream);
 }
 
 extern "C" int tpq_ivfpq_search_fused_tickets(const uint8_t* packed, const uint8_t* codes,
diff --git a/torchpq_amd/csrc/scan_cells.h b/torchpq_amd/csrc/scan_cells.h
--- a/torchpq_amd/csrc/scan_cells.h
+++ b/torchpq_amd/csrc/scan_cells.h
@@ -20,11 +20,24 @@
 constexpr int kCellMinRereads = 96;
 constexpr int kCellQSplit = 256;
 constexpr int kCellGroup = 32;
+#ifndef TPQ_CELL_PIECES_A
+#define TPQ_CELL_PIECES_A 2
+#endif
+#ifndef TPQ_CELL_PIECES_B
+#define TPQ_CELL_PIECES_B 1
+#endif
+constexpr int kCellPiecesA = TPQ_CELL_PIECES_A, kCellPiecesB = TPQ_CELL_PIECES_B;
+static_assert(kCellPiecesA >= 1 && kCellPiecesA <= 8 && kCellPiecesB >= 1 && kCellPiecesB <= 8, "pieces per block");
+constexpr int cell_pieces(bool maxima) { return maxima ? kCellPiecesA : kCellPiecesB; }
 #ifndef TPQ_CELL_SLICE
 #define TPQ_CELL_SLICE 128
 #endif
 constexpr int kCellSlice = TPQ_CELL_SLICE;
 constexpr int kCellLdsCells = 16384;
+
+struct CellView {
+  int *hist, *cell_off, *blk_off, *cell_st, *cell_sz, *pairs;
+};
 
 struct CellArgs {
   const uint8_t* codes;
@@ -68,12 +81,31 @@
   float* norm;
   int* hist2;
   int* n_max;
+  int p_a;
+  CellView va;
+  float* kparams;
+  unsigned* book;
+  int kept_build;
 };
+inline size_t cell_book_bytes(int ds) { return (size_t)64 * 256 * 4 * ds; }
+inline size_t cell_kept_bytes(int64_t n_slots, int ds) {
+  return 256 + cell_book_bytes(ds) + ((((size_t)(n_slots > 0 ? n_slots : 0) * 4) + 255) & ~(size_t)255);
+}
+inline void cell_use_kept(CellArgs& a, void* kept, int valid) {
+  char* p = reinterpret_cast<char*>(kept);
+  a.kparams = reinterpret_cast<float*>(p);
+  a.book = reinterpret_cast<unsigned*>(p + 256);
+  a.norm = reinterpret_cast<float*>(p + 256 + cell_book_bytes(a.ds));
+  a.kept_build = valid ? 0 : 1;
+}
 struct CellThrArrays {
   int* pairs_b;
   int *hist, *cell_off, *blk_off, *cell_st, *cell_sz, *pairs, *n_max;
 };
 
+__host__ __device__ inline CellView cell_view(const CellArgs& a) {
+  return CellView{a.hist, a.cell_off, a.blk_off, a.cell_st, a.cell_sz, a.pairs};
+}
 inline size_t cell_align(size_t x) { return (x + 255) & ~(size_t)255; }
 inline size_t cell_extra_bytes(int nq, int max_nprobe, int n_cells, int p0) {
   const int np = max_nprobe > p0 ? max_nprobe - p0 : 0;
diff --git a/torchpq_amd/csrc/scan_cells.hip b/torchpq_amd/csrc/scan_cells.hip
--- a/torchpq_amd/csrc/scan_cells.hip
+++ b/torchpq_amd/csrc/scan_cells.hip
@@ -1,3 +1,4 @@
+#include <atomic>
 #include <cmath>
 
 #include "mfma_util.h"
@@ -37,6 +38,9 @@
   a.cell_sz = reinterpret_cast<int*>(take((size_t)a.n_cells * 4));
   a.pairs = reinterpret_cast<int*>(take((size_t)a.nq * np * 4));
   a.qsplit = reinterpret_cast<_Float16*>(take((size_t)a.nq * kCellQSplit * 2));
+  a.kparams = a.params;
+  a.book = nullptr;
+  a.kept_build = 0;
 }
 
 constexpr int kCellScaleExp = 12;
@@ -45,33 +49,46 @@
 
 __device__ __forceinline__ float pow2i(int e) { return __uint_as_float((unsigned)(e + 127) << 23); }
 __device__ __forceinline__ int exp_of_bits(unsigned bits) { return (int)((bits >> 23) & 255u) - 127; }
+
+template <int DS>
+__device__ __forceinline__ unsigned prep_maxima(const float* __restrict__ codebook, int lane, int wave, float* c2max_s) {
+  float y[4][4][DS];
+#pragma unroll
+  for (int jj = 0; jj < 4; ++jj)
+#pragma unroll
+    for (int cc = 0; cc < 4; ++cc)
+#pragma unroll
+      for (int e = 0; e < DS; ++e) y[jj][cc][e] = codebook[((wave + 16 * jj) * DS + e) * 256 + lane + 64 * cc];
+  unsigned mb = 0u;
+#pragma unroll
+  for (int jj = 0; jj < 4; ++jj) {
+    float c2m = 0.f;
+#pragma unroll
+    for (int cc = 0; cc < 4; ++cc) {
+      float c2 = 0.f;
+#pragma unroll
+      for (int e = 0; e < DS; ++e) {
+        const unsigned b = __float_as_uint(y[jj][cc][e]) & 0x7fffffffu;
+        mb = b > mb ? b : mb;
+        c2 = fmaf(y[jj][cc][e], y[jj][cc][e], c2);
+      }
+      c2m = fmaxf(c2m, c2);
+    }
+#pragma unroll
+    for (int d = 32; d > 0; d >>= 1) c2m = fmaxf(c2m, __shfl_xor(c2m, d, 64));
+    if (lane == 0) c2max_s[wave + 16 * jj] = c2m;
+  }
+  return mb;
+}
 
 __global__ __launch_bounds__(1024) void cell_prep_kernel(CellArgs a) {
   __shared__ unsigned maxbits_s;
   __shared__ float c2max_s[64];
   const int tid = (int)threadIdx.x, lane = tid & 63, wave = tid >> 6;
   if (tid == 0) maxbits_s = 0u;
-  for (int i = tid; i < a.n_cells; i += 1024) a.hist[i] = 0;
-  if (a.hist2)
-    for (int i = tid; i < a.n_cells; i += 1024) a.hist2[i] = 0;
   __syncthreads();
-  unsigned mb = 0u;
-  for (int j = wave; j < 64; j += 16) {
-    float c2m = 0.f;
-    for (int c = lane; c < 256; c += 64) {
-      float c2 = 0.f;
-      for (int e = 0; e < a.ds; ++e) {
-        const float y = a.codebook[((int64_t)j * a.ds + e) * 256 + c];
-        const unsigned b = __float_as_uint(y) & 0x7fffffffu;
-        mb = b > mb ? b : mb;
-        c2 = fmaf(y, y, c2);
-      }
-      c2m = fmaxf(c2m, c2);
-    }
-#pragma unroll
-    for (int d = 32; d > 0; d >>= 1) c2m = fmaxf(c2m, __shfl_xor(c2m, d, 64));
-    if (lane == 0) c2max_s[j] = c2m;
-  }
+  const unsigned mb = a.ds == 1 ? prep_maxima<1>(a.codebook, lane, wave, c2max_s)
+                                : prep_maxima<2>(a.codebook, lane, wave, c2max_s);
   atomicMax(&maxbits_s, mb);
   __syncthreads();
   if (tid == 0) {
@@ -81,12 +98,10 @@
     const unsigned bits = maxbits_s;
     const int e = exp_of_bits(bits);
     const bool ok = bits != 0u && bits <= kMaxFiniteBits && e >= -kCellMaxExp && e <= kCellMaxExp && x2 <= 3e38f;
-    a.params[0] = __uint_as_float(bits);
-    a.params[1] = x2;
-    a.params[2] = ok ? 1.f : 0.f;
-    a.params[3] = ok ? pow2i(kCellScaleExp - e) : 0.f;
-    reinterpret_cast<int*>(a.params)[8] = 0;
-    reinterpret_cast<int*>(a.params)[9] = 0;
+    a.kparams[0] = __uint_as_float(bits);
+    a.kparams[1] = x2;
+    a.kparams[2] = ok ? 1.f : 0.f;
+    a.kparams[3] = ok ? pow2i(kCellScaleExp - e) : 0.f;
   }
 }
 
@@ -108,6 +123,11 @@
 __global__ __launch_bounds__(256) void cell_seed_kernel(CellArgs a) {
   const int lane = (int)(threadIdx.x & 63);
   const int q = (int)blockIdx.x * 4 + (int)(threadIdx.x >> 6);
+  for (int i = (int)(blockIdx.x * 256 + threadIdx.x); i < a.n_cells; i += (int)gridDim.x * 256) {
+    a.hist[i] = 0;
+    if (a.hist2) a.hist2[i] = 0;
+  }
+  if (blockIdx.x == 0 && threadIdx.x < 2) reinterpret_cast<int*>(a.params)[8 + threadIdx.x] = 0;
   if (q >= a.nq) return;
   const int D = 64 * a.ds;
   const float x0 = lane < D ? a.query[(int64_t)lane * a.nq + q] : 0.f;
@@ -132,7 +152,7 @@
   const float tau = a.k > 0 ? a.seed_vals[(int64_t)q * a.k + a.k - 1] : (a.thr_k > 0 ? 0.f : a.thr_in[q]);
   const int eq = exp_of_bits(mb);
   const bool flagged = a.k > 0 && a.flags[q] == a.epoch;
-  const bool scalable = a.params[2] != 0.f && mb != 0u && mb <= kMaxFiniteBits && eq >= -kCellMaxExp &&
+  const bool scalable = a.kparams[2] != 0.f && mb != 0u && mb <= kMaxFiniteBits && eq >= -kCellMaxExp &&
                         eq <= kCellMaxExp && q2 <= 3e38f;
   const bool tau_ok = tau == tau && tau != INFINITY;
   const bool active = !flagged && scalable && tau_ok && !bad_cell;
@@ -144,7 +164,7 @@
     }
     return;
   }
-  const float B = sqrtf(q2) * 1.000001f + sqrtf(a.params[1]) * 1.000001f;
+  const float B = sqrtf(q2) * 1.000001f + sqrtf(a.kparams[1]) * 1.000001f;
   const float delta = a.rel * (B * B);
   if (lane == 0) {
     if (a.thr_k == 0) a.thr[q] = a.euclid ? cell_fold_threshold(tau - delta, q2) : tau - delta;
@@ -196,19 +216,28 @@
     if (lp.listed) f(q, p, lp.cell);
   }
 }
+template <bool TWO>
 __device__ __forceinline__ void count_slice(const CellArgs& a, int q0, int* cell_h) {
-  for (int c = (int)threadIdx.x; c < a.n_cells; c += kCellSliceThreads) cell_h[c] = 0;
+  for (int c = (int)threadIdx.x; c < (TWO ? 2 : 1) * a.n_cells; c += kCellSliceThreads) cell_h[c] = 0;
   __syncthreads();
-  for_slice_pairs(a, q0, [&](int, int, int c) { atomicAdd(&cell_h[c], 1); });
+  for_slice_pairs(a, q0, [&](int, int p, int c) {
+    atomicAdd(&cell_h[c], 1);
+    if (TWO && p < a.p_a) atomicAdd(&cell_h[a.n_cells + c], 1);
+  });
   __syncthreads();
 }
 
+template <bool TWO>
 __global__ __launch_bounds__(kCellSliceThreads) void cell_count_kernel(CellArgs a) {
   extern __shared__ int cell_h[];
-  count_slice(a, (int)blockIdx.x * kCellSlice, cell_h);
+  count_slice<TWO>(a, (int)blockIdx.x * kCellSlice, cell_h);
   for (int c = (int)threadIdx.x; c < a.n_cells; c += kCellSliceThreads) {
     const int h = cell_h[c];
     if (h) atomicAdd(&a.hist[c], h);
+    if constexpr (TWO) {
+      const int ha = cell_h[a.n_cells + c];
+      if (ha) atomicAdd(&a.hist2[c], ha);
+    }
   }
 }
 
@@ -227,6 +256,11 @@
 __global__ __launch_bounds__(1024) void cell_scan_kernel(CellArgs a) {
   __shared__ int sp[2][1024], sb[2][1024];
   const int tid = (int)threadIdx.x;
+  if (blockIdx.x == 1) {
+    a.hist = a.va.hist;
+    a.cell_off = a.va.cell_off;
+    a.blk_off = a.va.blk_off;
+  }
   const int per = (a.n_cells + 1023) / 1024;
   const int lo = tid * per < a.n_cells ? tid * per : a.n_cells;
   const int hi = lo + per < a.n_cells ? lo + per : a.n_cells;
@@ -263,25 +297,33 @@
   }
 }
 
-__device__ __forceinline__ void place_pair(const CellArgs& a, int q, int p, int c, int pos) {
-  a.pairs[pos] = q;
-  if (pos == a.cell_off[c]) {
+__device__ __forceinline__ void place_pair(const CellArgs& a, const CellView& v, int q, int p, int c, int pos) {
+  v.pairs[pos] = q;
+  if (pos == v.cell_off[c]) {
     const int64_t o = (int64_t)q * a.max_nprobe + p;
-    a.cell_st[c] = (int)a.cell_start[o];
-    a.cell_sz[c] = (int)a.cell_size[o];
-  }
-}
-
+    v.cell_st[c] = (int)a.cell_start[o];
+    v.cell_sz[c] = (int)a.cell_size[o];
+  }
+}
+
+template <bool TWO>
 __global__ __launch_bounds__(kCellSliceThreads) void cell_scatter_kernel(CellArgs a) {
   extern __shared__ int cell_h[];
   const int q0 = (int)blockIdx.x * kCellSlice;
-  count_slice(a, q0, cell_h);
+  count_slice<TWO>(a, q0, cell_h);
   for (int c = (int)threadIdx.x; c < a.n_cells; c += kCellSliceThreads) {
     const int h = cell_h[c];
     if (h) cell_h[c] = atomicAdd(&a.hist[c], h);
+    if constexpr (TWO) {
+      const int ha = cell_h[a.n_cells + c];
+      if (ha) cell_h[a.n_cells + c] = atomicAdd(&a.hist2[c], ha);
+    }
   }
   __syncthreads();
-  for_slice_pairs(a, q0, [&](int q, int p, int c) { place_pair(a, q, p, c, atomicAdd(&cell_h[c], 1)); });
+  for_slice_pairs(a, q0, [&](int q, int p, int c) {
+    place_pair(a, cell_view(a), q, p, c, atomicAdd(&cell_h[c], 1));
+    if (TWO && p < a.p_a) place_pair(a, a.va, q, p, c, atomicAdd(&cell_h[a.n_cells + c], 1));
+  });
 }
 
 __global__ __launch_bounds__(256) void cell_scatter_wide_kernel(CellArgs a) {
@@ -292,7 +334,7 @@
   const int n_probe = cell_n_probe(a, q);
   for (int p = a.p0 + lane; p < n_probe; p += 64) {
     const ListedProbe lp = listed_probe(a, q, p);
-    if (lp.listed) place_pair(a, q, p, lp.cell, atomicAdd(&a.hist[lp.cell], 1));
+    if (lp.listed) place_pair(a, cell_view(a), q, p, lp.cell, atomicAdd(&a.hist[lp.cell], 1));
   }
 }
 
@@ -320,12 +362,35 @@
 __device__ __forceinline__ float f16_hi(unsigned w) { return (float)__builtin_bit_cast(_Float16, (unsigned short)(w >> 16)); }
 
 template <int DS>
+__device__ __forceinline__ void book_entry(const float* __restrict__ codebook, float sx, int i, unsigned* book) {
+  const int j = i >> 8, c = i & 255;
+  _Float16 h[DS], l[DS];
+#pragma unroll
+  for (int e = 0; e < DS; ++e) {
+    const float ys = codebook[(j * DS + e) * 256 + c] * sx;
+    h[e] = (_Float16)ys;
+    l[e] = (_Float16)(ys - (float)h[e]);
+  }
+  if constexpr (DS == 2) {
+    book[2 * i] = pack_f16x2(h[0], h[1]);
+    book[2 * i + 1] = pack_f16x2(l[0], l[1]);
+  } else {
+    book[i] = pack_f16x2(h[0], l[0]);
+  }
+}
+template <int DS>
+__global__ __launch_bounds__(256) void cell_book_kernel(CellArgs a) {
+  const int i = (int)(blockIdx.x * 256 + threadIdx.x);
+  book_entry<DS>(a.codebook, a.kparams[3], i, a.book);
+}
+
+template <int DS, bool ALL = false>
 __global__ __launch_bounds__(512) void cell_norm_kernel(CellArgs a) {
   constexpr int KS = 4 * DS;
   extern __shared__ __attribute__((aligned(16))) char smem[];
   float* sums = reinterpret_cast<float*>(smem);
   const int tid = (int)threadIdx.x;
-  const float sx = a.params[3];
+  const float sx = a.kparams[3];
   const float inv_sx = 1.f / sx;
   const float inv_sx2 = inv_sx * inv_sx;
   for (int i = tid; i < 64 * 256; i += 512) {
@@ -339,11 +404,19 @@
     }
   }
   __syncthreads();
-  for (int c = (int)blockIdx.x; c < a.n_cells; c += (int)gridDim.x) {
-    if (a.cell_off[c + 1] == a.cell_off[c]) continue;
-    const int64_t st = a.cell_st[c];
-    int sz = a.cell_sz[c];
-    if (st < 0 || sz < 0 || st + sz > a.n_slots) sz = 0;
+  const int n_units = ALL ? (int)((a.n_slots + 511) / 512) : a.n_cells;
+  for (int c = (int)blockIdx.x; c < n_units; c += (int)gridDim.x) {
+    int64_t st;
+    int sz;
+    if constexpr (ALL) {
+      st = (int64_t)c * 512;
+      sz = a.n_slots - st < 512 ? (int)(a.n_slots - st) : 512;
+    } else {
+      if (a.cell_off[c + 1] == a.cell_off[c]) continue;
+      st = a.cell_st[c];
+      sz = a.cell_sz[c];
+      if (st < 0 || sz < 0 || st + sz > a.n_slots) sz = 0;
+    }
     for (int r = tid; r < sz; r += 512) {
       const int64_t slot = st + r;
       const uint32_t* __restrict__ cw = reinterpret_cast<const uint32_t*>(a.codes) + slot;
@@ -382,6 +455,7 @@
 __global__ __launch_bounds__(CellBook<DS>::kThreads) void cell_cand_kernel(CellArgs a) {
   static_assert(!MAXIMA || NORMS, "pass A reads the slot norms");
   using T = CellBook<DS>;
+  constexpr int S = cell_pieces(MAXIMA);
   constexpr int KS = T::KS;
   constexpr int kDepth = T::kDepth;
   extern __shared__ __attribute__((aligned(16))) char smem[];
@@ -392,25 +466,15 @@
   int* work = reinterpret_cast<int*>(a.params) + 8 + a.work;
   const int n_blocks = a.blk_off[a.n_cells];
   const int col = lane & 31, half = lane >> 5;
-  const float sx = a.params[3];
+  const float sx = a.kparams[3];
   const float inv_sx = 1.f / sx;
   const float inv_sx2 = inv_sx * inv_sx;
   const uint8_t* __restrict__ emp = a.is_empty ? a.is_empty : a.codes;
-  for (int i = tid; i < 64 * 256; i += T::kThreads) {
-    const int j = i >> 8, c = i & 255;
-    _Float16 h[DS], l[DS];
-#pragma unroll
-    for (int e = 0; e < DS; ++e) {
-      const float ys = a.codebook[(j * DS + e) * 256 + c] * sx;
-      h[e] = (_Float16)ys;
-      l[e] = (_Float16)(ys - (float)h[e]);
-    }
-    if constexpr (DS == 2) {
-      book[2 * i] = pack_f16x2(h[0], h[1]);
-      book[2 * i + 1] = pack_f16x2(l[0], l[1]);
-    } else {
-      book[i] = pack_f16x2(h[0], l[0]);
-    }
+  if (a.book) {
+    const u32x4* __restrict__ img = reinterpret_cast<const u32x4*>(a.book);
+    for (int i = tid; i < (int)(T::kBook / 16); i += T::kThreads) reinterpret_cast<u32x4*>(book)[i] = img[i];
+  } else {
+    for (int i = tid; i < 64 * 256; i += T::kThreads) book_entry<DS>(a.codebook, sx, i, book);
   }
   __syncthreads();
   const int64_t cap = (int64_t)a.chunks * 64;
@@ -419,6 +483,8 @@
     int b = 0;
     if (lane == 0) b = atomicAdd(work, 1);
     b = __builtin_amdgcn_readfirstlane(b);
+    const int piece = S > 1 ? b % S : 0;
+    if constexpr (S > 1) b /= S;
     if (b >= n_blocks) break;
     int lo = 0, hi = a.n_cells;
     while (hi - lo > 1) {
@@ -433,6 +499,14 @@
     int sz = a.cell_sz[c];
     if (st < 0 || sz < 0 || st + sz > a.n_slots) sz = 0;
     if (sz == 0) continue;
+    int r_lo = 0, r_hi = sz;
+    if constexpr (S > 1) {
+      const int nt = (sz + 31) >> 5;
+      r_lo = (piece * nt / S) << 5;
+      r_hi = ((piece + 1) * nt / S) << 5;
+      if (r_lo == r_hi) continue;
+      if (r_hi > sz) r_hi = sz;
+    }
     const bool qvalid = col < nqs;
     const int q = qvalid ? a.pairs[first + col] : 0;
     const float sq = qvalid ? a.qscale[q] : 0.f;
@@ -482,12 +556,12 @@
     int me = (int)cap;
     unsigned* __restrict__ mkeys = a.keys + (int64_t)q * cap;
     if constexpr (MAXIMA) {
-      if (qvalid) me = atomicAdd(&a.cnt[q], ((sz + 31) >> 5) * (16 / kCellThrGroup));
+      if (qvalid) me = atomicAdd(&a.cnt[q], ((r_hi - r_lo + 31) >> 5) * (16 / kCellThrGroup));
     }
     uint32_t w[8], wn[8];
     unsigned aux = 0u, aux_n = 0u;
-    load_tile(0, w, aux);
-    for (int r0 = 0; r0 < sz; r0 += 32) {
+    load_tile(r_lo, w, aux);
+    for (int r0 = r_lo; r0 < r_hi; r0 += 32) {
       load_tile(r0 + 32, wn, aux_n);
       const bool rv = r0 + col < sz;
       asm volatile("" : "+v"(aux));
@@ -647,21 +721,52 @@
   return n_cus;
 }
 
-static int launch_cell_head(const CellArgs& a, hipStream_t st) {
+static int launch_cell_kept_build(const CellArgs& a, hipStream_t st) {
   hipLaunchKernelGGL(cell_prep_kernel, dim3(1), dim3(1024), 0, st, a);
   TPQ_LAUNCH_CHECK("cell_prep_kernel");
+  if (a.ds == 1)
+    hipLaunchKernelGGL(cell_book_kernel<1>, dim3(64), dim3(256), 0, st, a);
+  else
+    hipLaunchKernelGGL(cell_book_kernel<2>, dim3(64), dim3(256), 0, st, a);
+  TPQ_LAUNCH_CHECK("cell_book_kernel");
+  const int64_t units = (a.n_slots + 511) / 512;
+  if (units < 1) return TPQ_OK;
+  const int n_cus = cell_cus();
+  const dim3 grid((unsigned)(units < n_cus ? units : n_cus)), wg(512);
+  return a.ds == 1 ? launch_with_lds(cell_norm_kernel<1, true>, "cell_norm_kernel", grid, wg, 64 * 256 * 4, st, a)
+                   : launch_with_lds(cell_norm_kernel<2, true>, "cell_norm_kernel", grid, wg, 64 * 256 * 8, st, a);
+}
+
+static int launch_cell_head(const CellArgs& a, hipStream_t st) {
+  if (!a.book) {
+    hipLaunchKernelGGL(cell_prep_kernel, dim3(1), dim3(1024), 0, st, a);
+    TPQ_LAUNCH_CHECK("cell_prep_kernel");
+  } else if (a.kept_build) {
+    if (int rc = launch_cell_kept_build(a, st)) return rc;
+  }
   hipLaunchKernelGGL(cell_seed_kernel, dim3((unsigned)((a.nq + 3) / 4)), dim3(256), 0, st, a);
   TPQ_LAUNCH_CHECK("cell_seed_kernel");
   return TPQ_OK;
 }
 
+static std::atomic<long long> g_cell_inversions{0};
 static int launch_cell_inversion(const CellArgs& a, hipStream_t st) {
+  g_cell_inversions.fetch_add(1);
   const dim3 per_query((unsigned)((a.nq + 3) / 4));
   const bool lds_hist = a.n_cells <= kCellLdsCells;
   const dim3 per_slice((unsigned)((a.nq + kCellSlice - 1) / kCellSlice)), slice_wg(kCellSliceThreads);
   const size_t hist_lds = (size_t)a.n_cells * sizeof(int);
+  if (a.p_a > 0) {
+    hipLaunchKernelGGL(cell_count_kernel<true>, per_slice, slice_wg, 2 * hist_lds, st, a);
+    TPQ_LAUNCH_CHECK("cell_count_kernel");
+    hipLaunchKernelGGL(cell_scan_kernel, dim3(2), dim3(1024), 0, st, a);
+    TPQ_LAUNCH_CHECK("cell_scan_kernel");
+    hipLaunchKernelGGL(cell_scatter_kernel<true>, per_slice, slice_wg, 2 * hist_lds, st, a);
+    TPQ_LAUNCH_CHECK("cell_scatter_kernel");
+    return TPQ_OK;
+  }
   if (lds_hist) {
-    hipLaunchKernelGGL(cell_count_kernel, per_slice, slice_wg, hist_lds, st, a);
+    hipLaunchKernelGGL(cell_count_kernel<false>, per_slice, slice_wg, hist_lds, st, a);
     TPQ_LAUNCH_CHECK("cell_count_kernel");
   } else {
     hipLaunchKernelGGL(cell_count_wide_kernel, per_query, dim3(256), 0, st, a);
@@ -670,7 +775,7 @@
   hipLaunchKernelGGL(cell_scan_kernel, dim3(1), dim3(1024), 0, st, a);
   TPQ_LAUNCH_CHECK("cell_scan_kernel");
   if (lds_hist) {
-    hipLaunchKernelGGL(cell_scatter_kernel, per_slice, slice_wg, hist_lds, st, a);
+    hipLaunchKernelGGL(cell_scatter_kernel<false>, per_slice, slice_wg, hist_lds, st, a);
     TPQ_LAUNCH_CHECK("cell_scatter_kernel");
   } else {
     hipLaunchKernelGGL(cell_scatter_wide_kernel, per_query, dim3(256), 0, st, a);
@@ -685,24 +790,32 @@
                    : launch_with_lds(cell_norm_kernel<2>, "cell_norm_kernel", norm_grid, wg, 64 * 256 * 8, st, a);
 }
 
-static unsigned cell_cand_grid(const CellArgs& a, int n_cus) {
+static unsigned cell_cand_grid(const CellArgs& a, int n_cus, bool maxima = false) {
   const int64_t np = (int64_t)a.nq * (a.p_hi > a.p0 ? a.p_hi - a.p0 : 0);
   int64_t blocks = (int64_t)a.n_cells + np / kCellGroup;
   if (blocks > np) blocks = np;
   if (blocks < 1) return 0;
-  blocks = (blocks + kCellWaves - 1) / kCellWaves;
+  blocks = (blocks * cell_pieces(maxima) + kCellWaves - 1) / kCellWaves;
   return (unsigned)(blocks > n_cus ? n_cus : blocks);
+}
+
+static bool cell_draws_fit(const CellArgs& a) {
+  const int64_t blocks = (int64_t)a.n_cells + (int64_t)a.nq * a.max_nprobe / kCellGroup;
+  const int s = kCellPiecesA > kCellPiecesB ? kCellPiecesA : kCellPiecesB;
+  return blocks * s + 65536 < 0x7fffffffLL;
 }
 
 int launch_cell_candidates(const CellArgs& a, hipStream_t st) {
   if (a.nq <= 0) return TPQ_OK;
+  TPQ_REQUIRE(cell_draws_fit(a), "ivfpq_scan (cell-major): more pieces of blocks than the draw counter holds");
   if (int rc = launch_cell_head(a, st)) return rc;
   if (a.p_hi <= a.p0) return TPQ_OK;
   if (int rc = launch_cell_inversion(a, st)) return rc;
   const int n_cus = cell_cus();
   const dim3 grid(cell_cand_grid(a, n_cus)), cand_wg(64 * kCellWaves);
   if (a.norm) {
-    if (int rc = launch_cell_norms(a, n_cus, st)) return rc;
+    if (!a.book)
+      if (int rc = launch_cell_norms(a, n_cus, st)) return rc;
     return a.ds == 1 ? launch_cand<1, true>(a, grid, cand_wg, st) : launch_cand<2, true>(a, grid, cand_wg, st);
   }
   return a.ds == 1 ? launch_cand<1, false>(a, grid, cand_wg, st) : launch_cand<2, false>(a, grid, cand_wg, st);
@@ -730,6 +843,7 @@
   if (a.nq <= 0) return TPQ_OK;
   TPQ_REQUIRE(a.norm && a.k == 0 && a.thr_k >= 1 && a.p0 == 0 && a.p_hi == a.max_nprobe && a.chunks <= 16,
               "ivfpq_scan (cell threshold): arguments outside the form");
+  TPQ_REQUIRE(cell_draws_fit(a), "ivfpq_scan (cell threshold): more pieces of blocks than the draw counter holds");
   CellArgs b = a;
   b.n_max = t.n_max;
   b.pairs = t.pairs_b;
@@ -742,13 +856,21 @@
   pa.hist2 = nullptr;
   pa.work = 1;
   if (int rc = launch_cell_head(b, st)) return rc;
+  const bool one_walk = a.n_cells <= kCellLdsCells / 2;
+  if (one_walk) {
+    b.p_a = pa.p_hi;
+    b.va = CellView{t.hist, t.cell_off, t.blk_off, t.cell_st, t.cell_sz, t.pairs};
+  }
   if (int rc = launch_cell_inversion(b, st)) return rc;
+  b.p_a = 0;
   const int n_cus = cell_cus();
-  if (int rc = launch_cell_norms(b, n_cus, st)) return rc;
-  if (int rc = launch_cell_inversion(pa, st)) return rc;
+  if (!b.book)
+    if (int rc = launch_cell_norms(b, n_cus, st)) return rc;
+  if (!one_walk)
+    if (int rc = launch_cell_inversion(pa, st)) return rc;
   const dim3 cand_wg(64 * kCellWaves);
-  if (int rc = a.ds == 1 ? launch_cand<1, true, true>(pa, dim3(cell_cand_grid(pa, n_cus)), cand_wg, st)
-                         : launch_cand<2, true, true>(pa, dim3(cell_cand_grid(pa, n_cus)), cand_wg, st))
+  if (int rc = a.ds == 1 ? launch_cand<1, true, true>(pa, dim3(cell_cand_grid(pa, n_cus, true)), cand_wg, st)
+                         : launch_cand<2, true, true>(pa, dim3(cell_cand_grid(pa, n_cus, true)), cand_wg, st))
     return rc;
   const dim3 per_query((unsigned)((a.nq + 3) / 4));
   if (a.chunks <= 8)
@@ -801,6 +923,8 @@
   return launch_cell_candidates(a, reinterpret_cast<hipStream_t>(stream));
 }
 
+extern "C" long long tpq_ivfpq_scan_cell_inversions(void) { return g_cell_inversions.load(); }
+
 extern "C" float tpq_ivfpq_cell_fold_threshold(float threshold, float q2) { return cell_fold_threshold(threshold, q2); }
 
 extern "C" size_t tpq_ivfpq_cell_candidates_workspace_bytes(int nq, int max_nprobe, int n_cells, int first_probe) {
diff --git a/torchpq_amd/fn/IVFPQTopk.py b/torchpq_amd/fn/IVFPQTopk.py
--- a/torchpq_amd/fn/IVFPQTopk.py
+++ b/torchpq_amd/fn/IVFPQTopk.py
@@ -17,13 +17,13 @@
 
     def topk_fused(self, data, query, codebook, cell_start, cell_size, is_empty, n_probe_list, k=256,
                    distance="euclidean", packed=None, address2id=None, slots_hint=None, cells=None, n_cells=0,
-                   cell_threshold=True):
+                   cell_threshold=True, kept=None):
         assert 0 < k <= 1024
         return self._scan.topk_fused(data=data, query=query, codebook=codebook, is_empty=is_empty,
                                      cell_start=cell_start, cell_size=cell_size,
                                      n_probe_list=n_probe_list, n_candidates=k, distance=distance,
                                      packed=packed, address2id=address2id, slots_hint=slots_hint,
-                                     cells=cells, n_cells=n_cells, cell_threshold=cell_threshold)
+                                     cells=cells, n_cells=n_cells, cell_threshold=cell_threshold, kept=kept)
 
     def topk_residual(self, data, precomputed, cell_start, cell_size, base_sims, is_empty,
                       n_probe_list, k=256, address2id=None):
diff --git a/torchpq_amd/index/IVFPQIndex.py b/torchpq_amd/index/IVFPQIndex.py
--- a/torchpq_amd/index/IVFPQIndex.py
+++ b/torchpq_amd/index/IVFPQIndex.py
@@ -4,7 +4,7 @@
 from ..codec import PQCodec
 from ..container import CellContainer
 from ..fn import IVFPQTopk
-from ..kernels import PACKED_M, IVFPQFilteredTopkHip, IVFPQRangeHip, ResidualPart1Hip, ResidualSlotTermsHip
+from ..kernels import PACKED_M, CellKeptState, IVFPQFilteredTopkHip, IVFPQRangeHip, ResidualPart1Hip, ResidualSlotTermsHip
 from ._coarse import CoarseProbeMixin
 from ._filter import IdFilter, filtered_search_batches
 from ._range import range_search_batches
@@ -16,6 +16,7 @@
     fused_lut_max_subvector = 4
     use_cell_major = True
     use_cell_threshold = True
+    use_cell_kept = True
 
     def __init__(self, d_vector, n_subvectors=8, n_cells=128, initial_size=None,
                  expand_step_size=128, expand_mode="double", distance="euclidean",
@@ -49,6 +50,9 @@
         self.use_fused_lut = True
         self.use_cell_major = True
         self.use_cell_threshold = True
+        self.use_cell_kept = True
+        self._cell_kept = None
+        self._cell_kept_built = 0
 
         self._init_coarse(n_cells, verbose)
         self.pq_codec = PQCodec(d_vector=d_vector, n_subvectors=n_subvectors, n_clusters=256,
@@ -144,9 +148,38 @@
     pq_codec_tolerance = _codec_knob("pq_codec", "tol", False)
     del _codec_knob
 
+    def _cell_kept_state(self, n_bytes, device):
+        def ident(t):
+            return None if t is None else (t.data_ptr(), tuple(t.shape), util.tensor_version(t), str(t.device))
+        key = (self._codes_version, bool(self._has_holes), ident(self.pq_codec.codebook), ident(self._storage),
+               ident(self._is_empty))
+        st = self._cell_kept
+        if st is not None and st.key == key and st.buf.numel() >= n_bytes and st.buf.device == torch.device(device):
+            return st
+        if torch.cuda.is_current_stream_capturing():
+            return None
+        self._drop_cell_kept()
+        self._cell_kept = CellKeptState(n_bytes, device, key)
+        return self._cell_kept
+
+    def _drop_cell_kept(self):
+        if self._cell_kept is not None:
+            self._cell_kept_built += self._cell_kept.builds
+        self._cell_kept = None
+
+    @property
+    def cell_kept_builds(self):
+        return self._cell_kept_built + (0 if self._cell_kept is None else self._cell_kept.builds)
+
+    def to(self, *args, **kwargs):
+        if getattr(self, "_cell_kept", None) is not None:
+            self._drop_cell_kept()
+        return super().to(*args, **kwargs)
+
     def _after_load_state_dict(self):
         self.to(self.device)
         self._drop_part2()
+        self._drop_cell_kept()
         super()._after_load_state_dict()
 
     def train(self, x, force_retrain=False):
@@ -247,7 +280,8 @@
             found = self._ivfpq_topk.topk_fused(
                 packed=self._scan_layout(), query=x, codebook=self.pq_codec.codebook, k=k, distance=self.distance,
                 slots_hint=slots_hint, cells=cells if self.use_cell_major else None, n_cells=self.n_cells,
-                cell_threshold=self.use_cell_threshold, **lists)
+                cell_threshold=self.use_cell_threshold,
+                kept=self._cell_kept_state if self.use_cell_kept and self.use_cell_major else None, **lists)
         else:
             found = self._ivfpq_topk.topk(
                 packed=self._scan_layout(), precomputed=self.pq_codec.precompute_adc(x), k=k,
diff --git a/torchpq_amd/index/graphed.py b/torchpq_amd/index/graphed.py
--- a/torchpq_amd/index/graphed.py
+++ b/torchpq_amd/index/graphed.py
@@ -6,12 +6,13 @@
 class GraphedSearch:
 
     KNOBS = ("n_probe", "use_smart_probing", "_smart_probing_temperature", "use_packed_layout",
-             "use_fused_lut", "use_cell_major", "use_cell_threshold", "use_fused_probe", "use_cublas", "_use_precomputed", "pq_use_residual",
+             "use_fused_lut", "use_cell_major", "use_cell_threshold", "use_cell_kept", "use_fused_probe", "use_cublas", "_use_precomputed", "pq_use_residual",
              "distance", "max_query_batch", "_has_holes", "_codes_version")
 
     @staticmethod
     def _buffers(index):
         slot = index._slot_terms
+        kept = getattr(index, "_cell_kept", None)
         return {
             "vq_codebook": index.vq_codec.codebook, "pq_codebook": index.pq_codec.codebook,
             "_storage": index._storage, "_packed": index._packed if index._packed_valid else None,
@@ -20,6 +21,7 @@
             "_part2_by_cell": index._part2_by_cell,
             "slot_term": None if slot is None else slot[1],
             "cell_bound": None if slot is None else slot[2],
+            "cell_kept": None if kept is None or not kept.valid else kept.buf,
         }
 
     @classmethod
diff --git a/torchpq_amd/kernels/__init__.py b/torchpq_amd/kernels/__init__.py
--- a/torchpq_amd/kernels/__init__.py
+++ b/torchpq_amd/kernels/__init__.py
@@ -4,7 +4,7 @@
                         GetWriteAddressHip, GrowCellsHip, PackCodesHip, PQDecodeHip, ScatterCodesHip)
 from .flat import FlatRangeHip, FlatTopkHip
 from .kmeans import ComputeCentroidsHip, CoarseAssignHip, LloydStepHip, MaxSimHip, MaxSimSelectHip
-from .scan import (PACKED_M, AdcLutHip, CellCandidatesHip, IVFFlatRangeHip, IVFFlatTopkHip, IVFPQ4FilteredTopkHip, IVFPQ4ResidualTopkHip, IVFPQ4TopkHip, IVFPQFilteredTopkHip, IVFPQRangeHip,
+from .scan import (PACKED_M, AdcLutHip, CellCandidatesHip, CellKeptState, IVFFlatRangeHip, IVFFlatTopkHip, IVFPQ4FilteredTopkHip, IVFPQ4ResidualTopkHip, IVFPQ4TopkHip, IVFPQFilteredTopkHip, IVFPQRangeHip,
                    IVFPQRerankHip, IVFPQTop1Hip, IVFPQTopkHip, ResidualPart1Hip, ResidualSlotTermsHip, ScanOrderHip, SlotFilterBuildHip,
                    packed_chunk_width)
 
@@ -12,5 +12,5 @@
     "IVFPQTopkHip", "IVFPQTop1Hip", "ScanOrderHip", "CellCandidatesHip", "ResidualPart1Hip", "ResidualSlotTermsHip", "AdcLutHip", "TopkSelectHip", "CoarseSelectHip", "CoarseProbeHip", "Top1SelectHip",
     "Top32SelectHip", "SmartProbingHip", "MaxSimHip", "CoarseAssignHip", "MaxSimSelectHip", "LloydStepHip", "ComputeCentroidsHip", "GetIOAHip",
     "GetWriteAddressHip", "GetCellByAddressHip", "GetIdByAddressHip", "GetAddressByIdHip", "GrowCellsHip", "PQDecodeHip",
-    "ScatterCodesHip", "PackCodesHip", "IVFPQRerankHip", "IVFFlatTopkHip", "IVFFlatRangeHip", "IVFPQ4TopkHip", "IVFPQ4ResidualTopkHip", "IVFPQ4FilteredTopkHip", "IVFPQRangeHip", "IVFPQFilteredTopkHip", "SlotFilterBuildHip", "FlatTopkHip", "FlatRangeHip", "packed_chunk_width", "PACKED_M",
+    "ScatterCodesHip", "PackCodesHip", "IVFPQRerankHip", "IVFFlatTopkHip", "IVFFlatRangeHip", "IVFPQ4TopkHip", "IVFPQ4ResidualTopkHip", "IVFPQ4FilteredTopkHip", "IVFPQRangeHip", "IVFPQFilteredTopkHip", "SlotFilterBuildHip", "FlatTopkHip", "FlatRangeHip", "packed_chunk_width", "PACKED_M", "CellKeptState",
 ]
diff --git a/torchpq_amd/kernels/scan.py b/torchpq_amd/kernels/scan.py
--- a/torchpq_amd/kernels/scan.py
+++ b/torchpq_amd/kernels/scan.py
@@ -8,6 +8,27 @@
 
 def packed_chunk_width(m):
     return 16 if m % 16 == 0 else (8 if m % 8 == 0 else 4)
+
+
+class CellKeptState:
+
+    def __init__(self, n_bytes, device, key=None):
+        self.buf = torch.empty(n_bytes, device=device, dtype=torch.uint8)
+        self.key = key
+        self.valid = False
+        self.builds = 0
+        self.ready = None
+
+    def before_use(self, device):
+        if self.valid and not torch.cuda.is_current_stream_capturing():
+            torch.cuda.current_stream(device).wait_event(self.ready)
+
+    def after_build(self, device):
+        stream = torch.cuda.current_stream(device)
+        self.ready = torch.cuda.Event()
+        self.ready.record(stream)
+        self.valid = True
+        self.builds += 1
 
 
 class IVFPQTopkHip:
@@ -33,6 +54,7 @@
         self._last_device = None
         self._last_cells = None
         self._last_withheld = False
+        self.last_cell_kept = None
 
     def _tickets(self, n_query, n_split, device):
         if n_split <= 1:
@@ -176,7 +198,7 @@
         return workgroups_per_query(n_query, self.n_cus, per_cu, waves, slots_hint)
 
     def _scan(self, name, inputs, data, cell_start, address2id, k, n_split, slots_hint, packed, ticketed,
-              cells=None, n_cells=0, cell_threshold=True, **route):
+              cells=None, n_cells=0, cell_threshold=True, kept=None, **route):
         n_data, device = data.shape[1], data.device
         n_query, n_probe = cell_start.shape
         values, address, ids = alloc_topk(n_query, k, device, address2id)
@@ -195,6 +217,13 @@
             ws_bytes = int(self.workspace_bytes)
         self.last_workspace_bytes, self._last_device = ws_bytes, device
         ws = torch.empty(max(ws_bytes, 1), device=device, dtype=torch.uint8)
+        self.last_cell_kept = None
+        if kept is not None and cells is not None and self.cell_norms(ws_bytes, n_cells, n_data):
+            kept = kept(lib.tpq_ivfpq_cell_kept_bytes(int(n_data), int(route["ds"])), device)
+            if kept is not None and not kept.valid and torch.cuda.is_current_stream_capturing():
+                kept = None
+        else:
+            kept = None
         ev = None
         if self.record_events is not None:
             ev = (torch.cuda.Event(enable_timing=True), torch.cuda.Event(enable_timing=True))
@@ -206,6 +235,10 @@
                 tail = (ptr(tickets), int(slots_hint or 0))
                 if cells is not None:
                     tail += (ptr(cells), int(n_cells))
+                if kept is not None:
+                    name = "tpq_ivfpq_search_fused_cells_kept"
+                    kept.before_use(device)
+                    tail += (ptr(kept.buf), kept.buf.numel(), int(kept.valid))
             before = lib.tpq_ivfpq_scan_use_cell_threshold(1 if cell_threshold else 0)
             try:
                 rc = getattr(lib, name)(*inputs, ptr(values), ptr(address), ptr(address2id), ptr(ids), n_data, n_query,
@@ -215,6 +248,10 @@
             if rc != 0 and ticketed:
                 self._drop_tickets(device)
             check(rc, name)
+            if kept is not None:
+                self.last_cell_kept = "reused" if kept.valid else "built"
+                if not kept.valid:
+                    kept.after_build(device)
         if self.keep_workspace:
             self.last_workspace = ws
         if ev is not None:
@@ -252,7 +289,7 @@
 
     def topk_fused(self, data, query, codebook, is_empty, cell_start, cell_size, n_probe_list,
                    n_candidates, distance="euclidean", packed=None, address2id=None, n_split=None,
-                   slots_hint=None, cells=None, n_cells=0, cell_threshold=True):
+                   slots_hint=None, cells=None, n_cells=0, cell_threshold=True, kept=None):
         n_data = data.shape[1]
         n_query, n_probe = cell_start.shape
         m, ds, kk = codebook.shape
@@ -276,7 +313,7 @@
             require_gpu(cells)
             return self._scan("tpq_ivfpq_search_fused_cells", inputs, data, cell_start, address2id, n_candidates,
                               n_split, slots_hint, packed, True, cells=cells, n_cells=n_cells, cell_threshold=cell_threshold,
-                              ds=ds, has_lut=False)
+                              kept=kept, ds=ds, has_lut=False)
         return self._scan("tpq_ivfpq_search_fused_tickets", inputs, data, cell_start, address2id, n_candidates,
                           n_split, slots_hint, packed, True, ds=ds, has_lut=False)
 
```

Measured after the change: 12.84 million queries/s, median of 6. 1.1x the previous value.
